# aubin-tchoi/shot-fpfh

Measured on AMD Instinct MI355X. Metric: descriptors/sec (SHOT+FPFH) on 1M-pt cloud, higher is better.
Workload: dtype f64

## Files before the change

### include/shotfpfh.h

```cpp
#ifndef SHOTFPFH_H
#define SHOTFPFH_H

#include <stddef.h>
#include <stdint.h>

#ifdef __cplusplus
extern "C" {
#endif

#define SF_OK 0
#define SF_ERR_ARG (-1)
#define SF_ERR_HIP (-2)
#define SF_ERR_NOMEM (-3)
#define SF_ERR_COMM (-4)
#define SF_ERR_STATE (-5)
#define SF_ERR_UNSUPPORTED (-6)
#define SF_ERR_BIN_RANGE (-7)

#define SF_HOST 0
#define SF_OUT_DEVICE 1
#define SF_IN_DEVICE 2

#define SF_SHOT_LEN 352
#define SF_SHOT_MAX_COSINE_BINS 64
#define SF_FAST_FPFH_BINS 8
#define SF_MAX_FPFH_BINS 1290

typedef struct sf_ctx sf_ctx;
typedef struct sf_cloud sf_cloud;
typedef struct sf_nbrs sf_nbrs;
typedef struct sf_spfh sf_spfh;
typedef struct sf_voxels sf_voxels;

const char *sf_last_error(void);
const char *sf_version(void);
int sf_device_count(void);
sf_ctx *sf_create(int device);
void sf_destroy(sf_ctx *ctx);
int sf_sync(sf_ctx *ctx);
void *sf_stream(sf_ctx *ctx);
int sf_fork(sf_ctx *ctx);
int sf_switch(sf_ctx *ctx, int side);
int sf_join(sf_ctx *ctx);
int sf_mark(sf_ctx *ctx);
int sf_wait_mark(sf_ctx *ctx);

void *sf_dev_alloc(sf_ctx *ctx, size_t bytes);
int sf_dev_free(sf_ctx *ctx, void *dev_ptr);
void *sf_host_alloc(sf_ctx *ctx, size_t bytes);
int sf_host_free(sf_ctx *ctx, void *host_ptr);
int sf_h2d(sf_ctx *ctx, void *dst_dev, const void *src_host, size_t bytes);
int sf_d2h(sf_ctx *ctx, void *dst_host, const void *src_dev, size_t bytes);
int sf_d2d(sf_ctx *ctx, void *dst_dev, const void *src_dev, size_t bytes);

sf_cloud *sf_cloud_upload(sf_ctx *ctx, const double *xyz, const double *normals, int64_t n, int flags);
int sf_cloud_set_normals(sf_ctx *ctx, sf_cloud *cloud, const double *normals, int flags);
int sf_cloud_build_grid(sf_ctx *ctx, sf_cloud *cloud, double cell);
int sf_cloud_build_grid_block(sf_ctx *ctx, sf_cloud *cloud, double cell, int64_t begin, int64_t end, int reach,
                              int64_t *pop_begin, int64_t *pop_end);
int64_t sf_cloud_size(const sf_cloud *cloud);
void sf_cloud_free(sf_ctx *ctx, sf_cloud *cloud);
int sf_cloud_perm(sf_ctx *ctx, sf_cloud *cloud, int32_t *perm);
int sf_cloud_halo_range(sf_ctx *ctx, sf_cloud *cloud, int64_t begin, int64_t end, int64_t *halo_begin,
                        int64_t *halo_end);
int sf_cloud_layer_table(sf_ctx *ctx, sf_cloud *cloud, int64_t *first, int64_t cap, int64_t *n_layers);

sf_nbrs *sf_radius_search(sf_ctx *ctx, sf_cloud *cloud, const double *queries, int64_t m, double radius,
                          int flags);
sf_nbrs *sf_radius_search_self(sf_ctx *ctx, sf_cloud *cloud, double radius, int64_t begin, int64_t end);
sf_nbrs *sf_knn_search(sf_ctx *ctx, sf_cloud *cloud, const double *queries, int64_t m, int k, int flags);
sf_nbrs *sf_nbrs_import(sf_ctx *ctx, sf_cloud *cloud, const double *queries, int64_t m, const int64_t *offsets,
                        const int64_t *idx, double radius, int flags);
sf_nbrs *sf_nbrs_slice(sf_ctx *ctx, sf_nbrs *nbrs, int64_t first, int64_t count);
int64_t sf_nbrs_num_queries(const sf_nbrs *nbrs);
int64_t sf_nbrs_total(const sf_nbrs *nbrs);
int64_t sf_nbrs_max_count(const sf_nbrs *nbrs);
int64_t sf_nbrs_max_count_all(const sf_nbrs *nbrs);
int sf_nbrs_export(sf_ctx *ctx, sf_cloud *cloud, sf_nbrs *nbrs, int64_t *offsets ,
                   int32_t *idx , double *dist );
void sf_nbrs_free(sf_ctx *ctx, sf_nbrs *nbrs);

int sf_normals_radius(sf_ctx *ctx, sf_cloud *cloud, const double *queries, int64_t m, int64_t begin, int64_t end, double radius,
                      const double *pre, double *out , int flags);
int sf_normals(sf_ctx *ctx, sf_cloud *cloud, sf_nbrs *nbrs, const double *pre, double *out ,
               int flags);

int sf_iss_saliency(sf_ctx *ctx, sf_cloud *cloud, double salient_radius, double gamma_21, double gamma_32, int min_neighbors,
                    double *saliency , int32_t *count , int flags);
int sf_iss_select(sf_ctx *ctx, sf_cloud *cloud, const double *saliency , double non_max_radius, int min_neighbors,
                  int64_t *selected , int64_t *n_selected, int flags);
int sf_iss_keypoints(sf_ctx *ctx, sf_cloud *cloud, double salient_radius, double non_max_radius, double gamma_21, double gamma_32,
                     int min_neighbors, double *saliency , int64_t *selected , int64_t *n_selected,
                     int flags);
int sf_pca(sf_ctx *ctx, sf_cloud *cloud, sf_nbrs *nbrs, double *eigenvalues ,
           double *eigenvectors , double *moments , int flags);

int sf_shot_lrf(sf_ctx *ctx, sf_cloud *cloud, sf_nbrs *nbrs, double *lrf , int flags);
int sf_shot(sf_ctx *ctx, sf_cloud *cloud, sf_nbrs *nbrs, const double *lrf , int normalize,
            int64_t min_neighborhood_size, double *out , int flags);
int sf_shot_single_scale(sf_ctx *ctx, sf_cloud *cloud, sf_nbrs *nbrs, int normalize, int64_t min_neighborhood_size,
                         double *lrf , double *out , int flags);

int sf_azimuth_idx(sf_ctx *ctx, const double *x, const double *y, int64_t n, int64_t *idx, int flags);
int sf_shot_serial(sf_ctx *ctx, sf_cloud *cloud, sf_nbrs *nbrs, int64_t min_neighborhood_size, double *out ,
                   int flags);
int sf_shot_serial_bins(sf_ctx *ctx, sf_cloud *cloud, sf_nbrs *nbrs, int64_t n_cosine_bins, int64_t min_neighborhood_size,
                        double *out , int flags);

typedef struct sf_graph sf_graph;
unsigned long long sf_sync_count(void);
int sf_graph_begin(sf_ctx *ctx);
sf_graph *sf_graph_end(sf_ctx *ctx);
int sf_graph_launch(sf_ctx *ctx, sf_graph *graph);
void sf_graph_free(sf_ctx *ctx, sf_graph *graph);

sf_spfh *sf_spfh_create(sf_ctx *ctx, sf_cloud *cloud, int n_bins, int64_t max_count);
sf_spfh *sf_spfh_create_for_radius(sf_ctx *ctx, sf_cloud *cloud, int n_bins, int64_t max_count, double radius);
int sf_spfh_elem_bytes(const sf_spfh *spfh);
int sf_spfh_compute(sf_ctx *ctx, sf_cloud *cloud, sf_nbrs *self_nbrs, sf_spfh *spfh, const double *edges);
int sf_spfh_compute_moments(sf_ctx *ctx, sf_cloud *cloud, sf_nbrs *self_nbrs, sf_spfh *spfh, const double *edges,
                            double *cov_dev );
int sf_shot_from_moments(sf_ctx *ctx, sf_cloud *cloud, sf_nbrs *nbrs, const double *cov_dev , int normalize,
                         int64_t min_neighborhood_size, double *lrf , double *out ,
                         int flags);
int sf_lrf_raw_from_moments(sf_ctx *ctx, sf_cloud *cloud, sf_nbrs *nbrs, const double *cov_dev, double *lrf_dev);
int sf_shot_from_raw_lrf(sf_ctx *ctx, sf_cloud *cloud, sf_nbrs *nbrs, double *lrf_dev, int normalize,
                         int64_t min_neighborhood_size, double *out_dev);
int sf_spfh_allgather(sf_ctx *ctx, sf_spfh *spfh, int64_t rows_per_rank);
int sf_spfh_exchange_rows(sf_ctx *ctx, sf_spfh *spfh, int n_ops, const int *peer, const int64_t *send_begin,
                          const int64_t *send_end, const int64_t *recv_begin, const int64_t *recv_end);
int sf_spfh_rows_image(sf_ctx *ctx, sf_spfh *spfh, int64_t begin, int64_t end, void *host, size_t cap, int write_back,
                       size_t *bytes);
int sf_spfh_export(sf_ctx *ctx, sf_cloud *cloud, sf_spfh *spfh, double *out , int flags);
void sf_spfh_free(sf_ctx *ctx, sf_spfh *spfh);
int sf_fpfh(sf_ctx *ctx, sf_cloud *cloud, sf_nbrs *self_nbrs, sf_spfh *spfh, const int64_t *kp_idx, int64_t m,
            double *out , int flags);

int sf_match_argmin(sf_ctx *ctx, const double *a, int64_t m1, const double *b, int64_t m2, int64_t d,
                    int64_t *idx, double *dist, int64_t *col_idx, int flags);
int sf_match_top2(sf_ctx *ctx, const double *a, int64_t m1, const double *b, int64_t m2, int64_t d,
                  int64_t *idx, double *dist, int64_t *n_exact, int flags);

int sf_rows_nonzero(sf_ctx *ctx, const double *rows_dev, int64_t m, int64_t d, unsigned char *mask_dev);
int sf_rows_gather(sf_ctx *ctx, const double *rows_dev, int64_t n_rows, const int64_t *sel_dev, int64_t m, int64_t d,
                   double *out_dev);
int sf_match_argmin_multiscale(sf_ctx *ctx, const double *a, const double *b, int n_scales, int64_t m1, int64_t m2,
                               int64_t d, const unsigned char *a_ok, const unsigned char *b_ok, double max_val,
                               int64_t *idx, double *dist, int flags);

int sf_match_col_candidates(sf_ctx *ctx, const double *local_dist_dev, const double *global_dist_dev,
                            const int64_t *local_idx_dev, int64_t row_offset, int64_t m, void *cand_dev);

typedef struct sf_match_stream sf_match_stream;
sf_match_stream *sf_match_stream_begin(sf_ctx *ctx, const double *a_dev, const unsigned char *a_ok_dev, int64_t m1,
                                       const double *b_dev, const unsigned char *b_ok_dev, int64_t m2, int64_t d,
                                       double b_entry_max, int64_t max_ranges);
int sf_match_stream_feed(sf_ctx *ctx, sf_match_stream *stream, int64_t row_begin, int64_t row_end);
int sf_match_stream_end(sf_ctx *ctx, sf_match_stream *stream, int64_t *idx_dev, double *dist_dev );
void sf_match_stream_abort(sf_ctx *ctx, sf_match_stream *stream);
int sf_rows_abs_max(sf_ctx *ctx, const double *rows_dev, int64_t m, int64_t d, double *out_host);

int sf_ransac_score(sf_ctx *ctx, const double *a, const double *b, int64_t m, const double *Rt, int64_t n_draws,
                    double thr, int64_t *inliers, int flags);

#define SF_RANSAC_MIN_DRAW_SIZE 3
#define SF_RANSAC_MAX_DRAW_SIZE 8
int sf_ransac_hypotheses(sf_ctx *ctx, const double *a_dev, const double *b_dev, int64_t m, const int64_t *draws_dev,
                         int64_t n_draws, int draw_size, double edge_similarity, unsigned char *status_dev, double *Rt_dev);
int sf_ransac_refit_sums(sf_ctx *ctx, const double *a_dev, const double *b_dev, int64_t m, const double *Rt , double thr,
                         double *sums );
int sf_ransac_prerejective(sf_ctx *ctx, const double *a_dev, const double *b_dev, int64_t m, const int64_t *draws_dev,
                           int64_t n_draws, int draw_size, double edge_similarity, double thr, unsigned char *status_dev,
                           double *Rt_dev, int64_t *map_dev, int64_t *counts_dev, int64_t *result , double *best_Rt );

int sf_fgr_sums(sf_ctx *ctx, const double *a_dev, const double *b_dev, int64_t m, const int64_t *sel_dev , int64_t k,
                const double *state , double *sums );
int sf_fgr(sf_ctx *ctx, const double *a_dev, const double *b_dev, int64_t m, const int64_t *sel_dev , int64_t k,
           double distance_threshold, int iterations, int decrease_every, double division_factor, double *Rt ,
           double *info , double *trace );

int sf_consistency_degree(sf_ctx *ctx, const double *a_dev, const double *b_dev, int64_t m,
                          const unsigned char *member_dev , double distance_threshold, double min_edge,
                          unsigned *degree_out_dev);
int sf_consistency_group(sf_ctx *ctx, const double *a_dev, const double *b_dev, int64_t m, double distance_threshold,
                         double min_edge, unsigned *degree_dev, unsigned char *member_dev, unsigned *group_degree_dev,
                         int64_t *info );

#define SF_SC2_MAX_MATCHES 32768
#define SF_SC2_TILE 256
#define SF_SC2_PAD(m) (((m) + SF_SC2_TILE - 1) / SF_SC2_TILE * SF_SC2_TILE)
int sf_consistency_matrix(sf_ctx *ctx, const double *a_dev, const double *b_dev, int64_t m, double distance_threshold,
                          double min_edge, unsigned char *cmat_dev);
int sf_consistency_sc2(sf_ctx *ctx, const unsigned char *cmat_dev, int64_t m, unsigned *s2_dev);
int sf_consistency_sc2_group(sf_ctx *ctx, const double *a_dev, const double *b_dev, int64_t m, double distance_threshold,
                             double min_edge, unsigned *s2_dev, unsigned char *member_dev, unsigned *group_degree_dev,
                             int64_t *info );

#define SF_SC2_MAX_SEEDS 1024
#define SF_SC2_SEED_TILE 64
int sf_sc2_seeds(sf_ctx *ctx, const unsigned *s2_dev, int64_t m, int64_t n_seeds, int *seeds_dev);
int sf_sc2_seed_rows(sf_ctx *ctx, const unsigned char *cmat_dev, int64_t m, const int *seeds_dev, int64_t n_seeds,
                     unsigned *rows_dev);
int sf_sc2_seed_fits(sf_ctx *ctx, const double *a_dev, const double *b_dev, int64_t m, const int *seeds_dev,
                     const unsigned *rows_dev, int64_t n_seeds, double group_share, unsigned char *status_dev, int *size_dev,
                     double *Rt_dev, double *sums_dev , unsigned char *member_dev );
int sf_sc2_registration(sf_ctx *ctx, const double *a_dev, const double *b_dev, int64_t m, double distance_threshold,
                        double min_edge, int64_t n_seeds, double group_share, unsigned *s2_dev, int *seeds_dev,
                        unsigned char *status_dev, int *size_dev, double *Rt_dev, int64_t *map_dev, int64_t *counts_dev,
                        int64_t *result , double *best_Rt );

sf_voxels *sf_voxels_build(sf_ctx *ctx, const double *xyz, int64_t n, double voxel_size, int flags);
int64_t sf_voxels_count(const sf_voxels *vox);
int sf_voxels_inverse(sf_ctx *ctx, sf_voxels *vox, int64_t *inverse );
int sf_voxels_select(sf_ctx *ctx, sf_voxels *vox, const int64_t *order , int64_t *selected ,
                     int64_t *counts );
void sf_voxels_free(sf_ctx *ctx, sf_voxels *vox);

int sf_icp_accumulate(sf_ctx *ctx, sf_cloud *ref, const double *pts_dev, const int64_t *sel_dev, int64_t m, const double *Rt,
                      double d_max, int mode, double *sums );
int sf_transform_points(sf_ctx *ctx, double *pts_dev, int64_t n, const double *Rt );

int sf_icp_accumulate_gicp(sf_ctx *ctx, sf_cloud *ref, const double *pts_dev, const double *nrm_dev ,
                           const int64_t *sel_dev, int64_t m, const double *Rt, double d_max, double epsilon, double *sums );

int sf_icp_accumulate_robust(sf_ctx *ctx, sf_cloud *ref, const double *pts_dev, const double *nrm_dev ,
                             const int64_t *sel_dev, int64_t m, const double *Rt, double d_max, int mode , double epsilon,
                             int loss , double scale, double *sums );

int sf_comm_unique_id(char id[128]);
int sf_comm_init(sf_ctx *ctx, const char id[128], int nranks, int rank);
int sf_comm_allgather(sf_ctx *ctx, const void *send_dev, void *recv_dev, size_t bytes_per_rank);
int sf_comm_exchange(sf_ctx *ctx, int n_ops, const int *peer, const void *const *send_dev, const size_t *send_bytes,
                     void *const *recv_dev, const size_t *recv_bytes);
int sf_comm_allreduce_min_u64(sf_ctx *ctx, const void *send_dev, void *recv_dev, size_t n);
int sf_comm_collective_stats(sf_ctx *ctx, int on);
int sf_comm_destroy(sf_ctx *ctx);

int sf_profile_enable(sf_ctx *ctx, int on);
int sf_profile_reset(sf_ctx *ctx);
int sf_profile_only(sf_ctx *ctx, const char *name);
int64_t sf_profile_report(sf_ctx *ctx, char *buf, int64_t cap);

#ifdef __cplusplus
}
#endif
#endif
```

### shot_fpfh_amd/_ffi.py

```python
from __future__ import annotations

import ctypes as C
import os

_HERE = os.path.dirname(os.path.abspath(__file__))
LIB_PATH = os.path.join(_HERE, "libshotfpfh.so")

SF_HOST, SF_OUT_DEVICE, SF_IN_DEVICE = 0, 1, 2
SHOT_LEN = 352
MAX_COSINE_BINS = 64
SF_ERR_BIN_RANGE = -7
MAX_FPFH_BINS = 1290


class ShotFpfhError(RuntimeError):
    """Raised for any failure reported by the native library (or its absence)."""


_vp, _i64, _i32, _f64, _int, _sz = C.c_void_p, C.c_int64, C.c_int32, C.c_double, C.c_int, C.c_size_t

SIGNATURES = {
    "sf_last_error": (C.c_char_p, []),
    "sf_version": (C.c_char_p, []),
    "sf_device_count": (_int, []),
    "sf_create": (_vp, [_int]),
    "sf_destroy": (None, [_vp]),
    "sf_sync": (_int, [_vp]),
    "sf_stream": (_vp, [_vp]),
    "sf_fork": (_int, [_vp]),
    "sf_switch": (_int, [_vp, _int]),
    "sf_join": (_int, [_vp]),
    "sf_mark": (_int, [_vp]),
    "sf_wait_mark": (_int, [_vp]),
    "sf_dev_alloc": (_vp, [_vp, _sz]),
    "sf_dev_free": (_int, [_vp, _vp]),
    "sf_host_alloc": (_vp, [_vp, _sz]),
    "sf_host_free": (_int, [_vp, _vp]),
    "sf_h2d": (_int, [_vp, _vp, _vp, _sz]),
    "sf_d2h": (_int, [_vp, _vp, _vp, _sz]),
    "sf_d2d": (_int, [_vp, _vp, _vp, _sz]),
    "sf_cloud_upload": (_vp, [_vp, _vp, _vp, _i64, _int]),
    "sf_cloud_set_normals": (_int, [_vp, _vp, _vp, _int]),
    "sf_cloud_build_grid": (_int, [_vp, _vp, _f64]),
    "sf_cloud_build_grid_block": (_int, [_vp, _vp, _f64, _i64, _i64, _int, _vp, _vp]),
    "sf_cloud_size": (_i64, [_vp]),
    "sf_cloud_free": (None, [_vp, _vp]),
    "sf_cloud_perm": (_int, [_vp, _vp, _vp]),
    "sf_cloud_halo_range": (_int, [_vp, _vp, _i64, _i64, _vp, _vp]),
    "sf_cloud_layer_table": (_int, [_vp, _vp, _vp, _i64, _vp]),
    "sf_radius_search": (_vp, [_vp, _vp, _vp, _i64, _f64, _int]),
    "sf_radius_search_self": (_vp, [_vp, _vp, _f64, _i64, _i64]),
    "sf_knn_search": (_vp, [_vp, _vp, _vp, _i64, _int, _int]),
    "sf_nbrs_import": (_vp, [_vp, _vp, _vp, _i64, _vp, _vp, _f64, _int]),
    "sf_nbrs_slice": (_vp, [_vp, _vp, _i64, _i64]),
    "sf_nbrs_num_queries": (_i64, [_vp]),
    "sf_nbrs_total": (_i64, [_vp]),
    "sf_nbrs_max_count": (_i64, [_vp]),
    "sf_nbrs_max_count_all": (_i64, [_vp]),
    "sf_nbrs_export": (_int, [_vp, _vp, _vp, _vp, _vp, _vp]),
    "sf_nbrs_free": (None, [_vp, _vp]),
    "sf_normals": (_int, [_vp, _vp, _vp, _vp, _vp, _int]),
    "sf_normals_radius": (_int, [_vp, _vp, _vp, _i64, _i64, _i64, _f64, _vp, _vp, _int]),
    "sf_iss_saliency": (_int, [_vp, _vp, _f64, _f64, _f64, _int, _vp, _vp, _int]),
    "sf_iss_select": (_int, [_vp, _vp, _vp, _f64, _int, _vp, _vp, _int]),
    "sf_iss_keypoints": (_int, [_vp, _vp, _f64, _f64, _f64, _f64, _int, _vp, _vp, _vp, _int]),
    "sf_pca": (_int, [_vp, _vp, _vp, _vp, _vp, _vp, _int]),
    "sf_shot_lrf": (_int, [_vp, _vp, _vp, _vp, _int]),
    "sf_shot": (_int, [_vp, _vp, _vp, _vp, _int, _i64, _vp, _int]),
    "sf_shot_single_scale": (_int, [_vp, _vp, _vp, _int, _i64, _vp, _vp, _int]),
    "sf_azimuth_idx": (_int, [_vp, _vp, _vp, _i64, _vp, _int]),
    "sf_shot_serial": (_int, [_vp, _vp, _vp, _i64, _vp, _int]),
    "sf_shot_serial_bins": (_int, [_vp, _vp, _vp, _i64, _i64, _vp, _int]),
    "sf_sync_count": (C.c_ulonglong, []),
    "sf_graph_begin": (_int, [_vp]),
    "sf_graph_end": (_vp, [_vp]),
    "sf_graph_launch": (_int, [_vp, _vp]),
    "sf_graph_free": (None, [_vp, _vp]),
    "sf_spfh_create": (_vp, [_vp, _vp, _int, _i64]),
    "sf_spfh_create_for_radius": (_vp, [_vp, _vp, _int, _i64, C.c_double]),
    "sf_spfh_elem_bytes": (_int, [_vp]),
    "sf_spfh_compute": (_int, [_vp, _vp, _vp, _vp, _vp]),
    "sf_spfh_compute_moments": (_int, [_vp, _vp, _vp, _vp, _vp, _vp]),
    "sf_shot_from_moments": (_int, [_vp, _vp, _vp, _vp, _int, _i64, _vp, _vp, _int]),
    "sf_lrf_raw_from_moments": (_int, [_vp, _vp, _vp, _vp, _vp]),
    "sf_shot_from_raw_lrf": (_int, [_vp, _vp, _vp, _vp, _int, _i64, _vp]),
    "sf_spfh_allgather": (_int, [_vp, _vp, _i64]),
    "sf_spfh_exchange_rows": (_int, [_vp, _vp, _int, _vp, _vp, _vp, _vp, _vp]),
    "sf_spfh_rows_image": (_int, [_vp, _vp, _i64, _i64, _vp, _sz, _int, _vp]),
    "sf_spfh_export": (_int, [_vp, _vp, _vp, _vp, _int]),
    "sf_spfh_free": (None, [_vp, _vp]),
    "sf_fpfh": (_int, [_vp, _vp, _vp, _vp, _vp, _i64, _vp, _int]),
    "sf_match_argmin": (_int, [_vp, _vp, _i64, _vp, _i64, _i64, _vp, _vp, _vp, _int]),
    "sf_match_top2": (_int, [_vp, _vp, _i64, _vp, _i64, _i64, _vp, _vp, _vp, _int]),
    "sf_rows_nonzero": (_int, [_vp, _vp, _i64, _i64, _vp]),
    "sf_rows_gather": (_int, [_vp, _vp, _i64, _vp, _i64, _i64, _vp]),
    "sf_match_argmin_multiscale": (_int, [_vp, _vp, _vp, _int, _i64, _i64, _i64, _vp, _vp, _f64, _vp, _vp, _int]),
    "sf_match_col_candidates": (_int, [_vp, _vp, _vp, _vp, _i64, _i64, _vp]),
    "sf_match_stream_begin": (_vp, [_vp, _vp, _vp, _i64, _vp, _vp, _i64, _i64, _f64, _i64]),
    "sf_match_stream_feed": (_int, [_vp, _vp, _i64, _i64]),
    "sf_match_stream_end": (_int, [_vp, _vp, _vp, _vp]),
    "sf_match_stream_abort": (None, [_vp, _vp]),
    "sf_rows_abs_max": (_int, [_vp, _vp, _i64, _i64, _vp]),
    "sf_ransac_score": (_int, [_vp, _vp, _vp, _i64, _vp, _i64, _f64, _vp, _int]),
    "sf_ransac_hypotheses": (_int, [_vp, _vp, _vp, _i64, _vp, _i64, _int, _f64, _vp, _vp]),
    "sf_ransac_refit_sums": (_int, [_vp, _vp, _vp, _i64, _vp, _f64, _vp]),
    "sf_ransac_prerejective": (_int, [_vp, _vp, _vp, _i64, _vp, _i64, _int, _f64, _f64, _vp, _vp, _vp, _vp, _vp, _vp]),
    "sf_fgr_sums": (_int, [_vp, _vp, _vp, _i64, _vp, _i64, _vp, _vp]),
    "sf_fgr": (_int, [_vp, _vp, _vp, _i64, _vp, _i64, _f64, _int, _int, _f64, _vp, _vp, _vp]),
    "sf_consistency_degree": (_int, [_vp, _vp, _vp, _i64, _vp, _f64, _f64, _vp]),
    "sf_consistency_group": (_int, [_vp, _vp, _vp, _i64, _f64, _f64, _vp, _vp, _vp, _vp]),
    "sf_consistency_matrix": (_int, [_vp, _vp, _vp, _i64, _f64, _f64, _vp]),
    "sf_consistency_sc2": (_int, [_vp, _vp, _i64, _vp]),
    "sf_consistency_sc2_group": (_int, [_vp, _vp, _vp, _i64, _f64, _f64, _vp, _vp, _vp, _vp]),
    "sf_sc2_seeds": (_int, [_vp, _vp, _i64, _i64, _vp]),
    "sf_sc2_seed_rows": (_int, [_vp, _vp, _i64, _vp, _i64, _vp]),
    "sf_sc2_seed_fits": (_int, [_vp, _vp, _vp, _i64, _vp, _vp, _i64, _f64, _vp, _vp, _vp, _vp, _vp]),
    "sf_sc2_registration": (_int, [_vp, _vp, _vp, _i64, _f64, _f64, _i64, _f64, _vp, _vp, _vp, _vp, _vp, _vp, _vp, _vp, _vp]),
    "sf_voxels_build": (_vp, [_vp, _vp, _i64, _f64, _int]),
    "sf_voxels_count": (_i64, [_vp]),
    "sf_voxels_inverse": (_int, [_vp, _vp, _vp]),
    "sf_voxels_select": (_int, [_vp, _vp, _vp, _vp, _vp]),
    "sf_voxels_free": (None, [_vp, _vp]),
    "sf_icp_accumulate": (_int, [_vp, _vp, _vp, _vp, _i64, _vp, _f64, _int, _vp]),
    "sf_transform_points": (_int, [_vp, _vp, _i64, _vp]),
    "sf_icp_accumulate_gicp": (_int, [_vp, _vp, _vp, _vp, _vp, _i64, _vp, _f64, _f64, _vp]),
    "sf_icp_accumulate_robust": (_int, [_vp, _vp, _vp, _vp, _vp, _i64, _vp, _f64, _int, _f64, _int, _f64, _vp]),
    "sf_comm_unique_id": (_int, [_vp]),
    "sf_comm_init": (_int, [_vp, _vp, _int, _int]),
    "sf_comm_allgather": (_int, [_vp, _vp, _vp, _sz]),
    "sf_comm_exchange": (_int, [_vp, _int, _vp, _vp, _vp, _vp, _vp]),
    "sf_comm_allreduce_min_u64": (_int, [_vp, _vp, _vp, _sz]),
    "sf_comm_collective_stats": (_int, [_vp, _int]),
    "sf_comm_destroy": (_int, [_vp]),
    "sf_profile_enable": (_int, [_vp, _int]),
    "sf_profile_reset": (_int, [_vp]),
    "sf_profile_only": (_int, [_vp, C.c_char_p]),
    "sf_profile_report": (_i64, [_vp, _vp, _i64]),
}

_lib = None


def load() -> C.CDLL:
    global _lib
    if _lib is not None:
        return _lib
    if not os.path.exists(LIB_PATH):
        raise ShotFpfhError(
            f"{LIB_PATH} is missing: build it with `python -c 'import __graft_entry__ as g; g.build()'` "
            "(hipcc --offload-arch=gfx950).  shot_fpfh_amd has no CPU fallback."
        )
    try:
        lib = C.CDLL(LIB_PATH, mode=C.RTLD_GLOBAL)
    except OSError as exc:
        raise ShotFpfhError(f"cannot load {LIB_PATH}: {exc}") from exc
    for name, (res, args) in SIGNATURES.items():
        fn = getattr(lib, name)
        fn.restype = res
        fn.argtypes = args
    _lib = lib
    return lib


def last_error() -> str:
    return load().sf_last_error().decode("utf-8", "replace")


def check(rc: int, what: str = "") -> None:
    if rc != 0:
        raise ShotFpfhError(f"{what or 'libshotfpfh'} failed ({rc}): {last_error()}")


def check_handle(h, what: str):
    if not h:
        raise ShotFpfhError(f"{what} failed: {last_error()}")
    return h
```

### shot_fpfh_amd/csrc/device_util.h

```cpp
#pragma once
#include <hip/hip_runtime.h>

#include <cstdint>

struct sf_cloud;

struct sf_grid_desc {
    double lo[3];
    double inv_cell;
    double inv_cell_x;
    double cell;
    int dim[3];
    int xsub;
};

#ifdef __HIPCC__
__host__ __device__ inline int sf_cell_coord(double v, double lo, double inv_cell, int dim)
{
    double t = floor((v - lo) * inv_cell);
    if (!(t >= 0.0)) t = 0.0;
    double top = (double)(dim - 1);
    if (t > top) t = top;
    return (int)t;
}

__device__ inline int sf_lane() { return (int)__builtin_amdgcn_mbcnt_hi(~0u, __builtin_amdgcn_mbcnt_lo(~0u, 0u)); }

__device__ inline int sf_prefix_count(unsigned long long mask)
{
    return (int)__builtin_amdgcn_mbcnt_hi((unsigned)(mask >> 32), __builtin_amdgcn_mbcnt_lo((unsigned)mask, 0u));
}

__device__ inline double sf_wave_sum(double v)
{
#define SF_DPP_ADD_ALL(ctrl)                                                                                    \
    {                                                                                                           \
        const int lo = __builtin_amdgcn_mov_dpp(__double2loint(v), ctrl, 0xf, 0xf, true);                       \
        const int hi = __builtin_amdgcn_mov_dpp(__double2hiint(v), ctrl, 0xf, 0xf, true);                       \
        v += __hiloint2double(hi, lo);                                                                          \
    }
#define SF_DPP_ADD(ctrl, row_mask)                                                                              \
    {                                                                                                           \
        const int lo = __builtin_amdgcn_update_dpp(0, __double2loint(v), ctrl, row_mask, 0xf, false);           \
        const int hi = __builtin_amdgcn_update_dpp(0, __double2hiint(v), ctrl, row_mask, 0xf, false);           \
        v += __hiloint2double(hi, lo);                                                                          \
    }
    SF_DPP_ADD_ALL(0xB1)
    SF_DPP_ADD_ALL(0x4E)
    SF_DPP_ADD_ALL(0x141)
    SF_DPP_ADD_ALL(0x140)
    SF_DPP_ADD(0x142, 0xa)
    SF_DPP_ADD(0x143, 0xc)
#undef SF_DPP_ADD
#undef SF_DPP_ADD_ALL
    return __hiloint2double(__builtin_amdgcn_readlane(__double2hiint(v), 63),
                            __builtin_amdgcn_readlane(__double2loint(v), 63));
}

__device__ inline double sf_wave_max_nonneg(double v)
{
#define SF_DPP_MAX(ctrl, row_mask)                                                                              \
    {                                                                                                           \
        const int lo = __builtin_amdgcn_update_dpp(0, __double2loint(v), ctrl, row_mask, 0xf, false);           \
        const int hi = __builtin_amdgcn_update_dpp(0, __double2hiint(v), ctrl, row_mask, 0xf, false);           \
        v = fmax(v, __hiloint2double(hi, lo));                                                                  \
    }
    SF_DPP_MAX(0xB1, 0xf)
    SF_DPP_MAX(0x4E, 0xf)
    SF_DPP_MAX(0x141, 0xf)
    SF_DPP_MAX(0x140, 0xf)
    SF_DPP_MAX(0x142, 0xa)
    SF_DPP_MAX(0x143, 0xc)
#undef SF_DPP_MAX
    return __hiloint2double(__builtin_amdgcn_readlane(__double2hiint(v), 63),
                            __builtin_amdgcn_readlane(__double2loint(v), 63));
}

__device__ inline double sf_wave_sum8(const double (&v)[8])
{
    const int lane = sf_lane();
    const bool b5 = lane & 32, b4 = lane & 16, b3 = lane & 8;
    double k4[4], k2[2];
#pragma unroll
    for (int i = 0; i < 4; ++i) {
        const double mine = b5 ? v[4 + i] : v[i], send = b5 ? v[i] : v[4 + i];
        k4[i] = mine + __shfl_xor(send, 32);
    }
#pragma unroll
    for (int i = 0; i < 2; ++i) {
        const double mine = b4 ? k4[2 + i] : k4[i], send = b4 ? k4[i] : k4[2 + i];
        k2[i] = mine + __shfl_xor(send, 16);
    }
    double r;
    {
        const double mine = b3 ? k2[1] : k2[0], send = b3 ? k2[0] : k2[1];
        const int lo = __builtin_amdgcn_update_dpp(0, __double2loint(send), 0x128, 0xf, 0xf, false);
        const int hi = __builtin_amdgcn_update_dpp(0, __double2hiint(send), 0x128, 0xf, 0xf, false);
        r = mine + __hiloint2double(hi, lo);
    }
#define SF_DPP_ADD(ctrl)                                                                                  \
    {                                                                                                     \
        const int lo = __builtin_amdgcn_update_dpp(0, __double2loint(r), ctrl, 0xf, 0xf, false);          \
        const int hi = __builtin_amdgcn_update_dpp(0, __double2hiint(r), ctrl, 0xf, 0xf, false);          \
        r += __hiloint2double(hi, lo);                                                                    \
    }
    SF_DPP_ADD(0xB1)
    SF_DPP_ADD(0x4E)
    SF_DPP_ADD(0x141)
#undef SF_DPP_ADD
    return r;
}

__device__ inline double sf_wave_sum4(const double (&v)[4])
{
    const int lane = sf_lane();
    const bool b5 = lane & 32, b4 = lane & 16;
    double k2[2];
#pragma unroll
    for (int i = 0; i < 2; ++i) {
        const double mine = b5 ? v[2 + i] : v[i], send = b5 ? v[i] : v[2 + i];
        k2[i] = mine + __shfl_xor(send, 32);
    }
    const double mine = b4 ? k2[1] : k2[0], send = b4 ? k2[0] : k2[1];
    double r = mine + __shfl_xor(send, 16);
#define SF_DPP_ADD(ctrl)                                                                                  \
    {                                                                                                     \
        const int lo = __builtin_amdgcn_update_dpp(0, __double2loint(r), ctrl, 0xf, 0xf, false);          \
        const int hi = __builtin_amdgcn_update_dpp(0, __double2hiint(r), ctrl, 0xf, 0xf, false);          \
        r += __hiloint2double(hi, lo);                                                                    \
    }
    SF_DPP_ADD(0xB1)
    SF_DPP_ADD(0x4E)
    SF_DPP_ADD(0x141)
    SF_DPP_ADD(0x140)
#undef SF_DPP_ADD
    return r;
}
__device__ inline double sf_read_lane(double v, int lane)
{
    return __hiloint2double(__builtin_amdgcn_readlane(__double2hiint(v), lane), __builtin_amdgcn_readlane(__double2loint(v), lane));
}

__device__ inline double sf_row16_sum(double v)
{
#define SF_DPP_ADD(ctrl)                                                                                  \
    {                                                                                                     \
        const int lo = __builtin_amdgcn_update_dpp(0, __double2loint(v), ctrl, 0xf, 0xf, false);          \
        const int hi = __builtin_amdgcn_update_dpp(0, __double2hiint(v), ctrl, 0xf, 0xf, false);          \
        v += __hiloint2double(hi, lo);                                                                    \
    }
    SF_DPP_ADD(0xB1)
    SF_DPP_ADD(0x4E)
    SF_DPP_ADD(0x141)
    SF_DPP_ADD(0x140)
#undef SF_DPP_ADD
    return v;
}

__device__ inline int sf_row16_sum(int v)
{
    v += __builtin_amdgcn_update_dpp(0, v, 0xB1, 0xf, 0xf, false);
    v += __builtin_amdgcn_update_dpp(0, v, 0x4E, 0xf, 0xf, false);
    v += __builtin_amdgcn_update_dpp(0, v, 0x141, 0xf, 0xf, false);
    v += __builtin_amdgcn_update_dpp(0, v, 0x140, 0xf, 0xf, false);
    return v;
}

__device__ inline void sf_store_stream(double *p, double v) { __builtin_nontemporal_store(v, p); }
__device__ inline void sf_store_stream2(double *p, double a, double b)
{
    typedef double sf_d2 __attribute__((ext_vector_type(2)));
    const sf_d2 v = {a, b};
    __builtin_nontemporal_store(v, reinterpret_cast<sf_d2 *>(p));
}

#define SF_LIST_LOAD(p) __builtin_nontemporal_load(p)
#define SF_LIST_STORE(p, v) __builtin_nontemporal_store((int)(v), p)

__device__ inline long long sf_xcd_block()
{
    const unsigned b = blockIdx.x, chunk = gridDim.x >> 3;
    return (long long)(b & 7u) * chunk + (b >> 3);
}

__device__ inline void sf_load_xyz(const double *__restrict__ rec, int j, double &x, double &y, double &z)
{
    const double2 *p = reinterpret_cast<const double2 *>(rec + 6 * (size_t)j);
    const double2 a = p[0], b = p[1];
    x = a.x; y = a.y; z = b.x;
}
__device__ inline void sf_load_pn(const double *__restrict__ rec, int j, double &x, double &y, double &z, double &nx,
                                  double &ny, double &nz)
{
    const double2 *p = reinterpret_cast<const double2 *>(rec + 6 * (size_t)j);
    const double2 a = p[0], b = p[1], c = p[2];
    x = a.x; y = a.y; z = b.x; nx = b.y; ny = c.x; nz = c.y;
}

__device__ inline double sf_sqrt_fast(double x)
{
    const double y = __builtin_amdgcn_rsq(x);
    double g = x * y, h = 0.5 * y;
    const double r = __builtin_fma(-h, g, 0.5);
    g = __builtin_fma(g, r, g);
    h = __builtin_fma(h, r, h);
    const double d = __builtin_fma(-g, g, x);
    g = __builtin_fma(d, h, g);
    return x > 0.0 ? g : 0.0;
}

__device__ inline double sf_rcp_fast(double d)
{
    double r = __builtin_amdgcn_rcp(d);
    double e = __builtin_fma(-d, r, 1.0);
    r = __builtin_fma(r, e, r);
    e = __builtin_fma(-d, r, 1.0);
    return __builtin_fma(r, e, r);
}

__device__ inline int sf_uniform(int v) { return __builtin_amdgcn_readfirstlane(v); }

__device__ inline long long sf_uniform64(long long v)
{
    unsigned lo = (unsigned)__builtin_amdgcn_readfirstlane((int)(unsigned)v);
    unsigned hi = (unsigned)__builtin_amdgcn_readfirstlane((int)(unsigned)((unsigned long long)v >> 32));
    return (long long)(((unsigned long long)hi << 32) | lo);
}
#endif

static inline unsigned sf_xcd_grid(long long blocks) { return (unsigned)(((blocks + 7) / 8) * 8); }

sf_grid_desc sf_make_grid_desc(const sf_cloud *c);
int sf_cloud_ensure_sorted_normals(struct sf_ctx *ctx, sf_cloud *c);
int sf_cloud_ensure_inv_perm(struct sf_ctx *ctx, sf_cloud *c);
int sf_cloud_normals_max2(struct sf_ctx *ctx, sf_cloud *c, double *out);
```

### shot_fpfh_amd/csrc/fpfh.hip

```cpp
#include <algorithm>
#include <cmath>
#include <cstring>

#include "common.h"
#include "device_util.h"

namespace {


template <typename CT, int LPR, int NP, int NCH>
__global__ __launch_bounds__(256) void k_fpfh(const double *__restrict__ rec, const int64_t *__restrict__ offset,
                                              const int32_t *__restrict__ cnt, const int32_t *__restrict__ idx,
                                              int64_t nbrs_begin,
                                              const int32_t *__restrict__ kp_pos, int64_t m, int nb3, int stride,
                                              const CT *__restrict__ counts, unsigned table_bytes,
                                              const int32_t *__restrict__ kk, double *__restrict__ out)
{
    constexpr int BPP = 16 / (int)sizeof(CT);
    constexpr int RPI = 64 / LPR;
    const int lane = threadIdx.x & 63;
    const int64_t q = sf_uniform64(sf_xcd_block() * 4 + (threadIdx.x >> 6));
    if (q >= m) return;
    const int64_t i = kp_pos ? (int64_t)kp_pos[q] : nbrs_begin + q;
    const int64_t slot = i - nbrs_begin;
// ... 23 lines not shown
            acc[u][0] = __builtin_fma(u2d(v.x & 0xffffu), ww, acc[u][0]);
            acc[u][1] = __builtin_fma(u2d(v.x), ww, acc[u][1]);
            acc[u][2] = __builtin_fma(u2d(v.y & 0xffffu), ww, acc[u][2]);
            acc[u][3] = __builtin_fma(u2d(v.y), ww, acc[u][3]);
            acc[u][4 % BPP] = __builtin_fma(u2d(v.z & 0xffffu), ww, acc[u][4 % BPP]);
            acc[u][5 % BPP] = __builtin_fma(u2d(v.z), ww, acc[u][5 % BPP]);
            acc[u][6 % BPP] = __builtin_fma(u2d(v.w & 0xffffu), ww, acc[u][6 % BPP]);
            acc[u][7 % BPP] = __builtin_fma(u2d(v.w), ww, acc[u][7 % BPP]);
        } else {
            acc[u][0] = __builtin_fma(u2d(v.x), ww, acc[u][0]);
            acc[u][1] = __builtin_fma(u2d(v.y), ww, acc[u][1]);
            acc[u][2] = __builtin_fma(u2d(v.z), ww, acc[u][2]);
            acc[u][3] = __builtin_fma(u2d(v.w), ww, acc[u][3]);
        }
    };
    auto stream_rows = [&](int j, double w, int cnt) {
        constexpr int UNR = 4;
        for (int tt = 0; tt < cnt; tt += RPI * UNR) {
            uint4 v[UNR][NP];
            double ww[UNR];
#pragma unroll
            for (int e = 0; e < UNR; ++e) {
                const int src = tt + e * RPI + grp;
                const int jj = __shfl(j, src & 63);
                ww[e] = (tt + e * RPI < cnt) ? __shfl(w, src & 63) : 0.0;
                const unsigned voff = (unsigned)jj * (unsigned)(LPR * 16 * NP) + (unsigned)piece * 16u;
#pragma unroll
                for (int u = 0; u < NP; ++u) {
                    const auto r = __builtin_amdgcn_raw_buffer_load_b128(rsrc, voff + (unsigned)u * 1024u, 0, 0);
                    v[e][u] = make_uint4(r[0], r[1], r[2], r[3]);
                }
            }
#pragma unroll
            for (int e = 0; e < UNR; ++e)
#pragma unroll
                for (int u = 0; u < NP; ++u) accumulate(v[e][u], ww[e], u);
        }
    };
    if (NCH > 0) {
        constexpr int NC = NCH > 0 ? NCH : 1;
        int jv[NC];
        double wv[NC];
#pragma unroll
        for (int c = 0; c < NC; ++c) {
            const int t = c * 64 + lane;
            jv[c] = t < k ? idx[s + t] : -1;
        }
        double gx[NC], gy[NC], gz[NC];
        int gk[NC];
#pragma unroll
        for (int c = 0; c < NC; ++c) {
            if (c * 64 < k) {
                const int j = jv[c] < 0 ? 0 : jv[c];
                sf_load_xyz(rec, j, gx[c], gy[c], gz[c]);
                gk[c] = kk[j];
            } else {
                gx[c] = gy[c] = gz[c] = 0.0;
                gk[c] = 1;
            }
        }
#pragma unroll
        for (int c = 0; c < NC; ++c) {
            if (c * 64 < k) {
                wv[c] = jv[c] < 0 ? 0.0 : weight_of(gx[c], gy[c], gz[c], gk[c]);
                jv[c] = jv[c] < 0 ? 0 : jv[c];
                stream_rows(jv[c], wv[c], min(64, k - c * 64));
            }
        }
    } else {
        for (int t0 = 0; t0 < k; t0 += 64) {
            const int t = t0 + lane;
            int j = 0;
            double w = 0.0;
            if (t < k) {
                j = idx[s + t];
                double x, y, z;
                sf_load_xyz(rec, j, x, y, z);
                w = weight_of(x, y, z, kk[j]);
            }
            stream_rows(j, w, min(64, k - t0));
        }
    }
#pragma unroll
    for (int off = LPR; off < 64; off <<= 1)
#pragma unroll
        for (int u = 0; u < NP; ++u)
#pragma unroll
            for (int e = 0; e < BPP; ++e) acc[u][e] += __shfl_xor(acc[u][e], off);
    if (sizeof(CT) == 2) {
#pragma unroll
        for (int u = 0; u < NP; ++u)
#pragma unroll
            for (int e = 1; e < BPP; e += 2) acc[u][e] = (acc[u][e] - acc[u][e - 1]) * (1.0 / 65536.0);
    }
    {
        const double kd = (double)k;
        double inv_k = __builtin_amdgcn_rcp(kd);
        inv_k = __builtin_fma(inv_k, __builtin_fma(-kd, inv_k, 1.0), inv_k);
        inv_k = __builtin_fma(inv_k, __builtin_fma(-kd, inv_k, 1.0), inv_k);
        const CT *own = counts + i * (int64_t)stride;
        double *o = out + q * (int64_t)nb3;
#pragma unroll
        for (int u = 0; u < NP; ++u)
#pragma unroll
            for (int e0 = 0; e0 < BPP; e0 += RPI) {
                double a = acc[u][e0];
#pragma unroll
                for (int g = 1; g < RPI; ++g)
                    if (e0 + g < BPP) a = grp == g ? acc[u][e0 + g] : a;
                const int e = e0 + grp;
                const int b = (u * 64 + piece) * BPP + e;
                if (e < BPP && b < nb3) o[b] = (double)own[b] / kd + a * inv_k;
            }
    }
}

#include "fpfh_mc.h"

__device__ inline void fpfh_mc_wrong_form(const unsigned *__restrict__ live, double *__restrict__ out, int64_t q, int nb3)
{
    const int lane = threadIdx.x & 63;
    for (int b = lane; b < nb3; b += 64) out[q * nb3 + b] = __builtin_nan("");
    if (lane == 0) atomicOr(const_cast<unsigned *>(live) + 2, 1u);
}

template <int NKS, bool HI, bool PADC = false>
__global__ __launch_bounds__(64 * SF_MC_WPB) __attribute__((amdgpu_waves_per_eu(PADC ? 5 : 6, 8))) void k_fpfh_mc(const double *__restrict__ rec, const int64_t *__restrict__ offset,
                                                 const int32_t *__restrict__ cnt, const int32_t *__restrict__ idx,
                                                 int64_t nbrs_begin, const int32_t *__restrict__ kp_pos, int64_t m,
                                                 sf_bin_window W, const uint8_t *__restrict__ counts, unsigned table_bytes,
                                                 const double *__restrict__ p4, const unsigned *__restrict__ live,
                                                 const uint8_t *__restrict__ packed, unsigned packed_bytes,
                                                 double *__restrict__ out, const uint8_t *__restrict__ hi, int limit,
                                                 const int32_t *__restrict__ sel, int64_t nsel, int64_t view_first)
{
    __shared__ __attribute__((aligned(16))) unsigned rowbuf_all[SF_MC_WPB][32 * 32];
    __shared__ __attribute__((aligned(16))) unsigned char abuf_all[SF_MC_WPB][9 * 64];
    const int wv_id = threadIdx.x >> 6;
    int64_t q = sf_uniform64(sf_xcd_block() * SF_MC_WPB + wv_id);
    if (sel) {
        if (q >= nsel) return;
        q = (int64_t)sf_uniform(sel[q]) - view_first;
        if (q < 0) return;
    }
    if (q >= m) return;
    if (__popc(sf_uniform(*live) & 0xffu) <= 2) {
        fpfh_mc_wrong_form(live, out, q, W.nb3);
        return;
    }
    fpfh_mc_body<NKS, HI, PADC>(rec, offset, cnt, idx, nbrs_begin, kp_pos, W, counts, table_bytes, p4, out, q, rowbuf_all[wv_id],
                          abuf_all[wv_id], hi, limit);
}

template <int NKS, bool HI>
__global__ __launch_bounds__(64 * SF_MC_WPB) __attribute__((amdgpu_waves_per_eu(8, 8))) void k_fpfh_mc_sparse(
    const double *__restrict__ rec, const int64_t *__restrict__ offset, const int32_t *__restrict__ cnt,
    const int32_t *__restrict__ idx, int64_t nbrs_begin, const int32_t *__restrict__ kp_pos, int64_t m, sf_bin_window W,
    const uint8_t *__restrict__ counts, unsigned table_bytes, const double *__restrict__ p4, const unsigned *__restrict__ live,
    const uint8_t *__restrict__ packed, unsigned packed_bytes, double *__restrict__ out, const uint8_t *__restrict__ hi, int limit,
    const int32_t *__restrict__ sel, int64_t nsel, int64_t view_first)
{
    __shared__ __attribute__((aligned(16))) unsigned rowbuf_all[SF_MC_WPB][32 * 32];
    __shared__ __attribute__((aligned(16))) unsigned char abuf_all[SF_MC_WPB][9 * 64];
    const int wv_id = threadIdx.x >> 6;
    int64_t q = sf_uniform64(sf_xcd_block() * SF_MC_WPB + wv_id);
    if (sel) {
        if (q >= nsel) return;
        q = (int64_t)sf_uniform(sel[q]) - view_first;
        if (q < 0) return;
    }
    if (q >= m) return;
    const unsigned mask = sf_uniform(*live) & 0xffu;
    if (__popc(mask) > 2) {
        fpfh_mc_wrong_form(live, out, q, W.nb3);
        return;
    }
    const int b0 = mask ? __ffs(mask) - 1 : 0;
    const unsigned rest = mask & (mask - 1u);
    const int b1 = rest ? __ffs(rest) - 1 : (b0 + 1) & 7;
    if (sf_uniform(live[1]) == mask) {
        fpfh_mc_body_sparse<NKS, true, HI>(rec, offset, cnt, idx, nbrs_begin, kp_pos, W, counts, packed, packed_bytes, p4, out, q,
                                           b0, b1, rowbuf_all[wv_id], abuf_all[wv_id], hi, limit);
    } else {
        fpfh_mc_body_sparse<NKS, false, HI>(rec, offset, cnt, idx, nbrs_begin, kp_pos, W, counts, counts, table_bytes, p4, out, q,
                                            b0, b1, rowbuf_all[wv_id], abuf_all[wv_id], hi, limit);
    }
}

#ifndef SF_MCL_SC
#define SF_MCL_SC 8
#endif
template <bool SEL, bool SPARSE, bool PADC = false>
__global__ __launch_bounds__(64 * SF_MC_WPB) void k_fpfh_mcl(const double *__restrict__ rec, const int64_t *__restrict__ offset,
                                                 const int32_t *__restrict__ cnt, const int32_t *__restrict__ idx,
                                                 int64_t nbrs_begin, const int32_t *__restrict__ kp_pos, int64_t m,
                                                 sf_bin_window W, const uint8_t *__restrict__ counts, unsigned table_bytes,
                                                 const double *__restrict__ p4, const unsigned *__restrict__ live,
                                                 const uint8_t *__restrict__ packed, unsigned packed_bytes,
                                                 double *__restrict__ out, const uint8_t *__restrict__ hi, int limit,
                                                 const int32_t *__restrict__ sel, int64_t nsel, int64_t view_first)
{
    __shared__ __attribute__((aligned(16))) unsigned rowbuf_all[SF_MC_WPB][32 * 32];
    __shared__ __attribute__((aligned(16))) unsigned char abuf_all[SF_MC_WPB][9 * 64];
    const int wv_id = threadIdx.x >> 6;
    int64_t q = sf_uniform64(sf_xcd_block() * SF_MC_WPB + wv_id);
    if (SEL) {
        if (q >= nsel) return;
        q = (int64_t)sf_uniform(sel[q]) - view_first;
        if (q < 0) return;
    }
    if (q >= m) return;
    const unsigned mask = sf_uniform(*live) & 0xffu;
    if ((__popc(mask) <= 2) != SPARSE) {
        const int64_t i = kp_pos ? (int64_t)kp_pos[q] : nbrs_begin + q;
        if (sf_uniform(cnt[i - nbrs_begin]) > limit) fpfh_mc_wrong_form(live, out, q, W.nb3);
        return;
    }
    if (SPARSE) {
        const int b0 = mask ? __ffs(mask) - 1 : 0;
        const unsigned rest = mask & (mask - 1u);
        const int b1 = rest ? __ffs(rest) - 1 : (b0 + 1) & 7;
        if (sf_uniform(live[1]) == mask) {
            fpfh_mcl_body_sparse<true, SF_MCL_SC>(rec, offset, cnt, idx, nbrs_begin, kp_pos, W, counts, packed, packed_bytes, p4, out, q, b0, b1,
                                                  rowbuf_all[wv_id], abuf_all[wv_id], hi, limit);
        } else {
            fpfh_mcl_body_sparse<false, SF_MCL_SC>(rec, offset, cnt, idx, nbrs_begin, kp_pos, W, counts, counts, table_bytes, p4, out, q, b0, b1,
                                                   rowbuf_all[wv_id], abuf_all[wv_id], hi, limit);
        }
    } else {
        fpfh_mcl_body<4, PADC>(rec, offset, cnt, idx, nbrs_begin, kp_pos, W, counts, table_bytes, p4, out, q, rowbuf_all[wv_id], abuf_all[wv_id], hi,
                         limit);
    }
}



constexpr int FG_TILE = 512;
__global__ __launch_bounds__(256) void k_fpfh_generic(const double *__restrict__ rec, const int64_t *__restrict__ offset,
                                                      const int32_t *__restrict__ cnt, const int32_t *__restrict__ idx,
                                                      int64_t nbrs_begin, const int32_t *__restrict__ kp_pos, int64_t m, int nb3,
                                                      int stride, const unsigned *__restrict__ counts,
                                                      const int32_t *__restrict__ kk, double *__restrict__ out)
{
    __shared__ int tj[FG_TILE];
    __shared__ double tinvd[FG_TILE], tk[FG_TILE];
    const int64_t q = blockIdx.x;
    if (q >= m) return;
    const int64_t i = kp_pos ? (int64_t)kp_pos[q] : nbrs_begin + q;
    const int64_t lq = i - nbrs_begin, s = offset[lq];
    const int k = cnt[lq];
    double px, py, pz;
    sf_load_xyz(rec, (int)i, px, py, pz);
    double *o = out + q * (int64_t)nb3;
    for (int t0 = 0; t0 < k || t0 == 0; t0 += FG_TILE) {
        const int nt = min(FG_TILE, k - t0);
        __syncthreads();
        for (int t = threadIdx.x; t < nt; t += 256) {
            const int j = idx[s + t0 + t];
            double x, y, z;
            sf_load_xyz(rec, j, x, y, z);
            const double cx = x - px, cy = y - py, cz = z - pz;
            const double d = sqrt((cx * cx + cy * cy) + cz * cz);
            tj[t] = j;
            tinvd[t] = d > 0.0 ? d : 0.0;
            tk[t] = (double)kk[j];
        }
        __syncthreads();
        for (int b = threadIdx.x; b < nb3; b += 256) {
            double acc = t0 ? o[b] : 0.0;
            for (int t = 0; t < nt; ++t)
                if (tinvd[t] > 0.0) acc += ((double)counts[(int64_t)tj[t] * stride + b] / tk[t]) / tinvd[t];
            o[b] = acc;
        }
        if (k == 0) break;
    }
    __syncthreads();
    const double kd = (double)k;
    for (int b = threadIdx.x; b < nb3; b += 256)
        o[b] = (double)counts[i * (int64_t)stride + b] / kd + o[b] / kd;
}

__global__ void k_map_positions(const int64_t *__restrict__ kp_idx, const int32_t *__restrict__ inv_perm, int64_t m,
                                int64_t n, int32_t *__restrict__ pos, int *__restrict__ bad)
{
    int64_t i = (int64_t)blockIdx.x * blockDim.x + threadIdx.x;
    if (i >= m) return;
    int64_t v = kp_idx[i];
    if (v < 0) v += n;
    if (v < 0 || v >= n) { *bad = 1; pos[i] = 0; return; }
    pos[i] = inv_perm[v];
}

}


template <typename CT>
static int launch_fpfh(sf_ctx *ctx, sf_cloud *c, sf_nbrs *nb, sf_spfh *sp, const int32_t *kp_pos, int64_t m,
                       double *dout)
{
    const dim3 grid(sf_xcd_grid(sf_div_up(m, 4))), block(256);
    const size_t tb = (size_t)sp->rows_alloc * sp->stride * sizeof(CT);
    if (tb >= ((size_t)1 << 32)) {
        sf_set_error("sf_fpfh: SPFH table of %zu bytes exceeds the 4 GiB buffer-addressing limit of the K7 kernel", tb);
        return SF_ERR_UNSUPPORTED;
    }
    const unsigned table_bytes = (unsigned)tb;
    const int row_bytes = sp->stride * (int)sizeof(CT);
    int nch = 0;
    if (sizeof(CT) == 2) {
        const int64_t chunks = sf_div_up(nb->max_count > 0 ? nb->max_count : 1, 64);
        nch = chunks <= 2 ? 2 : (chunks <= 4 ? (int)chunks : 0);
    }
#define SF_FPFH_LAUNCH(LPR, NP, NCH)                                                                                 \
    SF_LAUNCH(ctx, "k7_fpfh", (k_fpfh<CT, LPR, NP, NCH>), grid, block, c->rec, nb->offset, nb->count, nb->idx,      \
              nb->self_begin, kp_pos, m, sp->nb3, sp->stride, (const CT *)sp->counts, table_bytes, sp->k, dout)
#define SF_FPFH_SHAPE(LPR, NP)                                                 \
    {                                                                          \
        if (sizeof(CT) == 2 && nch == 2) { SF_FPFH_LAUNCH(LPR, NP, 2); }       \
        else if (sizeof(CT) == 2 && nch == 3) { SF_FPFH_LAUNCH(LPR, NP, 3); }  \
        else if (sizeof(CT) == 2 && nch == 4) { SF_FPFH_LAUNCH(LPR, NP, 4); }  \
        else { SF_FPFH_LAUNCH(LPR, NP, 0); }                                   \
    }
    if (row_bytes == 256) SF_FPFH_SHAPE(16, 1)
    else if (row_bytes == 512) SF_FPFH_SHAPE(32, 1)
    else if (row_bytes == 1024) SF_FPFH_SHAPE(64, 1)
    else if (row_bytes == 2048) SF_FPFH_SHAPE(64, 2)
    else {
        sf_set_error("sf_fpfh: SPFH rows of %d bytes unsupported", row_bytes);
        return SF_ERR_UNSUPPORTED;
    }
#undef SF_FPFH_SHAPE
#undef SF_FPFH_LAUNCH
    return SF_OK;
}

static int launch_fpfh_mc(sf_ctx *ctx, sf_cloud *c, sf_nbrs *nb, sf_spfh *sp, const int32_t *kp_pos, int64_t m, double *dout)
{
    const dim3 grid(sf_xcd_grid(sf_div_up(m, SF_MC_WPB))), block(64 * SF_MC_WPB);
    const size_t tb = (size_t)sp->rows_alloc * 128;
    if (tb >= ((size_t)1 << 32) || sp->stride != 128 || (nb->max_count > 255 && !sp->hi)) {
        sf_set_error("sf_fpfh: uint8 SPFH table of %zu bytes / lists of %lld points outside the matrix-core kernel's range", tb,
                     (long long)nb->max_count);
        return SF_ERR_UNSUPPORTED;
    }
    sf_dispatch d = sf_nbrs_dispatch(nb);
    if (d.chunks == 0 || d.limit > 255) {
        d.chunks = d.chunks == 0 ? 4 : d.chunks;
        d.limit = 255;
    }
    if (kp_pos && d.n_mid) {
        d.chunks = 4;
        d.limit = 255;
        d.n_mid = 0;
    }
    if (sp->win_len > 127) {
        d.chunks = 4;
        d.limit = 255;
        d.n_mid = 0;
    }
    const int long_limit = 255;
    const bool any_tail = nb->max_count > long_limit;
    const uint8_t *hi = sp->hi;
    const sf_bin_window W{sp->nb3, sp->win_lo, sp->win_len};
    const bool padc = sp->win_len > 127;
#define SF_MC_ARGS c->rec, nb->offset, nb->count, nb->idx, nb->self_begin, kp_pos, m, W, (const uint8_t *)sp->counts,       \
                   (unsigned)tb, (const double *)sp->p4, (const unsigned *)sp->live, (const uint8_t *)sp->packed,                \
                   (unsigned)((size_t)sp->rows_alloc * 32), dout, hi
    if (!sp->host_live_valid) {
        void *pin = nullptr;
        SF_CHECK(sf_ctx_pinned(ctx, &pin));
        SF_HIP(hipMemcpyAsync(pin, sp->live, 3 * sizeof(unsigned), hipMemcpyDeviceToHost, ctx->stream));
        SF_HIP(hipStreamSynchronize(ctx->stream));
        memcpy(sp->host_live, pin, 2 * sizeof(unsigned));
        sp->host_live_valid = true;
        if (((const unsigned *)pin)[2]) {
            sf_set_error("sf_fpfh: an earlier launch took the wrong matrix-core form for this table (host copy of the block mask was stale); its rows are NaN");
            return SF_ERR_STATE;
        }
    }
    const bool sparse = __builtin_popcount(sp->host_live[0] & 0xffu) <= 2;
#define SF_MC_LAUNCH2(NAME, GRID, NKS, HI, LIMIT, SELP, NSEL)                                                         \
    if (sparse) { SF_LAUNCH(ctx, NAME, (k_fpfh_mc_sparse<NKS, HI>), GRID, block, SF_MC_ARGS, LIMIT, SELP, NSEL, d.view_first); } \
    else if (padc) { SF_LAUNCH(ctx, NAME, (k_fpfh_mc<4, true, true>), GRID, block, SF_MC_ARGS, LIMIT, SELP, NSEL, d.view_first); } \
    else { SF_LAUNCH(ctx, NAME, (k_fpfh_mc<NKS, true>), GRID, block, SF_MC_ARGS, LIMIT, SELP, NSEL, d.view_first); }
#define SF_MC_LAUNCH(NKS)                                                                                            \
    if (hi) { SF_MC_LAUNCH2("k7_fpfh", grid, NKS, true, d.limit, (const int32_t *)nullptr, (int64_t)0) }             \
    else { SF_MC_LAUNCH2("k7_fpfh", grid, NKS, false, d.limit, (const int32_t *)nullptr, (int64_t)0) }
    if (d.chunks <= 1) { SF_MC_LAUNCH(1); }
    else if (d.chunks == 2) { SF_MC_LAUNCH(2); }
    else if (d.chunks == 3) { SF_MC_LAUNCH(3); }
    else { SF_MC_LAUNCH(4); }
    if (d.n_mid) {
        const dim3 grid_mid(sf_xcd_grid(sf_div_up(d.n_mid, SF_MC_WPB)));
        if (hi) { SF_MC_LAUNCH2("k7_fpfh_mid", grid_mid, 4, true, 255, d.mid_sel, d.n_mid) }
        else { SF_MC_LAUNCH2("k7_fpfh_mid", grid_mid, 4, false, 255, d.mid_sel, d.n_mid) }
    }
#undef SF_MC_LAUNCH
#undef SF_MC_LAUNCH2
    if (any_tail) {
#define SF_MCL_LAUNCH(SEL, GRID, SELP, NSEL, VF)                                                                       \
        if (sparse) { SF_LAUNCH(ctx, "k7_fpfh_tail", (k_fpfh_mcl<SEL, true>), dim3(sf_xcd_grid(sf_div_up(GRID, SF_MC_WPB))), block, SF_MC_ARGS, long_limit, SELP, NSEL, VF); } \
        else if (padc) { SF_LAUNCH(ctx, "k7_fpfh_tail", (k_fpfh_mcl<SEL, false, true>), dim3(sf_xcd_grid(sf_div_up(GRID, SF_MC_WPB))), block, SF_MC_ARGS, long_limit, SELP, NSEL, VF); } \
        else { SF_LAUNCH(ctx, "k7_fpfh_tail", (k_fpfh_mcl<SEL, false>), dim3(sf_xcd_grid(sf_div_up(GRID, SF_MC_WPB))), block, SF_MC_ARGS, long_limit, SELP, NSEL, VF); }
        if (!kp_pos && d.n_tail) {
            SF_MCL_LAUNCH(true, d.n_tail, d.tail_sel, d.n_tail, d.view_first)
        } else {
            SF_MCL_LAUNCH(false, m, (const int32_t *)nullptr, (int64_t)0, (int64_t)0)
        }
#undef SF_MCL_LAUNCH
    }
#undef SF_MC_ARGS
    return SF_OK;
}

extern "C" int sf_fpfh(sf_ctx *ctx, sf_cloud *c, sf_nbrs *nb, sf_spfh *sp, const int64_t *kp_idx, int64_t m, double *out,
                       int flags)
{
    if (!ctx || !c || !nb || !sp || !out || m < 0) { sf_set_error("sf_fpfh: bad argument"); return SF_ERR_ARG; }
    if (!nb->self) { sf_set_error("sf_fpfh: needs a sf_radius_search_self result"); return SF_ERR_ARG; }
    SF_CHECK(sf_nbrs_on_grid(nb, c, "sf_fpfh"));
    if (!kp_idx && m != nb->m) { sf_set_error("sf_fpfh: m must equal the query count when kp_idx is NULL"); return SF_ERR_ARG; }
    if (kp_idx && !(nb->self_begin == 0 && nb->m == c->n)) {
        sf_set_error("sf_fpfh: keypoints by index need neighbour lists of the whole cloud");
        return SF_ERR_ARG;
    }
    SF_HIP(hipSetDevice(ctx->device));
    sf_pool_guard tmp(ctx);
    int32_t *pos = nullptr;
    if (kp_idx && m) {
        const int64_t *src = kp_idx;
        int64_t *dkp = nullptr;
        int *dbad = nullptr;
        if (!(flags & SF_IN_DEVICE)) {
            SF_CHECK(tmp.alloc(&dkp, (size_t)m));
            SF_HIP(hipMemcpyAsync(dkp, kp_idx, (size_t)m * sizeof(int64_t), hipMemcpyHostToDevice, ctx->stream));
            src = dkp;
        }
        SF_CHECK(tmp.alloc(&pos, (size_t)m));
        SF_CHECK(tmp.alloc(&dbad, 1));
        SF_HIP(hipMemsetAsync(dbad, 0, sizeof(int), ctx->stream));
        SF_CHECK(sf_cloud_ensure_inv_perm(ctx, c));
        SF_LAUNCH(ctx, "k7_map_positions", k_map_positions, dim3((unsigned)sf_div_up(m, 256)), dim3(256), src,
                  c->inv_perm, m, c->n, pos, dbad);
        int bad = 0;
        SF_HIP(hipMemcpyAsync(&bad, dbad, sizeof(int), hipMemcpyDeviceToHost, ctx->stream));
        SF_HIP(hipStreamSynchronize(ctx->stream));
        if (bad) {
            sf_set_error("sf_fpfh: keypoint index out of range for a cloud of %lld points", (long long)c->n);
            return SF_ERR_ARG;
        }
    }
    const int64_t tot = m * sp->nb3;
    double *dout = out, *owned = nullptr;
    if (!(flags & SF_OUT_DEVICE)) {
        SF_CHECK(tmp.alloc(&owned, (size_t)tot));
        dout = owned;
    }
    int rc = SF_OK;
    if (m && sp->n_bins > SF_FAST_FPFH_BINS && sp->elem_bytes != 1) {
        if (m > 2147483000LL) { sf_set_error("sf_fpfh: too many keypoints for one launch"); return SF_ERR_UNSUPPORTED; }
        SF_LAUNCH(ctx, "k7_fpfh", k_fpfh_generic, dim3((unsigned)m), dim3(256), c->rec, nb->offset, nb->count, nb->idx,
                  nb->self_begin, (const int32_t *)pos, m, sp->nb3, sp->stride, (const unsigned *)sp->counts, sp->k, dout);
    } else if (m)
        rc = sp->elem_bytes == 1   ? launch_fpfh_mc(ctx, c, nb, sp, pos, m, dout)
             : sp->elem_bytes == 2 ? launch_fpfh<uint16_t>(ctx, c, nb, sp, pos, m, dout)
                                   : launch_fpfh<uint32_t>(ctx, c, nb, sp, pos, m, dout);
    if (rc == SF_OK && owned) {
        if (tot) SF_HIP(hipMemcpyAsync(out, owned, (size_t)tot * sizeof(double), hipMemcpyDeviceToHost, ctx->stream));
        SF_HIP(hipStreamSynchronize(ctx->stream));
    }
    return rc;
}
```

### shot_fpfh_amd/csrc/fpfh_mc.h

```cpp
#pragma once
#include <hip/hip_runtime.h>

#include <cstdint>

#include "device_util.h"

typedef int v4i __attribute__((ext_vector_type(4)));

struct sf_bin_window { int nb3, win_lo, win_len; };
__device__ __forceinline__ void fpfh_mc_zero_outside(double *__restrict__ o, const sf_bin_window &W, int lane)
{
    if (W.win_len != W.nb3)
        for (int b = lane; b < W.nb3; b += 64)
            if (b < W.win_lo || b >= W.win_lo + W.win_len) sf_store_stream(o + b, 0.0);
}

__device__ __forceinline__ void fpfh_mc_store_row(double *__restrict__ o, int n, int i0, double v0, int i1, double v1,
                                                  double *stage , int lane)
{
    if (i0 < n) stage[i0] = v0;
    if (i1 < n) stage[i1] = v1;
    __builtin_amdgcn_fence(__ATOMIC_RELEASE, "wavefront");
    __builtin_amdgcn_wave_barrier();
    __builtin_amdgcn_fence(__ATOMIC_ACQUIRE, "wavefront");
    const int shift = (int)((reinterpret_cast<uintptr_t>(o) >> 3) & 1u);
    const int e = 2 * lane - shift;
    const bool a_ok = e >= 0 && e < n, b_ok = e + 1 < n;
    const double a = a_ok ? stage[e] : 0.0, b = b_ok ? stage[e + 1] : 0.0;
    if (a_ok && b_ok) sf_store_stream2(o + e, a, b);
    else if (a_ok) sf_store_stream(o + e, a);
    else if (b_ok) sf_store_stream(o + e + 1, b);
}

typedef int v2i_t __attribute__((ext_vector_type(2)));
#ifndef SF_MC_WPB
#define SF_MC_WPB 4
#endif

typedef unsigned sf_u2 __attribute__((ext_vector_type(2)));
template <int W>
__device__ __forceinline__ void sf_lane_swap(double &a, double &b)
{
    const unsigned alo = (unsigned)__double2loint(a), ahi = (unsigned)__double2hiint(a);
    const unsigned blo = (unsigned)__double2loint(b), bhi = (unsigned)__double2hiint(b);
    const sf_u2 lo = W == 32 ? __builtin_amdgcn_permlane32_swap(alo, blo, false, false) : __builtin_amdgcn_permlane16_swap(alo, blo, false, false);
    const sf_u2 hi = W == 32 ? __builtin_amdgcn_permlane32_swap(ahi, bhi, false, false) : __builtin_amdgcn_permlane16_swap(ahi, bhi, false, false);
    a = __hiloint2double((int)hi[0], (int)lo[0]);
    b = __hiloint2double((int)hi[1], (int)lo[1]);
}

template <int NKS>
__device__ __forceinline__ void fpfh_mc_list(const int32_t *__restrict__ idx, int64_t s, int k, int lane, int (&jv)[NKS])
{
#pragma unroll
    for (int c = 0; c < NKS; ++c) {
        const int t = c * 64 + lane;
        jv[c] = -1;
        if (c == 0 || c * 64 < k) jv[c] = t < k ? SF_LIST_LOAD(idx + s + t) : -1;
    }
}

template <int NKS, bool HI>
__device__ __forceinline__ int fpfh_mc_weights(const double *__restrict__ p4, double px, double py, double pz, int k,
                                               int (&jv)[NKS], double (&wv)[NKS], unsigned long long (&lm)[NKS])
{
    double gx[NKS], gy[NKS], gz[NKS], gk[NKS];
#pragma unroll
    for (int c = 0; c < NKS; ++c) {
        gx[c] = gy[c] = gz[c] = gk[c] = 0.0;
        if (c == 0 || c * 64 < k) {
            const int j = jv[c] < 0 ? 0 : jv[c];
            const double2 *pp = reinterpret_cast<const double2 *>(p4 + 4 * (size_t)j);
            const double2 u0 = pp[0], u1 = pp[1];
            gx[c] = u0.x; gy[c] = u0.y; gz[c] = u1.x; gk[c] = u1.y;
        }
    }
    double wmax = 0.0;
#pragma unroll
    for (int c = 0; c < NKS; ++c) {
        wv[c] = 0.0;
        if (c == 0 || c * 64 < k) {
            const double cx = gx[c] - px, cy = gy[c] - py, cz = gz[c] - pz;
            const double d2 = (cx * cx + cy * cy) + cz * cz;
            const double kd = gk[c], xx = d2 * (kd * kd);
            const double y0 = __builtin_amdgcn_rsq(xx);
            const double y1 = __builtin_fma(0.5 * y0, __builtin_fma(-(xx * y0), y0, 1.0), y0);
            const double y2 = __builtin_fma(0.5 * y1, __builtin_fma(-(xx * y1), y1, 1.0), y1);
            wv[c] = (jv[c] >= 0 && d2 > 0.0) ? y2 : 0.0;
            wmax = fmax(wmax, wv[c]);
            if (HI) lm[c] = __ballot(wv[c] > 0.0 && kd > 255.0);
        } else if (HI) {
            lm[c] = 0ull;
        }
        jv[c] = jv[c] < 0 ? 0 : jv[c];
    }
    wmax = sf_wave_max_nonneg(wmax);
    const int e2 = wmax > 0.0 ? (int)((__double2hiint(wmax) >> 20) & 0x7ff) - 1023 : 0;
    return 61 - e2;
}

template <int NKS>
__device__ __forceinline__ void fpfh_mc_hi(const uint8_t *__restrict__ hi, const int (&jv)[NKS], const double (&wv)[NKS],
                                           const unsigned long long (&lm)[NKS], int o0, int o1, double &c0, double &c1)
{
#pragma unroll
    for (int c = 0; c < NKS; ++c) {
        unsigned long long mk = lm[c];
        while (mk) {
            int t[4];
            bool on[4];
#pragma unroll
            for (int u = 0; u < 4; ++u) {
                on[u] = mk != 0ull;
                t[u] = on[u] ? __builtin_ctzll(mk) : t[0];
                mk &= mk - 1;
            }
            unsigned b0[4], b1[4];
            double w[4];
#pragma unroll
            for (int u = 0; u < 4; ++u) {
                const int j = __builtin_amdgcn_readlane(jv[c], t[u]);
                const uint8_t *r = hi + (size_t)j * 128;
                b0[u] = r[o0];
                b1[u] = r[o1];
                const double wu = __hiloint2double(__builtin_amdgcn_readlane(__double2hiint(wv[c]), t[u]),
                                                   __builtin_amdgcn_readlane(__double2loint(wv[c]), t[u]));
                w[u] = on[u] ? wu * 256.0 : 0.0;
            }
#pragma unroll
            for (int u = 0; u < 4; ++u) {
                c0 = __builtin_fma(w[u], (double)b0[u], c0);
                c1 = __builtin_fma(w[u], (double)b1[u], c1);
            }
        }
    }
}

__device__ __forceinline__ void fpfh_mc_limbs(unsigned char *abuf, int lane, double w, int S)
{
    const double x = ldexp(w, S - 32);
    const unsigned hi = (unsigned)x;
    const unsigned lo = (unsigned)ldexp(x - (double)hi, 32);
    const unsigned long long W = ((unsigned long long)hi << 32) | lo;
    const unsigned long long D = (W + 0x8080808080808080ull) ^ 0x8080808080808080ull;
    *reinterpret_cast<unsigned long long *>(abuf + 8 * lane) = D;
}

__device__ __forceinline__ long fpfh_mc_a_operand(const unsigned char *abuf, int a, int kb, int st)
{
    const unsigned char *ap = (a & 1) ? abuf + 512 : abuf + 8 * (32 * (st & 1) + 8 * kb + (a >> 1));
    const v2i_t t = __builtin_amdgcn_ds_read_tr8_b64_v2i32((__attribute__((address_space(3))) v2i_t *)ap);
    return (long)(((unsigned long long)(unsigned)t[1] << 32) | (unsigned)t[0]);
}

template <int NKS, bool HI, bool PADC = false>
__device__ __forceinline__ void fpfh_mc_body(const double *__restrict__ rec, const int64_t *__restrict__ offset,
                                             const int32_t *__restrict__ cnt, const int32_t *__restrict__ idx,
                                             int64_t nbrs_begin, const int32_t *__restrict__ kp_pos, sf_bin_window W,
                                             const uint8_t *__restrict__ counts, unsigned table_bytes,
                                             const double *__restrict__ p4, double *__restrict__ out, int64_t q,
                                             unsigned *rowbuf , unsigned char *abuf ,
                                             const uint8_t *__restrict__ hi, int limit)
{
    const int lane = threadIdx.x & 63;
    const int64_t i = kp_pos ? (int64_t)kp_pos[q] : nbrs_begin + q;
    const int64_t slot = i - nbrs_begin;
    const int64_t s = offset[slot];
    const int k = cnt[slot];
    if (sf_uniform(k) > limit) return;
    const double px = rec[6 * i + 0], py = rec[6 * i + 1], pz = rec[6 * i + 2];
    const auto rsrc = __builtin_amdgcn_make_buffer_rsrc(const_cast<uint8_t *>(counts), 0, (int)table_bytes, 0x00020000);
    const int a = lane & 15, kb = lane >> 4;
    const unsigned own0 = counts[i * 128 + 16 * (4 * (kb >> 1) + 2 * (kb & 1)) + a], own1 = counts[i * 128 + 16 * (4 * (kb >> 1) + 2 * (kb & 1)) + a + 16];
    if (lane == 0) *reinterpret_cast<unsigned long long *>(abuf + 512) = 0ull;
    const int frow = ((a >> 2) & 3) | ((kb & 1) << 2);
    const int rd_base = (8 * kb + (a >> 1)) * 128 + 8 * (a & 1);
    int xoff[8];
#pragma unroll
    for (int bb = 0; bb < 8; ++bb) xoff[bb] = rd_base + 16 * (bb ^ frow);
    const int dma_chunk = (lane & 7) ^ ((lane >> 4) & 3);
    const unsigned lds_rows = (unsigned)__builtin_amdgcn_readfirstlane(
        (int)(unsigned)(size_t)(__attribute__((address_space(3))) unsigned *)rowbuf);
#define SF_MC_DMA(ST)                                                                                               \
    {                                                                                                               \
        _Pragma("unroll") for (int u = 0; u < 4; ++u) {                                                             \
            const int jr0 = __shfl(jv[(ST) >> 1], 32 * ((ST) & 1) + 8 * u + (lane >> 3));                           \
            const int jr = jr0 < 0 ? 0 : jr0;                          \
            const unsigned voff = (unsigned)jr * 128u + 16u * (unsigned)(dma_chunk ^ ((u & 1) << 2));              \
            unsigned keep_;                                                                                         \
            asm volatile("s_mov_b32 %0, m0\n\ts_mov_b32 m0, %3\n\ts_nop 0\n\t"                                     \
                         "buffer_load_dwordx4 %1, %2, 0 offen lds\n\ts_mov_b32 m0, %0"                              \
                         : "=&s"(keep_)                                                                             \
                         : "v"(voff), "s"(rsrc), "s"(lds_rows + 1024u * u)                                          \
                         : "memory");                                                                               \
        }                                                                                                           \
    }
    int jv[NKS];
    double wv[NKS];
    unsigned long long lm[NKS];
    fpfh_mc_list<NKS>(idx, s, k, lane, jv);
    SF_MC_DMA(0)
    const int S = fpfh_mc_weights<NKS, HI>(p4, px, py, pz, k, jv, wv, lm);

    v4i acc[8];
#pragma unroll
    for (int bb = 0; bb < 8; ++bb) acc[bb] = v4i{0, 0, 0, 0};
    v4i accp = v4i{0, 0, 0, 0};

#pragma unroll
    for (int st = 0; st < 2 * NKS; ++st) {
        if (st * 32 < k) {
            if (st > 0) SF_MC_DMA(st)
            if ((st & 1) == 0) fpfh_mc_limbs(abuf, lane, wv[st >> 1], S);
            asm volatile("s_waitcnt vmcnt(0)" ::: "memory");
            __builtin_amdgcn_wave_barrier();
            const long A = fpfh_mc_a_operand(abuf, a, kb, st);
            const unsigned char *rb = reinterpret_cast<const unsigned char *>(rowbuf);
#pragma unroll
            for (int bb = 0; bb < 8; ++bb) {
                const v2i_t t = __builtin_amdgcn_ds_read_tr8_b64_v2i32(
                    (__attribute__((address_space(3))) v2i_t *)(rb + xoff[bb]));
                const long B = (long)(((unsigned long long)(unsigned)t[1] << 32) | (unsigned)t[0]);
                acc[bb] = __builtin_amdgcn_mfma_i32_16x16x32_i8(A, B, acc[bb], 0, 0, 0);
            }
            if (PADC) accp = __builtin_amdgcn_mfma_i32_16x16x32_i8(A, (long)0x8080808080808080ull, accp, 0, 0, 0);
            asm volatile("s_waitcnt lgkmcnt(0)" ::: "memory");
            __builtin_amdgcn_wave_barrier();
        }
    }
    int rpad[4];
#pragma unroll
    for (int r = 0; r < 4; ++r) rpad[r] = PADC ? accp[r] : __builtin_amdgcn_update_dpp(0, acc[7][r], 0x150 + 15, 0xf, 0xf, false);
    const int pad01 = (rpad[1] << 8) + rpad[0], pad23 = (rpad[3] << 8) + rpad[2];
    const double p0 = ldexp(1.0, 32 * kb - S);
    const double f0 = p0, f2 = p0 * 65536.0;
    const double kd = (double)k;
    double inv_k = __builtin_amdgcn_rcp(kd);
    inv_k = __builtin_fma(inv_k, __builtin_fma(-kd, inv_k, 1.0), inv_k);
    inv_k = __builtin_fma(inv_k, __builtin_fma(-kd, inv_k, 1.0), inv_k);
    double part[8];
#pragma unroll
    for (int bb = 0; bb < 8; ++bb) {
        const int e01 = ((acc[bb][1] << 8) + acc[bb][0]) - pad01;
        const int e23 = ((acc[bb][3] << 8) + acc[bb][2]) - pad23;
        part[bb] = __builtin_fma((double)e23, f2, (double)e01 * f0);
    }
    double keep[4];
#pragma unroll
    for (int u = 0; u < 4; ++u) {
        double a_ = part[u], b_ = part[4 + u];
        sf_lane_swap<32>(a_, b_);
        keep[u] = a_ + b_;
    }
    double a0 = keep[0], b0_ = keep[2], a1 = keep[1], b1_ = keep[3];
    sf_lane_swap<16>(a0, b0_);
    sf_lane_swap<16>(a1, b1_);
    const double vsel0 = a0 + b0_, vsel1 = a1 + b1_;
    {
        const int bb0 = 4 * (kb >> 1) + 2 * (kb & 1);
        const int b0 = 16 * bb0 + a, b1 = b0 + 16;
        double *o = out + q * (int64_t)W.nb3;
        fpfh_mc_zero_outside(o, W, lane);
        o += W.win_lo;
        const double c0 = (double)(own0 ^ 128u), c1 = (double)(own1 ^ 128u);
        double s0 = c0 * inv_k, s1 = c1 * inv_k;
        s0 = __builtin_fma(__builtin_fma(-s0, kd, c0), inv_k, s0);
        s1 = __builtin_fma(__builtin_fma(-s1, kd, c1), inv_k, s1);
        double h0 = 0.0, h1 = 0.0;
        if (HI) fpfh_mc_hi<NKS>(hi, jv, wv, lm, b0, b1, h0, h1);
        const double r0 = s0 + (HI ? vsel0 + h0 : vsel0) * inv_k, r1 = s1 + (HI ? vsel1 + h1 : vsel1) * inv_k;
        if (W.win_len == W.nb3 && W.win_len <= 126) {
            fpfh_mc_store_row(o, W.win_len, b0, r0, b1, r1, reinterpret_cast<double *>(rowbuf), lane);
        } else {
            if (b0 < W.win_len) sf_store_stream(o + b0, r0);
            if (b1 < W.win_len) sf_store_stream(o + b1, r1);
        }
    }
}

#undef SF_MC_DMA

template <int NKS, bool PACKED, bool HI>
__device__ __forceinline__ void fpfh_mc_body_sparse(const double *__restrict__ rec, const int64_t *__restrict__ offset,
                                                    const int32_t *__restrict__ cnt, const int32_t *__restrict__ idx,
                                                    int64_t nbrs_begin, const int32_t *__restrict__ kp_pos, sf_bin_window W,
                                                    const uint8_t *__restrict__ counts, const uint8_t *__restrict__ rows,
                                                    unsigned rows_bytes, const double *__restrict__ p4,
                                                    double *__restrict__ out, int64_t q, int b0, int b1,
                                                    unsigned *rowbuf , unsigned char *abuf ,
                                                    const uint8_t *__restrict__ hi, int limit)
{
    const int lane = threadIdx.x & 63;
    const int64_t i = kp_pos ? (int64_t)kp_pos[q] : nbrs_begin + q;
    const int64_t slot = i - nbrs_begin;
    const int64_t s = offset[slot];
    const int k = cnt[slot];
    if (sf_uniform(k) > limit) return;
    const double px = rec[6 * i + 0], py = rec[6 * i + 1], pz = rec[6 * i + 2];
    const auto rsrc = __builtin_amdgcn_make_buffer_rsrc(const_cast<uint8_t *>(rows), 0, (int)rows_bytes, 0x00020000);
    const int a = lane & 15, kb = lane >> 4;
    const int bb0 = 4 * (kb >> 1) + 2 * (kb & 1);
    const int o0 = 16 * bb0 + a, o1 = o0 + 16;
    const unsigned own0 = counts[i * 128 + o0], own1 = counts[i * 128 + o1];
    if (lane == 0) *reinterpret_cast<unsigned long long *>(abuf + 512) = 0ull;
    const int d_u = (lane >> 4) & 1, d_row = 16 * (lane >> 5) + (lane & 15);
    const unsigned dma_chunk16 = PACKED ? 16u * (unsigned)d_u : 16u * (unsigned)(d_u ? b1 : b0);
    constexpr unsigned ROW_BYTES = PACKED ? 32u : 128u;
    const int rd_piece = 32 * (kb >> 1) + 8 * (kb & 1) + (a >> 1);
    const int rd0 = 16 * rd_piece + 8 * (a & 1), rd1 = rd0 + 256;
    const unsigned lds_rows = (unsigned)__builtin_amdgcn_readfirstlane(
        (int)(unsigned)(size_t)(__attribute__((address_space(3))) unsigned *)rowbuf);
#define SF_MCS_DMA(ST)                                                                                              \
    {                                                                                                               \
        const int jr0 = __shfl(jv[((ST) >> 1) < NKS ? ((ST) >> 1) : 0], 32 * ((ST) & 1) + d_row);                   \
        const int jr = jr0 < 0 ? 0 : jr0;                              \
        const unsigned voff = (unsigned)jr * ROW_BYTES + dma_chunk16;                                               \
        unsigned keep_;                                                                                             \
        asm volatile("s_mov_b32 %0, m0\n\ts_mov_b32 m0, %3\n\ts_nop 0\n\t"                                         \
                     "buffer_load_dwordx4 %1, %2, 0 offen lds\n\ts_mov_b32 m0, %0"                                  \
                     : "=&s"(keep_)                                                                                 \
                     : "v"(voff), "s"(rsrc), "s"(lds_rows + 1024u * (unsigned)((ST) & 3))                           \
                     : "memory");                                                                                   \
    }
    int jv[NKS];
    double wv[NKS];
    unsigned long long lm[NKS];
    fpfh_mc_list<NKS>(idx, s, k, lane, jv);
    SF_MCS_DMA(0)
    if (32 < k) SF_MCS_DMA(1)
    if (NKS >= 2 && 64 < k) SF_MCS_DMA(2)
    if (NKS >= 2 && 96 < k) SF_MCS_DMA(3)
    const int S = fpfh_mc_weights<NKS, HI>(p4, px, py, pz, k, jv, wv, lm);

    v4i acc0 = v4i{0, 0, 0, 0}, acc1 = v4i{0, 0, 0, 0}, accp = v4i{0, 0, 0, 0};
    const long Bpad = (long)0x8080808080808080ull;

#pragma unroll
    for (int st = 0; st < 2 * NKS; ++st) {
        if (st * 32 < k) {
            if (st >= 4) SF_MCS_DMA(st)
            if ((st & 1) == 0) fpfh_mc_limbs(abuf, lane, wv[st >> 1], S);
            asm volatile("s_waitcnt vmcnt(0)" ::: "memory");
            __builtin_amdgcn_wave_barrier();
            const long A = fpfh_mc_a_operand(abuf, a, kb, st);
            const unsigned char *rb = reinterpret_cast<const unsigned char *>(rowbuf);
            const v2i_t t0 = __builtin_amdgcn_ds_read_tr8_b64_v2i32((__attribute__((address_space(3))) v2i_t *)(rb + rd0 + 1024 * (st & 3)));
            const v2i_t t1 = __builtin_amdgcn_ds_read_tr8_b64_v2i32((__attribute__((address_space(3))) v2i_t *)(rb + rd1 + 1024 * (st & 3)));
            accp = __builtin_amdgcn_mfma_i32_16x16x32_i8(A, Bpad, accp, 0, 0, 0);
            acc0 = __builtin_amdgcn_mfma_i32_16x16x32_i8(A, (long)(((unsigned long long)(unsigned)t0[1] << 32) | (unsigned)t0[0]), acc0, 0, 0, 0);
            acc1 = __builtin_amdgcn_mfma_i32_16x16x32_i8(A, (long)(((unsigned long long)(unsigned)t1[1] << 32) | (unsigned)t1[0]), acc1, 0, 0, 0);
            asm volatile("s_waitcnt lgkmcnt(0)" ::: "memory");
            __builtin_amdgcn_wave_barrier();
        }
    }
    const int pad01 = (accp[1] << 8) + accp[0], pad23 = (accp[3] << 8) + accp[2];
    const double p0 = ldexp(1.0, 32 * kb - S);
    const double f0 = p0, f2 = p0 * 65536.0;
    const double kd = (double)k;
    double inv_k = __builtin_amdgcn_rcp(kd);
    inv_k = __builtin_fma(inv_k, __builtin_fma(-kd, inv_k, 1.0), inv_k);
    inv_k = __builtin_fma(inv_k, __builtin_fma(-kd, inv_k, 1.0), inv_k);
    double part0, part1;
    {
        const int e01 = ((acc0[1] << 8) + acc0[0]) - pad01, e23 = ((acc0[3] << 8) + acc0[2]) - pad23;
        part0 = __builtin_fma((double)e23, f2, (double)e01 * f0);
        const int g01 = ((acc1[1] << 8) + acc1[0]) - pad01, g23 = ((acc1[3] << 8) + acc1[2]) - pad23;
        part1 = __builtin_fma((double)g23, f2, (double)g01 * f0);
    }
    sf_lane_swap<32>(part0, part1);
    double v = part0 + part1;
    double w = v;
    sf_lane_swap<16>(v, w);
    const double tot = v + w;
    double mine = tot, other = tot;
    sf_lane_swap<32>(mine, other);
    const double tot0 = mine, tot1 = other;
    {
        double *o = out + q * (int64_t)W.nb3;
        fpfh_mc_zero_outside(o, W, lane);
        o += W.win_lo;
        const double c0 = (double)(own0 ^ 128u), c1 = (double)(own1 ^ 128u);
        double s0 = c0 * inv_k, s1 = c1 * inv_k;
        s0 = __builtin_fma(__builtin_fma(-s0, kd, c0), inv_k, s0);
        s1 = __builtin_fma(__builtin_fma(-s1, kd, c1), inv_k, s1);
        const double v0 = bb0 == b0 ? tot0 : (bb0 == b1 ? tot1 : 0.0);
        const double v1 = bb0 + 1 == b0 ? tot0 : (bb0 + 1 == b1 ? tot1 : 0.0);
        double h0 = 0.0, h1 = 0.0;
        if (HI) fpfh_mc_hi<NKS>(hi, jv, wv, lm, o0, o1, h0, h1);
        const double r0 = s0 + (HI ? v0 + h0 : v0) * inv_k, r1 = s1 + (HI ? v1 + h1 : v1) * inv_k;
        if (W.win_len == W.nb3 && W.win_len <= 126) {
            fpfh_mc_store_row(o, W.win_len, o0, r0, o1, r1, reinterpret_cast<double *>(rowbuf), lane);
        } else {
            if (o0 < W.win_len) sf_store_stream(o + o0, r0);
            if (o1 < W.win_len) sf_store_stream(o + o1, r1);
        }
    }
}

#undef SF_MCS_DMA

template <int SC>
__device__ __forceinline__ void fpfh_mcl_load(const int32_t *__restrict__ idx, const double *__restrict__ p4, int64_t s, int k,
                                              int base, int lane, double px, double py, double pz, int (&jv)[SC], double (&wv)[SC],
                                              unsigned long long (&lm)[SC])
{
#pragma unroll
    for (int c = 0; c < SC; ++c) {
        const int t = base + 64 * c + lane;
        jv[c] = (base + 64 * c < k && t < k) ? SF_LIST_LOAD(idx + s + t) : -1;
    }
    double2 u0[SC], u1[SC];
#pragma unroll
    for (int c = 0; c < SC; ++c) {
        u0[c] = u1[c] = make_double2(0.0, 0.0);
        if (base + 64 * c < k) {
            const double2 *pp = reinterpret_cast<const double2 *>(p4 + 4 * (size_t)(jv[c] < 0 ? 0 : jv[c]));
            u0[c] = pp[0];
            u1[c] = pp[1];
        }
    }
#pragma unroll
    for (int c = 0; c < SC; ++c) {
        const double cx = u0[c].x - px, cy = u0[c].y - py, cz = u1[c].x - pz;
        const double d2 = (cx * cx + cy * cy) + cz * cz;
        const double kd = u1[c].y, xx = d2 * (kd * kd);
        const double y0 = __builtin_amdgcn_rsq(xx);
        const double y1 = __builtin_fma(0.5 * y0, __builtin_fma(-(xx * y0), y0, 1.0), y0);
        const double y2 = __builtin_fma(0.5 * y1, __builtin_fma(-(xx * y1), y1, 1.0), y1);
        const bool on = jv[c] >= 0;
        wv[c] = (on && d2 > 0.0) ? y2 : 0.0;
        lm[c] = __ballot(wv[c] > 0.0 && kd > 255.0);
        jv[c] = on ? jv[c] : 0;
    }
}

__device__ __forceinline__ double fpfh_mcl_pair(int hi_limb, int lo_limb, int pad_hi, int pad_lo)
{
    return __builtin_fma((double)hi_limb - (double)pad_hi, 256.0, (double)lo_limb - (double)pad_lo);
}

template <bool PACKED, int SC>
__device__ __forceinline__ void fpfh_mcl_body_sparse(const double *__restrict__ rec, const int64_t *__restrict__ offset,
                                                     const int32_t *__restrict__ cnt, const int32_t *__restrict__ idx,
                                                     int64_t nbrs_begin, const int32_t *__restrict__ kp_pos, sf_bin_window W,
                                                     const uint8_t *__restrict__ counts, const uint8_t *__restrict__ rows,
                                                     unsigned rows_bytes, const double *__restrict__ p4,
                                                     double *__restrict__ out, int64_t q, int b0, int b1,
                                                     unsigned *rowbuf , unsigned char *abuf ,
                                                     const uint8_t *__restrict__ hi, int limit)
{
    const int lane = threadIdx.x & 63;
    const int64_t i = kp_pos ? (int64_t)kp_pos[q] : nbrs_begin + q;
    const int64_t slot = i - nbrs_begin;
    const int k = sf_uniform(cnt[slot]);
    if (k <= limit) return;
    const int64_t s = offset[slot];
    const double px = rec[6 * i + 0], py = rec[6 * i + 1], pz = rec[6 * i + 2];
    const auto rsrc = __builtin_amdgcn_make_buffer_rsrc(const_cast<uint8_t *>(rows), 0, (int)rows_bytes, 0x00020000);
    const int a = lane & 15, kb = lane >> 4;
    const int bb0 = 4 * (kb >> 1) + 2 * (kb & 1);
    const int o0 = 16 * bb0 + a, o1 = o0 + 16;
    unsigned own0 = (unsigned)counts[i * 128 + o0] ^ 128u, own1 = (unsigned)counts[i * 128 + o1] ^ 128u;
    if (k > 255) { own0 += 256u * (unsigned)hi[i * 128 + o0]; own1 += 256u * (unsigned)hi[i * 128 + o1]; }
    if (lane == 0) *reinterpret_cast<unsigned long long *>(abuf + 512) = 0ull;
    const int d_u = (lane >> 4) & 1, d_row = 16 * (lane >> 5) + (lane & 15);
    const unsigned dma_chunk16 = PACKED ? 16u * (unsigned)d_u : 16u * (unsigned)(d_u ? b1 : b0);
    constexpr unsigned ROW_BYTES = PACKED ? 32u : 128u;
    const int rd_piece = 32 * (kb >> 1) + 8 * (kb & 1) + (a >> 1);
    const int rd0 = 16 * rd_piece + 8 * (a & 1), rd1 = rd0 + 256;
    const unsigned lds_rows = (unsigned)__builtin_amdgcn_readfirstlane(
        (int)(unsigned)(size_t)(__attribute__((address_space(3))) unsigned *)rowbuf);
#define SF_MCL_DMA(ST)                                                                                              \
    {                                                                                                               \
        const int jr = __shfl(jv[((ST) >> 1) < SC ? ((ST) >> 1) : 0], 32 * ((ST) & 1) + d_row);                     \
        const unsigned voff = (unsigned)jr * ROW_BYTES + dma_chunk16;                                               \
        unsigned keep_;                                                                                             \
        asm volatile("s_mov_b32 %0, m0\n\ts_mov_b32 m0, %3\n\ts_nop 0\n\t"                                         \
                     "buffer_load_dwordx4 %1, %2, 0 offen lds\n\ts_mov_b32 m0, %0"                                  \
                     : "=&s"(keep_)                                                                                 \
                     : "v"(voff), "s"(rsrc), "s"(lds_rows + 1024u * (unsigned)((ST) & 3))                           \
                     : "memory");                                                                                   \
    }
    int jv[SC];
    double wv[SC];
    unsigned long long lm[SC];
    double wmax = 0.0;
    for (int base = 0; base < k; base += 64 * SC) {
        fpfh_mcl_load<SC>(idx, p4, s, k, base, lane, px, py, pz, jv, wv, lm);
#pragma unroll
        for (int c = 0; c < SC; ++c) wmax = fmax(wmax, wv[c]);
    }
    wmax = sf_wave_max_nonneg(wmax);
    const int e2 = wmax > 0.0 ? (int)((__double2hiint(wmax) >> 20) & 0x7ff) - 1023 : 0;
    const int S = 61 - e2;

    v4i acc0 = v4i{0, 0, 0, 0}, acc1 = v4i{0, 0, 0, 0}, accp = v4i{0, 0, 0, 0};
    const long Bpad = (long)0x8080808080808080ull;
    double h0 = 0.0, h1 = 0.0;
    for (int base = 0; base < k; base += 64 * SC) {
        if (k > 64 * SC) fpfh_mcl_load<SC>(idx, p4, s, k, base, lane, px, py, pz, jv, wv, lm);
        const int left = k - base;
        const int nst = left >= 64 * SC ? 2 * SC : (left + 31) >> 5;
#pragma unroll
        for (int st = 0; st < 4; ++st)
            if (st < nst) SF_MCL_DMA(st)
#pragma unroll
        for (int st = 0; st < 2 * SC; ++st) {
            if (st < nst) {
                if ((st & 1) == 0) fpfh_mc_limbs(abuf, lane, wv[st >> 1], S);
                if (st + 3 < nst) asm volatile("s_waitcnt vmcnt(3)" ::: "memory");
                else if (st + 2 < nst) asm volatile("s_waitcnt vmcnt(2)" ::: "memory");
                else if (st + 1 < nst) asm volatile("s_waitcnt vmcnt(1)" ::: "memory");
                else asm volatile("s_waitcnt vmcnt(0)" ::: "memory");
                __builtin_amdgcn_wave_barrier();
                const long A = fpfh_mc_a_operand(abuf, a, kb, st);
                const unsigned char *rb = reinterpret_cast<const unsigned char *>(rowbuf);
                const v2i_t t0 = __builtin_amdgcn_ds_read_tr8_b64_v2i32((__attribute__((address_space(3))) v2i_t *)(rb + rd0 + 1024 * (st & 3)));
                const v2i_t t1 = __builtin_amdgcn_ds_read_tr8_b64_v2i32((__attribute__((address_space(3))) v2i_t *)(rb + rd1 + 1024 * (st & 3)));
                accp = __builtin_amdgcn_mfma_i32_16x16x32_i8(A, Bpad, accp, 0, 0, 0);
                acc0 = __builtin_amdgcn_mfma_i32_16x16x32_i8(A, (long)(((unsigned long long)(unsigned)t0[1] << 32) | (unsigned)t0[0]), acc0, 0, 0, 0);
                acc1 = __builtin_amdgcn_mfma_i32_16x16x32_i8(A, (long)(((unsigned long long)(unsigned)t1[1] << 32) | (unsigned)t1[0]), acc1, 0, 0, 0);
                asm volatile("s_waitcnt lgkmcnt(0)" ::: "memory");
                __builtin_amdgcn_wave_barrier();
                if (st + 4 < nst) SF_MCL_DMA(st + 4)
            }
        }
        fpfh_mc_hi<SC>(hi, jv, wv, lm, o0, o1, h0, h1);
    }
    const double p0 = ldexp(1.0, 32 * kb - S);
// ... 158 lines not shown
```

### shot_fpfh_amd/csrc/spfh.hip

```cpp
#include <algorithm>
#include <cmath>
#include <cstring>

#include "common.h"
#include "device_util.h"

namespace {

#define SF_WIN_FPFH_BINS 11
struct fpfh_edges {
    double a[SF_WIN_FPFH_BINS + 1], p[SF_WIN_FPFH_BINS + 1], t[SF_WIN_FPFH_BINS + 1];
    double tan_t[SF_WIN_FPFH_BINS + 1];
    double p_inv_width;
};

__device__ inline int hist_bin(const double *e, int nb, double x)
{
    if (!(x >= e[0]) || x > e[nb]) return -1;
    int b = 0;
#pragma unroll
    for (int i = 1; i < SF_WIN_FPFH_BINS; ++i)
        if (i < nb && x >= e[i]) b = i;
    return b;
}

__device__ inline int theta_bin(const fpfh_edges &ed, int nb, double a, double b)
{
    const double band = 1e-13;
    const double aa = fabs(a);
    if (b > band * aa) {
        int bin = 0;
        double gap = 1.0e300;
#pragma unroll
        for (int i = 1; i < SF_WIN_FPFH_BINS; ++i)
            if (i < nb) {
                const double di = __builtin_fma(-ed.tan_t[i], b, a);
                bin += di >= 0.0 ? 1 : 0;
                gap = fmin(gap, fabs(di));
            }
        if (gap > band * (aa + fabs(ed.tan_t[1]) * b)) return bin;
    } else if (b < -band * aa) {
        return -1;
    }
    return hist_bin(ed.t, nb, atan2(a, b));
}

__device__ inline int theta_bin_fast(const fpfh_edges &ed, int nb, double a, double b, double E)
{
    const double band = 1e-13;
    const double aa = fabs(a) + E;
    if (b > band * aa) {
        int bin = 0;
        double gap = 1.0e300;
#pragma unroll
        for (int i = 1; i < SF_WIN_FPFH_BINS; ++i)
            if (i < nb) {
                const double di = __builtin_fma(-ed.tan_t[i], b, a);
                bin += di >= 0.0 ? 1 : 0;
                gap = fmin(gap, fabs(di));
            }
        return gap > band * (aa + fabs(ed.tan_t[1]) * b) + E ? bin : -2;
    }
    return b < -band * aa ? -1 : -2;
}

#ifndef SF_SPFH_WPB
#define SF_SPFH_WPB 2
#endif

template <typename CT, int NCH, int NB, bool SEL>
__global__ __launch_bounds__(64 * SF_SPFH_WPB) __attribute__((amdgpu_waves_per_eu((NCH == 0 || NCH >= 4) ? 5 : 6))) void k_spfh(const double *__restrict__ rec,
                                              const int64_t *__restrict__ offset, const int32_t *__restrict__ cnt,
    const int32_t *__restrict__ idx,
                                              int64_t m, int64_t self_begin, fpfh_edges ed, int nb_rt, int nb3, int stride,
                                              CT *__restrict__ counts, int32_t *__restrict__ kout, unsigned bias,
                                              double *__restrict__ p4, double mom_radius, double *__restrict__ cov,
                                              unsigned *__restrict__ live, int alpha_bin, double nrm_max,
                                              uint8_t *__restrict__ packed, int pack_b0, int pack_b1,
                                              uint8_t *__restrict__ hi, int limit, const int32_t *__restrict__ sel,
                                              int64_t nsel, int64_t view_first, int alpha_pair, int win_lo, int win_len)
{
    const int nb = NB > 0 ? NB : nb_rt;
    __shared__ unsigned int hist[SF_SPFH_WPB][SF_FAST_FPFH_BINS * SF_FAST_FPFH_BINS * SF_FAST_FPFH_BINS];
    const int lane = threadIdx.x & 63, wave = threadIdx.x >> 6;
    int64_t q = sf_uniform64(sf_xcd_block() * SF_SPFH_WPB + wave);
    if (SEL) {
        if (q >= nsel) return;
        q = (int64_t)sf_uniform(sel[q]) - view_first;
        if (q < 0) return;
    }
    if (q >= m) return;
    unsigned int *h = hist[wave];
    for (int b = lane; b < win_len; b += 64) h[b] = 0;
    const int64_t i = self_begin + q;
    const int64_t s = offset[q];
    const int k = cnt[q];
#ifndef SF_AB_NOLIMIT
    if (!SEL && sf_uniform(k) > limit) return;
#endif
    const double px = rec[6 * i + 0], py = rec[6 * i + 1], pz = rec[6 * i + 2];
    const double ux = rec[6 * i + 3], uy = rec[6 * i + 4], uz = rec[6 * i + 5];
    __builtin_amdgcn_wave_barrier();
    const double p_inv_width = ed.p_inv_width;
    const double uu = (ux * ux + uy * uy) + uz * uz;
    const double e_per_dist = 1.5e-14 * nrm_max * uu;
    auto pair = [&](double cx, double cy, double cz, double njx, double njy, double njz) {
        const double d2 = (cx * cx + cy * cy) + cz * cz;
        if (d2 > 0.0) {
            const double num = (cx * ux + cy * uy) + cz * uz;
            const double y0 = __builtin_amdgcn_rsq(d2);
            const double y1 = __builtin_fma(0.5 * y0, __builtin_fma(-(d2 * y0), y0, 1.0), y0);
            double phi = num * y1;
            const double pos = (phi - ed.p[0]) * p_inv_width;
            if (fabs(pos - rint(pos)) <= 1e-9) phi = num / sqrt(d2);
            const double b = (njx * ux + njy * uy) + __builtin_fma(njz, uz, 0.0);
            constexpr bool EVEN = NB > 0 && NB % 2 == 0;
            int ba = alpha_bin, bt = -2;
            if (alpha_bin >= 0 || (EVEN && alpha_pair >= 0)) {
                const double nc = (njx * cx + njy * cy) + njz * cz;
                bt = theta_bin_fast(ed, nb, nc * uu - b * num, b, e_per_dist * (d2 * y1) * 1.01);
            }
            if (!EVEN) {
                if (bt == -2) {
                    const double vx = cy * uz - cz * uy, vy = cz * ux - cx * uz, vz = cx * uy - cy * ux;
                    if (alpha_bin < 0) ba = hist_bin(ed.a, nb, (vx * njx + vz * njz) + vy * njy);
                    const double wx = uy * vz - uz * vy, wy = uz * vx - ux * vz, wz = ux * vy - uy * vx;
                    bt = theta_bin(ed, nb, (njx * wx + njz * wz) + njy * wy, b);
                }
            } else if (bt == -2 || alpha_bin < 0) {
                const double vx = cy * uz - cz * uy, vy = cz * ux - cx * uz, vz = cx * uy - cy * ux;
                if (bt == -2) {
                    const double wx = uy * vz - uz * vy, wy = uz * vx - ux * vz, wz = ux * vy - uy * vx;
                    bt = theta_bin(ed, nb, (njx * wx + njz * wz) + njy * wy, b);
                }
                if (alpha_bin < 0) {
                    const double alpha = (vx * njx + vz * njz) + vy * njy;
                    ba = alpha_pair >= 0 ? alpha_pair + (alpha >= ed.a[alpha_pair + 1] ? 1 : 0) : hist_bin(ed.a, nb, alpha);
                }
            }
            const int bp = hist_bin(ed.p, nb, phi);
            if ((ba | bp | bt) >= 0) atomicAdd(&h[(ba * nb + bp) * nb + bt - win_lo], 1u);
        }
    };
    double ws = 0, a11 = 0, a21 = 0, a31 = 0, a22 = 0, a32 = 0, a33 = 0;
    auto moments = [&](double cx, double cy, double cz) {
        const double w = mom_radius - sf_sqrt_fast((cx * cx + cy * cy) + cz * cz);
        ws += w;
        const double wx = cx * w, wy = cy * w, wz = cz * w;
        a11 = __builtin_fma(cx, wx, a11); a21 = __builtin_fma(cy, wx, a21); a31 = __builtin_fma(cz, wx, a31);
        a22 = __builtin_fma(cy, wy, a22); a32 = __builtin_fma(cz, wy, a32); a33 = __builtin_fma(cz, wz, a33);
    };
    if (NCH > 0) {
        constexpr int NC = NCH > 0 ? NCH : 1;
        const int ku = sf_uniform(k);
        int jj[NC];
#pragma unroll
        for (int c = 0; c < NC; ++c) {
            const int t = c * 64 + lane;
            jj[c] = -1;
            if (c == 0 || c * 64 < ku) jj[c] = t < k ? SF_LIST_LOAD(idx + s + t) : -1;
        }
        double cx[NC], cy[NC], cz[NC], ax[NC], ay[NC], az[NC];
#pragma unroll
        for (int c = 0; c < NC; ++c) {
            cx[c] = cy[c] = cz[c] = ax[c] = ay[c] = az[c] = 0.0;
            if (c == 0 || c * 64 < ku) {
                const int j = jj[c] < 0 ? 0 : jj[c];
                sf_load_pn(rec, j, cx[c], cy[c], cz[c], ax[c], ay[c], az[c]);
            }
        }
#pragma unroll
        for (int c = 0; c < NC; ++c)
            if ((c == 0 || c * 64 < ku) && jj[c] >= 0) {
                if (cov) moments(cx[c] - px, cy[c] - py, cz[c] - pz);
                pair(cx[c] - px, cy[c] - py, cz[c] - pz, ax[c], ay[c], az[c]);
            }
    } else {
        for (int t = lane; t < k; t += 64) {
            double x, y, z, a, b, c;
            sf_load_pn(rec, idx[s + t], x, y, z, a, b, c);
            if (cov) moments(x - px, y - py, z - pz);
            pair(x - px, y - py, z - pz, a, b, c);
        }
    }
    if (cov) {
        const double part[8] = {ws, a11, a21, a31, a22, a32, a33, 0.0};
        const double tot = sf_wave_sum8(part);
        const double wsum = __hiloint2double(__builtin_amdgcn_readlane(__double2hiint(tot), 0),
                                             __builtin_amdgcn_readlane(__double2loint(tot), 0));
        const double iw = sf_rcp_fast(wsum);
        const int e = lane >> 3;
        if ((lane & 7) == 0 && e >= 1 && e <= 6) cov[6 * q + e - 1] = tot * iw;
    }
    __builtin_amdgcn_wave_barrier();
    __threadfence_block();
    CT *row = counts + i * (int64_t)stride;
    bool hi_empty = false;
    if (live) {
        const unsigned v0 = lane < win_len ? h[lane] : 0u, v1 = lane + 64 < win_len ? h[lane + 64] : 0u;
        __builtin_nontemporal_store((CT)(v0 ^ bias), row + lane);
        __builtin_nontemporal_store((CT)(v1 ^ bias), row + lane + 64);
        if (hi && sf_uniform(k) > 255) {
            hi[i * 128 + lane] = (uint8_t)(v0 >> 8);
            hi[i * 128 + lane + 64] = (uint8_t)(v1 >> 8);
            hi_empty = __ballot(((v0 | v1) >> 8) != 0u) == 0ull;
        }
        if (packed && lane < 8) {
            const int first = 16 * (lane < 4 ? pack_b0 : pack_b1) + 4 * (lane & 3);
            unsigned w = 0u;
#pragma unroll
            for (int t = 0; t < 4; ++t) w |= (((first + t < win_len ? h[first + t] : 0u) ^ bias) & 0xffu) << (8 * t);
            reinterpret_cast<unsigned *>(packed + i * 32)[lane] = w;
        }
        const unsigned long long n0 = __ballot(v0 != 0u), n1 = __ballot(v1 != 0u);
        unsigned mask = 0u;
#pragma unroll
        for (int kq = 0; kq < 4; ++kq) {
            mask |= ((n0 >> (16 * kq)) & 0xffffull) ? 1u << kq : 0u;
            mask |= ((n1 >> (16 * kq)) & 0xffffull) ? 16u << kq : 0u;
        }
        if (lane == 0 && (mask & ~*live)) atomicOr(live, mask);
    } else {
        for (int b = lane; b < stride; b += 64) row[b] = (CT)((b < nb3 ? h[b] : 0u) ^ bias);
    }
    if (lane == 0) {
        kout[i] = k;
        if (p4) {
            double2 *o = reinterpret_cast<double2 *>(p4 + 4 * i);
            o[0] = make_double2(rec[6 * i + 0], rec[6 * i + 1]);
            o[1] = make_double2(rec[6 * i + 2], hi_empty ? -(double)k : (double)k);
        }
    }
}

__device__ inline void spfh_pack_row(const uint8_t *__restrict__ counts, uint8_t *__restrict__ packed, int64_t row, unsigned mask)
{
    const int b0 = mask ? __ffs(mask) - 1 : 0;
    const unsigned rest = mask & (mask - 1u);
    const int b1 = rest ? __ffs(rest) - 1 : (b0 + 1) & 7;
    const uint4 *src = reinterpret_cast<const uint4 *>(counts + row * 128);
    uint4 *dst = reinterpret_cast<uint4 *>(packed + row * 32);
    dst[0] = src[b0];
    dst[1] = src[b1];
}

__global__ __launch_bounds__(256) void k_spfh_pack(const uint8_t *__restrict__ counts, int64_t begin, int64_t end,
                                                   const unsigned *__restrict__ live, uint8_t *__restrict__ packed)
{
    const unsigned mask = live[0] & 0xffu;
    if (__popc(mask) > 2) return;
    const int64_t row = begin + (int64_t)blockIdx.x * blockDim.x + threadIdx.x;
    if (row < end) spfh_pack_row(counts, packed, row, mask);
}

__global__ __launch_bounds__(256) void k_spfh_repack(const uint8_t *__restrict__ counts, int64_t n, int64_t begin, int64_t end,
                                                     const unsigned *__restrict__ live, uint8_t *__restrict__ packed)
{
    const unsigned mask = live[0] & 0xffu, sig = live[1];
    if (__popc(mask) > 2 || sig == mask) return;
    for (int64_t row = (int64_t)blockIdx.x * blockDim.x + threadIdx.x; row < n; row += (int64_t)gridDim.x * blockDim.x)
        if (row < begin || row >= end) spfh_pack_row(counts, packed, row, mask);
}

__global__ void k_spfh_live_or(unsigned *__restrict__ live, unsigned det) { live[0] |= det; }

__global__ void k_spfh_pack_done(unsigned *__restrict__ live)
{
    const unsigned mask = live[0] & 0xffu;
    live[1] = __popc(mask) <= 2 ? mask : ~0u;
}

template <typename CT>
__global__ void k_spfh_export(const CT *__restrict__ counts, const int32_t *__restrict__ kk,
                              const int32_t *__restrict__ perm, int64_t n, int nb3, int stride, unsigned bias,
                              double *__restrict__ out, const uint8_t *__restrict__ hi, int win_lo, int win_len)
{
    int64_t g = (int64_t)blockIdx.x * blockDim.x + threadIdx.x;
    if (g >= n * nb3) return;
    int64_t i = g / nb3;
    int b = (int)(g - i * nb3);
    const int col = b - win_lo;
    unsigned cnt = 0u;
    if (col >= 0 && col < win_len) {
        cnt = (unsigned)counts[i * stride + col] ^ bias;
        if (hi && kk[i] > 255) cnt += 256u * (unsigned)hi[i * stride + col];
    }
    out[(int64_t)perm[i] * nb3 + b] = (double)cnt / (double)kk[i];
}

__device__ inline int hist_bin_search(const double *__restrict__ e, int nb, double x)
{
    if (!(x >= e[0]) || x > e[nb]) return -1;
    if (x == e[nb]) return nb - 1;
    int lo = 0, hi = nb + 1;
    while (lo < hi) {
        const int mid = (lo + hi) >> 1;
        if (e[mid] <= x) lo = mid + 1; else hi = mid;
    }
    return lo - 1;
}

__global__ __launch_bounds__(256) void k_spfh_generic(const double *__restrict__ rec, const int64_t *__restrict__ offset,
                                                      const int32_t *__restrict__ cnt, const int32_t *__restrict__ idx, int64_t m,
                                                      int64_t self_begin, const double *__restrict__ edges, int nb, int nb3,
                                                      int stride, unsigned *__restrict__ counts, int32_t *__restrict__ kk)
{
    const int lane = threadIdx.x & 63;
    const int64_t q = sf_uniform64(sf_xcd_block() * 4 + (threadIdx.x >> 6));
    if (q >= m) return;
    const int64_t i = self_begin + q, s = offset[q];
    const int k = cnt[q];
    unsigned *row = counts + i * (int64_t)stride;
    for (int b = lane; b < stride; b += 64) row[b] = 0u;
    if (lane == 0) kk[i] = k;
    __threadfence();
    double px, py, pz, ux, uy, uz;
    sf_load_pn(rec, (int)i, px, py, pz, ux, uy, uz);
    const double *ea = edges, *ep = edges + (nb + 1), *et = edges + 2 * (nb + 1);
    for (int t = lane; t < k; t += 64) {
        double x, y, z, nx, ny, nz;
        sf_load_pn(rec, idx[s + t], x, y, z, nx, ny, nz);
        const double cx = x - px, cy = y - py, cz = z - pz;
        const double dist = sqrt((cx * cx + cy * cy) + cz * cz);
        if (!(dist > 0.0)) continue;
        const double vx = cy * uz - cz * uy, vy = cz * ux - cx * uz, vz = cx * uy - cy * ux;
        const double wx = uy * vz - uz * vy, wy = uz * vx - ux * vz, wz = ux * vy - uy * vx;
        const double alpha = (vx * nx + vz * nz) + vy * ny;
        const double phi = (((cx * ux + cy * uy) + cz * uz) + 0.0) / dist;
        const double theta = atan2((nx * wx + nz * wz) + ny * wy, ((nx * ux + ny * uy) + nz * uz) + 0.0);
        const int ba = hist_bin_search(ea, nb, alpha), bp = hist_bin_search(ep, nb, phi), bt = hist_bin_search(et, nb, theta);
        if (ba < 0 || bp < 0 || bt < 0) continue;
        atomicAdd(&row[(ba * nb + bp) * nb + bt], 1u);
    }
}
}


static bool alpha_bins_within_reach(const double *edges_a, int nb, double reach, int *first, int *last)
// ... 16 lines not shown
    return spfh_create(ctx, c, n_bins, max_count, 0.0);
}

extern "C" sf_spfh *sf_spfh_create_for_radius(sf_ctx *ctx, sf_cloud *c, int n_bins, int64_t max_count, double radius)
{
    return spfh_create(ctx, c, n_bins, max_count, radius);
}

extern "C" int sf_spfh_elem_bytes(const sf_spfh *sp) { return sp ? sp->elem_bytes : 0; }

static sf_spfh *spfh_create(sf_ctx *ctx, sf_cloud *c, int n_bins, int64_t max_count, double radius)
{
    if (!ctx || !c) { sf_set_error("sf_spfh_create: null argument"); return nullptr; }
    if (n_bins < 1 || n_bins > SF_MAX_FPFH_BINS) {
        sf_set_error("sf_spfh_create: n_bins=%d outside 1..%d (n_bins^3 bins per point)", n_bins, SF_MAX_FPFH_BINS);
        return nullptr;
    }
    if (hipSetDevice(ctx->device) != hipSuccess) { sf_set_error("hipSetDevice failed"); return nullptr; }
    sf_spfh *sp = new sf_spfh();
    sp->n = c->n;
    sp->n_bins = n_bins;
    sp->nb3 = n_bins * n_bins * n_bins;
    sp->win_lo = 0;
    sp->win_len = sp->nb3;
    bool window = false;
    if (sp->nb3 > 128 && n_bins <= SF_WIN_FPFH_BINS && max_count <= 65535 && radius > 0.0 && c->nrm_orig && !getenv("SF_FPFH_NO_WINDOW")) {
        double n2 = 0.0, ea[SF_WIN_FPFH_BINS + 1];
        if (sf_cloud_normals_max2(ctx, c, &n2) != SF_OK) { delete sp; return nullptr; }
        for (int i = 0; i <= n_bins; ++i) ea[i] = -1.0 + 2.0 * (double)i / (double)n_bins;
        int a0 = 0, a1 = 0;
        if (alpha_bins_within_reach(ea, n_bins, radius * n2 * (1.0 + 1e-6), &a0, &a1) && (a1 - a0 + 1) * n_bins * n_bins <= 128) {
            window = true;
            sp->win_lo = a0 * n_bins * n_bins;
            sp->win_len = (a1 - a0 + 1) * n_bins * n_bins;
        }
    }
    sp->elem_bytes = (max_count <= 65535 && (sp->nb3 <= 128 || window)) ? 1 : (max_count > 65535 ? 4 : 2);
    if (n_bins > SF_FAST_FPFH_BINS && !window) sp->elem_bytes = 4;
    sp->bias = sp->elem_bytes == 1 ? 128 : 0;
    sp->stride = 128;
    while (sp->stride < (window ? sp->win_len : sp->nb3)) sp->stride *= 2;
    if (n_bins > SF_FAST_FPFH_BINS && !window) sp->stride = (sp->nb3 + 3) & ~3;
    const int64_t nr = ctx->nranks > 0 ? ctx->nranks : 1;
    sp->rows_alloc = std::max<int64_t>(sf_div_up(c->n, nr) * nr, 1);
    size_t nn = (size_t)sp->rows_alloc;
    if ((double)nn * sp->stride * sp->elem_bytes > 2.0e11) {
        sf_set_error("sf_spfh_create: an SPFH table of %lld x %d bins does not fit the device", (long long)nn, sp->nb3);
        delete sp;
        return nullptr;
    }
    const bool bytes_tab = sp->elem_bytes == 1;
    bool ok = sf_pool_alloc(ctx, nn * sp->stride * sp->elem_bytes, &sp->counts) == SF_OK && sf_pool_alloc(ctx, nn * sizeof(int32_t), (void **)&sp->k) == SF_OK;
    if (ok && bytes_tab) ok = sf_pool_alloc(ctx, nn * 4 * sizeof(double), (void **)&sp->p4) == SF_OK;
    if (ok && bytes_tab && max_count > 255) ok = sf_pool_alloc(ctx, nn * 128, (void **)&sp->hi) == SF_OK;
    if (ok && bytes_tab)
        ok = sf_pool_alloc(ctx, 4 * sizeof(unsigned), (void **)&sp->live) == SF_OK && sf_pool_alloc(ctx, nn * 32, (void **)&sp->packed) == SF_OK &&
             hipMemsetAsync(sp->live, 0, 4 * sizeof(unsigned), ctx->stream) == hipSuccess &&
             hipMemsetAsync(sp->live, getenv("SF_FPFH_DENSE") ? 0xff : 0, sizeof(unsigned), ctx->stream) == hipSuccess &&
             hipMemsetAsync(sp->live + 1, 0xff, sizeof(unsigned), ctx->stream) == hipSuccess;
    if (!ok) {
        sf_set_error("sf_spfh_create: out of device memory");
        sf_spfh_free(ctx, sp);
        return nullptr;
    }
    sp->host_live[0] = getenv("SF_FPFH_DENSE") ? ~0u : 0u;
    sp->host_live[1] = ~0u;
    sp->host_live_valid = sp->mask_known = sp->elem_bytes == 1;
    return sp;
}

extern "C" void sf_spfh_free(sf_ctx *ctx, sf_spfh *sp)
{
    if (!sp) return;
    if (ctx) (void)hipStreamSynchronize(ctx->stream);
    for (void *p : {(void *)sp->counts, (void *)sp->k, (void *)sp->p4, (void *)sp->live, (void *)sp->packed, (void *)sp->hi})
        if (p) { if (ctx) sf_pool_release(ctx, p); else (void)hipFree(p); }
    delete sp;
}

static int spfh_compute(sf_ctx *ctx, sf_cloud *c, sf_nbrs *nb, sf_spfh *sp, const double *edges, double *cov)
{
    if (!ctx || !c || !nb || !sp || !edges) { sf_set_error("sf_spfh_compute: null argument"); return SF_ERR_ARG; }
    if (!nb->self) { sf_set_error("sf_spfh_compute: needs a sf_radius_search_self result"); return SF_ERR_ARG; }
    SF_CHECK(sf_nbrs_on_grid(nb, c, "sf_spfh_compute"));
    if (sp->n != c->n || nb->self_begin + nb->m > sp->n) { sf_set_error("sf_spfh_compute: table/cloud size mismatch"); return SF_ERR_ARG; }
    if (sp->elem_bytes == 1 && nb->max_count > 255 && !sp->hi) {
        sf_set_error("sf_spfh_compute: neighbourhood of %lld points needs a wider table (pass max_count to sf_spfh_create)",
                     (long long)nb->max_count);
        return SF_ERR_ARG;
    }
    if (sp->elem_bytes <= 2 && nb->max_count > 65535) {
        sf_set_error("sf_spfh_compute: neighbourhood of %lld points needs a 32-bit table (pass max_count to sf_spfh_create)",
                     (long long)nb->max_count);
        return SF_ERR_ARG;
    }
    SF_HIP(hipSetDevice(ctx->device));
    SF_CHECK(sf_cloud_ensure_sorted_normals(ctx, c));
    if (sp->n_bins > SF_FAST_FPFH_BINS && sp->elem_bytes != 1) {
        if (cov) { sf_set_error("sf_spfh_compute_moments: n_bins=%d has no shared-sweep form (use sf_spfh_compute)", sp->n_bins); return SF_ERR_UNSUPPORTED; }
        const int64_t mg = nb->m;
        if (!mg) return SF_OK;
        sf_pool_guard tmp(ctx);
        double *dedges = nullptr;
        const size_t ne = (size_t)3 * (sp->n_bins + 1);
        SF_CHECK(tmp.alloc(&dedges, ne));
        SF_HIP(hipMemcpyAsync(dedges, edges, ne * sizeof(double), hipMemcpyHostToDevice, ctx->stream));
        SF_LAUNCH(ctx, "k6_spfh", k_spfh_generic, dim3(sf_xcd_grid(sf_div_up(mg, 4))), dim3(256), c->rec, nb->offset, nb->count,
                  nb->idx, mg, nb->self_begin, (const double *)dedges, sp->n_bins, sp->nb3, sp->stride, (unsigned *)sp->counts, sp->k);
        SF_HIP(hipStreamSynchronize(ctx->stream));
        return SF_OK;
    }
    fpfh_edges ed;
    const int nbn = sp->n_bins;
    for (int i = 0; i <= SF_WIN_FPFH_BINS; ++i) {
        ed.a[i] = edges[i <= nbn ? i : nbn];
        ed.p[i] = edges[(nbn + 1) + (i <= nbn ? i : nbn)];
        ed.t[i] = edges[2 * (nbn + 1) + (i <= nbn ? i : nbn)];
        ed.tan_t[i] = std::tan(ed.t[i]);
    }
    ed.p_inv_width = (double)nbn / (ed.p[nbn] - ed.p[0]);
    const int64_t m = nb->m;
    if (!m) return SF_OK;
    int alpha_bin = -1, alpha_pair = -1;
    double nrm_max = 1.0;
    {
        double n2 = 0.0;
        SF_CHECK(sf_cloud_normals_max2(ctx, c, &n2));
        nrm_max = std::sqrt(n2) * (1.0 + 1e-12);
        const double reach = nb->radius * n2 * (1.0 + 1e-9);
        double nearest = INFINITY;
        for (int i = 0; i <= nbn; ++i) nearest = std::min(nearest, std::fabs(ed.a[i]));
        if (std::isfinite(reach) && reach < nearest)
            for (int i = 0; i < nbn; ++i)
                if (ed.a[i] < 0.0 && 0.0 < ed.a[i + 1]) alpha_bin = i;
        int a0 = 0, a1 = 0;
        const bool within = alpha_bins_within_reach(ed.a, nbn, reach, &a0, &a1);
        if (alpha_bin < 0 && within && a1 == a0 + 1) alpha_pair = a0;
        if (getenv("SF_FPFH_NO_ALPHA_SHORTCUT")) alpha_bin = alpha_pair = -1;
        if (sp->elem_bytes == 1 && sp->win_len != sp->nb3) {
            if (!within || a0 * nbn * nbn < sp->win_lo || (a1 + 1) * nbn * nbn > sp->win_lo + sp->win_len) {
                sf_set_error("sf_spfh_compute: the table keeps bins %d .. %d of %d (created for a smaller radius); a search radius of %g "
                             "reaches other alpha bins -- create the table for this radius", sp->win_lo, sp->win_lo + sp->win_len - 1,
                             sp->nb3, nb->radius);
                return SF_ERR_STATE;
            }
        }
    }
    const dim3 grid(sf_xcd_grid(sf_div_up(m, SF_SPFH_WPB))), block(64 * SF_SPFH_WPB);
    const sf_dispatch dsp = sf_nbrs_dispatch(nb);
    const dim3 grid_tail(sf_xcd_grid(sf_div_up(dsp.n_tail > 0 ? dsp.n_tail : 1, SF_SPFH_WPB)));
    const dim3 grid_mid(sf_xcd_grid(sf_div_up(dsp.n_mid > 0 ? dsp.n_mid : 1, SF_SPFH_WPB)));
    uint8_t *const hi_rows = sp->elem_bytes == 1 ? sp->hi : nullptr;
#define SF_SPFH_NB(NAME, GRID, CT, NCH, NB, SEL, SELP, NSEL)                                                            \
    SF_LAUNCH(ctx, NAME, (k_spfh<CT, NCH, NB, SEL>), GRID, block, c->rec, nb->offset, nb->count, nb->idx, m,            \
              nb->self_begin, ed, nbn, sp->nb3, sp->stride, (CT *)sp->counts, sp->k, (unsigned)sp->bias, sp->p4, nb->radius, cov, \
              sizeof(CT) == 1 ? sp->live : (unsigned *)nullptr, alpha_bin, nrm_max, fused_packed, fused_b0, fused_b1,   \
              hi_rows, dsp.limit, SELP, NSEL, dsp.view_first, alpha_pair, sizeof(CT) == 1 ? sp->win_lo : 0,                \
              sizeof(CT) == 1 ? sp->win_len : sp->nb3)
#define SF_SPFH_WIDE_1(NAME, GRID, CT, NCH, SEL, SELP, NSEL)                                                            \
    if (nbn == 9) { SF_SPFH_NB(NAME, GRID, CT, NCH, 9, SEL, SELP, NSEL); }                                              \
    else if (nbn == 11) { SF_SPFH_NB(NAME, GRID, CT, NCH, 11, SEL, SELP, NSEL); }                                       \
    else { sf_set_error("sf_spfh_compute: no fast kernel for %d bins", nbn); return SF_ERR_UNSUPPORTED; }
#define SF_SPFH_WIDE_0(NAME, GRID, CT, NCH, SEL, SELP, NSEL)                                                            \
    { sf_set_error("sf_spfh_compute: no fast kernel for %d bins on this table", nbn); return SF_ERR_UNSUPPORTED; }
#define SF_SPFH_LAUNCH(NAME, GRID, CT, NCH, SEL, SELP, NSEL, WIDE)                                                            \
    switch (nbn) {                    \
    case 1: { SF_SPFH_NB(NAME, GRID, CT, NCH, 1, SEL, SELP, NSEL); } break;                                            \
    case 2: { SF_SPFH_NB(NAME, GRID, CT, NCH, 2, SEL, SELP, NSEL); } break;                                            \
    case 3: { SF_SPFH_NB(NAME, GRID, CT, NCH, 3, SEL, SELP, NSEL); } break;                                            \
    case 4: { SF_SPFH_NB(NAME, GRID, CT, NCH, 4, SEL, SELP, NSEL); } break;                                            \
    case 5: { SF_SPFH_NB(NAME, GRID, CT, NCH, 5, SEL, SELP, NSEL); } break;                                            \
    case 6: { SF_SPFH_NB(NAME, GRID, CT, NCH, 6, SEL, SELP, NSEL); } break;                                            \
    case 7: { SF_SPFH_NB(NAME, GRID, CT, NCH, 7, SEL, SELP, NSEL); } break;                                            \
    case 8: { SF_SPFH_NB(NAME, GRID, CT, NCH, 8, SEL, SELP, NSEL); } break;                                            \
    default: { SF_SPFH_WIDE_##WIDE(NAME, GRID, CT, NCH, SEL, SELP, NSEL); } break;                                       \
    }
#define SF_SPFH_DISPATCH(CT, WIDE)                                                                        \
    switch (dsp.chunks) {                                                                           \
    case 1: { SF_SPFH_LAUNCH("k6_spfh", grid, CT, 1, false, (const int32_t *)nullptr, (int64_t)0, WIDE); } break;                \
    case 2: { SF_SPFH_LAUNCH("k6_spfh", grid, CT, 2, false, (const int32_t *)nullptr, (int64_t)0, WIDE); } break;                \
    case 3: { SF_SPFH_LAUNCH("k6_spfh", grid, CT, 3, false, (const int32_t *)nullptr, (int64_t)0, WIDE); } break;                \
    case 4: { SF_SPFH_LAUNCH("k6_spfh", grid, CT, 4, false, (const int32_t *)nullptr, (int64_t)0, WIDE); } break;                \
    default: { SF_SPFH_LAUNCH("k6_spfh", grid, CT, 0, false, (const int32_t *)nullptr, (int64_t)0, WIDE); } break;               \
    }                                                                                               \
    if (dsp.n_mid) { SF_SPFH_LAUNCH("k6_spfh_mid", grid_mid, CT, 4, true, dsp.mid_sel, dsp.n_mid, WIDE); } \
    if (dsp.n_tail) { SF_SPFH_LAUNCH("k6_spfh_tail", grid_tail, CT, 0, true, dsp.tail_sel, dsp.n_tail, WIDE); }
    uint8_t *fused_packed = nullptr;
    int fused_b0 = -1, fused_b1 = -1;
    if (sp->elem_bytes == 1) {
        unsigned det = 0u;
        const int pin0 = alpha_bin >= 0 ? alpha_bin : alpha_pair, pin1 = alpha_bin >= 0 ? alpha_bin : alpha_pair + 1;
        if (pin0 >= 0)
            for (int blk = (pin0 * nbn * nbn - sp->win_lo) / 16; blk <= ((pin1 + 1) * nbn * nbn - 1 - sp->win_lo) / 16; ++blk) det |= 1u << blk;
        const unsigned m8 = sp->host_live[0] & 0xffu;
        if (det && sp->mask_known && sp->host_live_valid && (m8 | det) == m8 && __builtin_popcount(m8) <= 2 && sp->host_live[1] == m8) {
            fused_packed = sp->packed;
            fused_b0 = m8 ? __builtin_ffs((int)m8) - 1 : 0;
            const unsigned rest = m8 & (m8 - 1u);
            fused_b1 = rest ? __builtin_ffs((int)rest) - 1 : (fused_b0 + 1) & 7;
            SF_SPFH_DISPATCH(uint8_t, 1)
            return SF_OK;
        }
        if (det) SF_LAUNCH(ctx, "k6_spfh_pack", k_spfh_live_or, dim3(1), dim3(1), sp->live, det);
        SF_SPFH_DISPATCH(uint8_t, 1)
        SF_LAUNCH(ctx, "k6_spfh_pack", k_spfh_pack, dim3((unsigned)sf_div_up(m, 256)), dim3(256), (const uint8_t *)sp->counts,
                  nb->self_begin, nb->self_begin + m, (const unsigned *)sp->live, sp->packed);
        SF_LAUNCH(ctx, "k6_spfh_pack", k_spfh_repack, dim3(2048), dim3(256), (const uint8_t *)sp->counts, sp->n, nb->self_begin,
                  nb->self_begin + m, (const unsigned *)sp->live, sp->packed);
        SF_LAUNCH(ctx, "k6_spfh_pack", k_spfh_pack_done, dim3(1), dim3(1), sp->live);
        if (det && sp->mask_known) {
            sp->host_live[0] |= det;
            const unsigned m8 = sp->host_live[0] & 0xffu;
            sp->host_live[1] = __builtin_popcount(m8) <= 2 ? m8 : ~0u;
            sp->host_live_valid = true;
        } else {
            sp->mask_known = false;
            sp->host_live_valid = false;
        }
    } else if (sp->elem_bytes == 2) {
        SF_SPFH_DISPATCH(uint16_t, 0)
    } else {
        SF_SPFH_DISPATCH(uint32_t, 0)
    }
#undef SF_SPFH_DISPATCH
#undef SF_SPFH_WIDE_1
#undef SF_SPFH_WIDE_0
#undef SF_SPFH_LAUNCH
#undef SF_SPFH_NB
    return SF_OK;
}

extern "C" int sf_spfh_compute(sf_ctx *ctx, sf_cloud *c, sf_nbrs *nb, sf_spfh *sp, const double *edges)
{
    return spfh_compute(ctx, c, nb, sp, edges, nullptr);
}

extern "C" int sf_spfh_compute_moments(sf_ctx *ctx, sf_cloud *c, sf_nbrs *nb, sf_spfh *sp, const double *edges,
                                       double *cov_dev)
{
    if (!cov_dev) { sf_set_error("sf_spfh_compute_moments: null cov"); return SF_ERR_ARG; }
    return spfh_compute(ctx, c, nb, sp, edges, cov_dev);
}

extern "C" int sf_spfh_allgather(sf_ctx *ctx, sf_spfh *sp, int64_t rows_per_rank)
{
    if (!ctx || !sp) { sf_set_error("sf_spfh_allgather: null argument"); return SF_ERR_ARG; }
    if (ctx->nranks == 1 && !ctx->comm) return SF_OK;
    if (rows_per_rank <= 0 || rows_per_rank * ctx->nranks > sp->rows_alloc || rows_per_rank * ctx->nranks < sp->n) {
        sf_set_error("sf_spfh_allgather: %lld rows/rank x %d ranks does not tile a table of %lld (+pad %lld) rows",
                     (long long)rows_per_rank, ctx->nranks, (long long)sp->n, (long long)sp->rows_alloc);
        return SF_ERR_ARG;
    }
    const size_t row_bytes = (size_t)sp->stride * sp->elem_bytes;
    char *base = (char *)sp->counts;
    if (ctx->comm && ctx->nranks > 1) {
        sf_pool_guard tmp(ctx);
        int *fw = nullptr;
        SF_CHECK(tmp.alloc(&fw, 2));
        const int word = (int)sp->elem_bytes | (sp->hi ? 1 << 8 : 0) | (sp->p4 ? 1 << 9 : 0) | ((int)sp->stride << 12);
        void *pin = nullptr;
        SF_CHECK(sf_ctx_pinned(ctx, &pin));
        int *hw = (int *)((char *)pin + SF_PINNED_BYTES - 16);
        hw[0] = word;
        hw[1] = -word;
        SF_HIP(hipMemcpyAsync(fw, hw, 2 * sizeof(int), hipMemcpyHostToDevice, ctx->stream));
        SF_CHECK(sf_comm_allreduce_max_i32(ctx, fw, fw, 2));
        SF_HIP(hipMemcpyAsync(hw, fw, 2 * sizeof(int), hipMemcpyDeviceToHost, ctx->stream));
        SF_HIP(hipStreamSynchronize(ctx->stream));
        if (hw[0] != word || hw[1] != -word) {
            sf_set_error("sf_spfh_allgather: the ranks hold SPFH tables of different storage (this rank: %d-byte counts%s%s, stride %d; "
                         "format words over the ranks %#x .. %#x) -- size every rank's table by the longest list of ANY rank",
                         sp->elem_bytes, sp->hi ? " + high-byte rows" : "", sp->p4 ? " + packed rows" : "", (int)sp->stride,
                         (unsigned)-hw[1], (unsigned)hw[0]);
            return SF_ERR_STATE;
        }
    }
    SF_CHECK(sf_comm_allgather(ctx, base + (size_t)ctx->rank * rows_per_rank * row_bytes, base,
                               (size_t)rows_per_rank * row_bytes));
    char *kb = (char *)sp->k;
    SF_CHECK(sf_comm_allgather(ctx, kb + (size_t)ctx->rank * rows_per_rank * sizeof(int32_t), kb,
                               (size_t)rows_per_rank * sizeof(int32_t)));
    if (sp->p4) {
        char *pb = (char *)sp->p4;
        SF_CHECK(sf_comm_allgather(ctx, pb + (size_t)ctx->rank * rows_per_rank * 32, pb, (size_t)rows_per_rank * 32));
    }
    if (sp->hi) {
        char *hb = (char *)sp->hi;
        SF_CHECK(sf_comm_allgather(ctx, hb + (size_t)ctx->rank * rows_per_rank * 128, hb, (size_t)rows_per_rank * 128));
    }
    if (sp->live) {
        SF_HIP(hipMemsetAsync(sp->live, 0xff, 2 * sizeof(unsigned), ctx->stream));
        sp->host_live[0] = sp->host_live[1] = ~0u;
        sp->host_live_valid = sp->mask_known = true;
    }
    return SF_OK;
}

struct spfh_part { char *base; size_t row; };
#define SF_WIRE_PARTS 3
static int spfh_wire_parts(sf_ctx *ctx, sf_spfh *sp, spfh_part parts[SF_WIRE_PARTS])
{
    parts[2] = spfh_part{nullptr, 0};
    if (sp->elem_bytes == 1) {
        const unsigned m8 = sp->host_live[0] & 0xffu;
        const bool sparse = sp->mask_known && sp->host_live_valid && __builtin_popcount(m8) <= 2 && sp->host_live[1] == m8;
        if (!sparse) {
            SF_HIP(hipMemsetAsync(sp->live, 0xff, 2 * sizeof(unsigned), ctx->streams[0]));
            sp->host_live[0] = sp->host_live[1] = ~0u;
            sp->host_live_valid = sp->mask_known = true;
        }
        parts[0] = sparse ? spfh_part{(char *)sp->packed, 32} : spfh_part{(char *)sp->counts, 128};
        parts[1] = spfh_part{(char *)sp->p4, 32};
        if (sp->hi) parts[2] = spfh_part{(char *)sp->hi, 128};
    } else {
        parts[0] = spfh_part{(char *)sp->counts, (size_t)sp->stride * sp->elem_bytes};
        parts[1] = spfh_part{(char *)sp->k, sizeof(int32_t)};
    }
    return SF_OK;
}

extern "C" int sf_spfh_rows_image(sf_ctx *ctx, sf_spfh *sp, int64_t begin, int64_t end, void *host, size_t cap, int write_back,
                                  size_t *bytes)
{
    if (!ctx || !sp || begin < 0 || begin > end || end > sp->n) { sf_set_error("sf_spfh_rows_image: bad argument"); return SF_ERR_ARG; }
    SF_HIP(hipSetDevice(ctx->device));
    spfh_part parts[SF_WIRE_PARTS];
    SF_CHECK(spfh_wire_parts(ctx, sp, parts));
    const size_t rows = (size_t)(end - begin), need = rows * (parts[0].row + parts[1].row + parts[2].row);
    if (bytes) *bytes = need;
    if (!host) return SF_OK;
    if (cap < need) { sf_set_error("sf_spfh_rows_image: %zu bytes needed, %zu given", need, cap); return SF_ERR_ARG; }
    char *h = (char *)host;
    for (const spfh_part &pt : parts) {
        if (!pt.row) continue;
        char *d = pt.base + (size_t)begin * pt.row;
        if (rows) {
            if (write_back) SF_HIP(hipMemcpyAsync(d, h, rows * pt.row, hipMemcpyHostToDevice, ctx->stream));
            else SF_HIP(hipMemcpyAsync(h, d, rows * pt.row, hipMemcpyDeviceToHost, ctx->stream));
        }
        h += rows * pt.row;
    }
    SF_HIP(hipStreamSynchronize(ctx->stream));
    return SF_OK;
}

extern "C" int sf_spfh_exchange_rows(sf_ctx *ctx, sf_spfh *sp, int n_ops, const int *peer, const int64_t *send_begin,
                                     const int64_t *send_end, const int64_t *recv_begin, const int64_t *recv_end)
{
    if (!ctx || !sp || n_ops < 0 || (n_ops && (!peer || !send_begin || !send_end || !recv_begin || !recv_end))) {
        sf_set_error("sf_spfh_exchange_rows: bad argument");
        return SF_ERR_ARG;
    }
    for (int i = 0; i < n_ops; ++i)
        if (send_begin[i] < 0 || send_begin[i] > send_end[i] || send_end[i] > sp->n || recv_begin[i] < 0 ||
            recv_begin[i] > recv_end[i] || recv_end[i] > sp->n) {
            sf_set_error("sf_spfh_exchange_rows: operation %d names rows outside the table of %lld", i, (long long)sp->n);
            return SF_ERR_ARG;
        }
    SF_HIP(hipSetDevice(ctx->device));
    spfh_part parts[SF_WIRE_PARTS];
    SF_CHECK(spfh_wire_parts(ctx, sp, parts));
    std::vector<int> peers;
    std::vector<const void *> sends;
    std::vector<void *> recvs;
    std::vector<size_t> sbytes, rbytes;
    for (int i = 0; i < n_ops; ++i)
        for (const spfh_part &pt : parts) {
            if (!pt.row) continue;
            peers.push_back(peer[i]);
            sends.push_back(pt.base + (size_t)send_begin[i] * pt.row);
            sbytes.push_back((size_t)(send_end[i] - send_begin[i]) * pt.row);
            recvs.push_back(pt.base + (size_t)recv_begin[i] * pt.row);
            rbytes.push_back((size_t)(recv_end[i] - recv_begin[i]) * pt.row);
        }
    return sf_comm_exchange(ctx, (int)peers.size(), peers.data(), sends.data(), sbytes.data(), recvs.data(), rbytes.data());
}

extern "C" int sf_spfh_export(sf_ctx *ctx, sf_cloud *c, sf_spfh *sp, double *out, int flags)
{
    if (!ctx || !c || !sp || !out) { sf_set_error("sf_spfh_export: null argument"); return SF_ERR_ARG; }
    SF_HIP(hipSetDevice(ctx->device));
// ... 27 lines not shown
```

### shot_fpfh_amd/engine.py

```python
from __future__ import annotations

import collections
import ctypes as C
import operator
import os
import threading
import weakref
from typing import Optional

import numpy as np

from . import _ffi
from ._ffi import SF_HOST, SF_IN_DEVICE, SF_OUT_DEVICE, ShotFpfhError

__all__ = ["Engine", "Cloud", "Neighbors", "Spfh", "DeviceArray", "default_engine", "ShotFpfhError", "fpfh_edges"]


def _f64(a, cols: Optional[int] = None) -> np.ndarray:
    arr = np.ascontiguousarray(a, dtype=np.float64)
    if cols is not None and (arr.ndim != 2 or arr.shape[1] != cols):
        raise ValueError(f"expected an (N, {cols}) array, got shape {arr.shape}")
    return arr


# ... 964 lines not shown
                "sf_shot_single_scale",
            )
            return out
        res = self.engine.host_empty((self.m, _ffi.SHOT_LEN))
        _ffi.check(
            self.engine.lib.sf_shot_single_scale(self.engine.h, self.cloud.h, self.h, int(bool(normalize)),
                                                 int(min_neighborhood_size), None, _ptr(res), SF_HOST),
            "sf_shot_single_scale",
        )
        return res

    def shot_serial(self, min_neighborhood_size: int = 10, n_cosine_bins: Optional[int] = None,
                    out: Optional[DeviceArray] = None):
        if n_cosine_bins is None:
            if out is not None:
                raise ValueError("shot_serial: `out` needs n_cosine_bins")
            res = self.engine.host_empty((self.m, _ffi.SHOT_LEN))
            _ffi.check(
                self.engine.lib.sf_shot_serial(self.engine.h, self.cloud.h, self.h, int(min_neighborhood_size), _ptr(res), SF_HOST),
                "sf_shot_serial",
            )
            return res
        n = operator.index(n_cosine_bins)
        if not 1 <= n <= _ffi.MAX_COSINE_BINS:
            raise ValueError(f"shot_serial: n_cosine_bins = {n} outside [1, {_ffi.MAX_COSINE_BINS}]")
        if out is None:
            res = self.engine.host_empty((self.m, 32 * n))
            ptr, flags = _ptr(res), SF_HOST
        else:
            if out.nbytes < self.m * 32 * n * 8:
                raise ValueError(f"shot_serial: `out` holds {out.nbytes} bytes, the rows need {self.m * 32 * n * 8}")
            res, ptr, flags = out, out.ptr, SF_OUT_DEVICE
        rc = self.engine.lib.sf_shot_serial_bins(self.engine.h, self.cloud.h, self.h, n, int(min_neighborhood_size), ptr, flags)
        if rc == _ffi.SF_ERR_BIN_RANGE:
            raise IndexError(_ffi.last_error())
        _ffi.check(rc, "sf_shot_serial_bins")
        return res

    def shot_from_moments(self, moments: DeviceArray, first_row: int, normalize: bool, min_neighborhood_size: int,
                          out: DeviceArray, lrf_out: Optional[DeviceArray] = None) -> DeviceArray:
        _ffi.check(
            self.engine.lib.sf_shot_from_moments(self.engine.h, self.cloud.h, self.h, moments.offset_ptr(first_row * 48),
                                                 int(bool(normalize)), int(min_neighborhood_size),
                                                 None if lrf_out is None else lrf_out.ptr, out.ptr, SF_OUT_DEVICE),
            "sf_shot_from_moments",
        )
        return out

    def lrf_raw_from_moments(self, moments: DeviceArray, first_row: int, lrf_out: DeviceArray) -> None:
        _ffi.check(
            self.engine.lib.sf_lrf_raw_from_moments(self.engine.h, self.cloud.h, self.h, moments.offset_ptr(first_row * 48),
                                                    lrf_out.ptr),
            "sf_lrf_raw_from_moments",
        )

    def shot_from_raw_lrf(self, lrf: DeviceArray, normalize: bool, min_neighborhood_size: int, out: DeviceArray) -> DeviceArray:
        _ffi.check(
            self.engine.lib.sf_shot_from_raw_lrf(self.engine.h, self.cloud.h, self.h, lrf.ptr, int(bool(normalize)),
                                                 int(min_neighborhood_size), out.ptr),
            "sf_shot_from_raw_lrf",
        )
        return out

    def free(self) -> None:
        if getattr(self, "h", None) and self.engine.h:
            self.engine.lib.sf_nbrs_free(self.engine.h, self.h)
        self.h = None

    def __del__(self):
        try:
            self.free()
        except Exception:
            pass


class Spfh:

    def __init__(self, cloud: Cloud, n_bins: int, max_count: int, radius: Optional[float] = None):
        self.cloud, self.engine, self.n_bins = cloud, cloud.engine, int(n_bins)
        self.edges = fpfh_edges(self.n_bins)
        if radius is not None and radius > 0:
            self.h = _ffi.check_handle(
                self.engine.lib.sf_spfh_create_for_radius(self.engine.h, cloud.h, self.n_bins, int(max_count), float(radius)),
                "sf_spfh_create_for_radius")
        else:
            self.h = _ffi.check_handle(
                self.engine.lib.sf_spfh_create(self.engine.h, cloud.h, self.n_bins, int(max_count)), "sf_spfh_create"
            )
        self.elem_bytes = int(self.engine.lib.sf_spfh_elem_bytes(self.h))

    def compute(self, self_nbrs: Neighbors, moments_out: Optional[DeviceArray] = None) -> "Spfh":
        if moments_out is not None:
            _ffi.check(
                self.engine.lib.sf_spfh_compute_moments(self.engine.h, self.cloud.h, self_nbrs.h, self.h, _ptr(self.edges),
                                                        moments_out.ptr),
                "sf_spfh_compute_moments",
            )
            return self
        _ffi.check(
            self.engine.lib.sf_spfh_compute(self.engine.h, self.cloud.h, self_nbrs.h, self.h, _ptr(self.edges)), "sf_spfh_compute"
        )
        return self

    def allgather(self, rows_per_rank: int) -> None:
        _ffi.check(self.engine.lib.sf_spfh_allgather(self.engine.h, self.h, int(rows_per_rank)), "sf_spfh_allgather")

    def exchange_rows(self, ops) -> None:
        ops = list(ops)
        n = len(ops)
        peers = (C.c_int * max(n, 1))(*[int(o[0]) for o in ops])
        cols = [(C.c_int64 * max(n, 1))(*[int(o[j]) for o in ops]) for j in (1, 2, 3, 4)]
        _ffi.check(self.engine.lib.sf_spfh_exchange_rows(self.engine.h, self.h, n, peers, *cols), "sf_spfh_exchange_rows")

    def rows_image(self, begin: int, end: int) -> np.ndarray:
        need = C.c_size_t(0)
        lib, eh = self.engine.lib, self.engine.h
        _ffi.check(lib.sf_spfh_rows_image(eh, self.h, int(begin), int(end), None, 0, 0, C.byref(need)), "sf_spfh_rows_image")
        img = np.zeros(need.value, dtype=np.uint8)
        _ffi.check(lib.sf_spfh_rows_image(eh, self.h, int(begin), int(end), _ptr(img), img.size, 0, None), "sf_spfh_rows_image")
        return img

    def set_rows_image(self, begin: int, end: int, image: np.ndarray) -> None:
        img = np.ascontiguousarray(image, dtype=np.uint8)
        _ffi.check(self.engine.lib.sf_spfh_rows_image(self.engine.h, self.h, int(begin), int(end), _ptr(img), img.size, 1, None),
                   "sf_spfh_rows_image")

    def export(self) -> np.ndarray:
        out = np.zeros((self.cloud.n, self.n_bins**3))
        _ffi.check(self.engine.lib.sf_spfh_export(self.engine.h, self.cloud.h, self.h, _ptr(out), SF_HOST), "sf_spfh_export")
        return out

    def fpfh(self, self_nbrs: Neighbors, keypoints_indices=None, out: Optional[DeviceArray] = None, out_row: int = 0):
        nb3 = self.n_bins**3
        if keypoints_indices is None:
            m, kp = self_nbrs.m, None
        else:
            kp = np.ascontiguousarray(keypoints_indices, dtype=np.int64)
            m = kp.shape[0]
        if out is not None:
            if out_row < 0 or out_row + m > out.shape[0]:
                raise ValueError("fpfh: output rows outside the array")
            _ffi.check(
                self.engine.lib.sf_fpfh(self.engine.h, self.cloud.h, self_nbrs.h, self.h, _ptr(kp), m,
                                        out.offset_ptr(out_row * nb3 * 8), SF_OUT_DEVICE),
                "sf_fpfh",
            )
            return out
        res = self.engine.host_empty((m, nb3))
        _ffi.check(
            self.engine.lib.sf_fpfh(self.engine.h, self.cloud.h, self_nbrs.h, self.h, _ptr(kp), m, _ptr(res), SF_HOST), "sf_fpfh"
        )
        return res

    def free(self) -> None:
        if getattr(self, "h", None) and self.engine.h:
            self.engine.lib.sf_spfh_free(self.engine.h, self.h)
        self.h = None

    def __del__(self):
        try:
            self.free()
        except Exception:
            pass


_default: Optional[Engine] = None
_default_lock = threading.Lock()


def default_engine() -> Engine:
    global _default
    with _default_lock:
        if _default is None or _default.pid != os.getpid() or _default.h is None:
            _default = Engine()
        return _default
```

### shot_fpfh_amd/sharding.py

```python
from __future__ import annotations

from dataclasses import dataclass
from typing import Optional

import numpy as np

from .engine import Cloud, DeviceArray, Engine, Neighbors, Spfh

__all__ = ["ShardPlan", "ExchangePlan", "exchange_plan", "DescriptorJob", "MatchJob", "SubsetMatchJob"]


@dataclass(frozen=True)
class ShardPlan:

    n: int
    world: int = 1
    rank: int = 0

    def __post_init__(self):
        if self.world < 1 or not 0 <= self.rank < self.world or self.n < 0:
            raise ValueError(f"bad shard plan n={self.n} world={self.world} rank={self.rank}")

    @property
    def rows_per_rank(self) -> int:
        return -(-self.n // self.world) if self.n else 0

    def block(self, rank: Optional[int] = None) -> tuple[int, int]:
        r = self.rank if rank is None else rank
        b = min(r * self.rows_per_rank, self.n)
        return b, min(b + self.rows_per_rank, self.n)

    @property
    def begin(self) -> int:
        return self.block()[0]

    @property
    def end(self) -> int:
        return self.block()[1]


@dataclass(frozen=True)
class ExchangePlan:

    halo: tuple[int, int]
    interior: tuple[int, int]
    ops: tuple


def _layer_of(first: np.ndarray, pos: int) -> int:
    return int(np.searchsorted(first, pos, side="right")) - 1


def exchange_plan(layer_first, n: int, world: int, rank: int) -> ExchangePlan:
    first = np.asarray(layer_first, dtype=np.int64)
    nl = first.size - 1
    if nl < 1 or first[0] != 0 or first[-1] != n:
        raise ValueError("layer table does not describe a cloud of this size")

    def halo_of(r: int):
        b, e = ShardPlan(n, world, r).block()
        if b == e:
            return b, e, b, e
        zb, ze = _layer_of(first, b), _layer_of(first, e - 1)
        return b, e, min(int(first[max(zb - 1, 0)]), b), max(int(first[min(ze + 2, nl)]), e)

    b, e, hb, he = halo_of(rank)
    i0 = i1 = b
    if b < e:
        zb, ze = _layer_of(first, b), _layer_of(first, e - 1)
        ok = [z for z in range(zb, ze + 1) if first[max(z - 1, 0)] >= b and first[min(z + 2, nl)] <= e]
        if ok:
            i0, i1 = max(int(first[ok[0]]), b), min(int(first[ok[-1] + 1]), e)
    ops = []
    for p in range(world):
        if p == rank:
            continue
        pb, pe, phb, phe = halo_of(p)
        rb, re = (max(hb, pb), min(b, pe)) if p < rank else (max(e, pb), min(he, pe))
        sb, se = (max(phb, b), min(pb, e)) if rank < p else (max(pe, b), min(phe, e))
        rb, re = (rb, re) if re > rb else (0, 0)
        sb, se = (sb, se) if se > sb else (0, 0)
        if re > rb or se > sb:
            ops.append((p, sb, se, rb, re))
    return ExchangePlan((hb, he), (i0, i1), tuple(ops))


class DescriptorJob:

    def __init__(self, engine: Engine, points, normals, radius: float, n_bins: int = 5, normalize: bool = True,
                 min_neighborhood_size: int = 10, world: int = 1, rank: int = 0, spfh_exchange: str = "neighbor",
                 do_fpfh: bool = True, do_shot: bool = True, overlap_chains: bool = False, share_sweep: bool = True,
                 emulate_peers: bool = False):
        if spfh_exchange not in ("neighbor", "halo", "allgather"):
            raise ValueError("spfh_exchange must be 'neighbor', 'halo' or 'allgather'")
        self.emulate_peers = bool(emulate_peers)
        self._halo_filled = False
        self.engine, self.radius, self.n_bins = engine, float(radius), int(n_bins)
        self.normalize, self.min_nb = bool(normalize), int(min_neighborhood_size)
        self.exchange, self.do_fpfh, self.do_shot = spfh_exchange, do_fpfh, do_shot
        self.overlap = bool(overlap_chains)
        self.share_sweep = bool(share_sweep) and do_fpfh and do_shot and self.n_bins <= 8
        self.moments: Optional[DeviceArray] = None
        self.cloud: Cloud = engine.cloud(points, normals)
        self.plan = ShardPlan(self.cloud.n, world, rank)
        m = self.plan.end - self.plan.begin
        self.m = m
        self.fpfh_out: Optional[DeviceArray] = engine.empty((m, self.n_bins**3)) if do_fpfh else None
        self.lrf_out: Optional[DeviceArray] = engine.empty((m, 9)) if do_shot else None
        self.shot_out: Optional[DeviceArray] = engine.empty((m, 352)) if do_shot else None
        self.spfh: Optional[Spfh] = None
        self._spfh_wide = -1
        self.last_pairs = 0

    def _spfh_table(self, max_count: int) -> Spfh:
        byte_capable = self.n_bins**3 <= 128 or getattr(self, "_spfh_bytes", False)
        if max_count <= 65535 and byte_capable:
            wide = 0 if max_count <= 255 else 3
        else:
            wide = 2 if max_count > 65535 else 1
        if wide == 0 and self._spfh_wide == 3:
            wide = 3
        if self.spfh is None or wide != self._spfh_wide:
            if self.spfh is not None:
                self.spfh.free()
            self.spfh = self.engine.spfh(self.cloud, self.n_bins, max_count, self.radius)
            self._spfh_bytes = getattr(self.spfh, "elem_bytes", 0) == 1
            if self._spfh_bytes and max_count <= 65535:
                wide = 3 if (max_count > 255 or wide == 3) else 0
            self._spfh_wide = wide
        return self.spfh

    def _prefill_halo(self, hb: int, he: int) -> None:
        cloud, (b, e) = self.cloud, self.plan.block()
        cloud.build_grid(self.radius, block=(b, e), reach=2)
        nb = cloud.radius_search_self(self.radius, hb, he)
        try:
            self._spfh_table(nb.max_count).compute(nb)
        finally:
            nb.free()
        self._halo_filled = True

    def _exchange_plan(self) -> ExchangePlan:
        first = self.cloud.layer_table()
        key = first.tobytes()
        if getattr(self, "_xp_key", None) != key:
            self._xp_key, self._xp = key, exchange_plan(first, self.cloud.n, self.plan.world, self.plan.rank)
        return self._xp

    def _step_neighbor(self) -> None:
        eng, cloud, (b, e) = self.engine, self.cloud, self.plan.block()
        cloud.build_grid(self.radius, block=(b, e), reach=1)
        xp = self._exchange_plan() if self.do_fpfh else None
        if self.do_fpfh and self.emulate_peers and not self._halo_filled:
            self._prefill_halo(*xp.halo)
            cloud.build_grid(self.radius, block=(b, e), reach=1)
        fold = self.do_fpfh and not self.emulate_peers
        if fold:
            eng.collective_stats(True)
        try:
            nb: Neighbors = cloud.radius_search_self(self.radius, b, e)
        finally:
            if fold:
                eng.collective_stats(False)
        try:
            self.last_pairs = nb.total
            if not self.do_fpfh:
                nb.shot_single_scale(self.normalize, self.min_nb, out=self.shot_out, lrf_out=self.lrf_out)
                return
            kind = self._spfh_wide
            longest = max(nb.max_count_all, nb.max_count)
            if getattr(eng, "fold_max_count", None) is not None and not self.emulate_peers:
                longest = eng.fold_max_count(longest)
            spfh = self._spfh_table(longest)
            if self.emulate_peers and self._spfh_wide != kind and kind != -1:
                raise RuntimeError("emulate_peers: the table changed its storage after the halo rows were filled")
            shared = self.share_sweep
            if shared:
                if self.moments is None or self.moments.shape[0] < nb.m:
                    if self.moments is not None:
                        self.moments.free()
                    self.moments = eng.empty((nb.m, 6))
                spfh.compute(nb, moments_out=self.moments)
            else:
                spfh.compute(nb)
            i0, i1 = xp.interior
            pieces = [(i0, i1), (b, i0), (i1, e)]
            views = [(lo, nb.slice(lo - b, hi - lo)) if (lo, hi) != (b, e) else (lo, nb) for lo, hi in pieces if hi > lo]
            forked = False
            try:
                eng.fork()
                forked = True
                if not self.emulate_peers:
                    spfh.exchange_rows(xp.ops)
                eng.mark()
                if shared:
                    nb.lrf_raw_from_moments(self.moments, 0, self.lrf_out)
                eng.switch(0)
                for lo, view in views:
                    if (lo, lo + view.m) != (i0, i1):
                        eng.wait_mark()
                    spfh.fpfh(view, None, out=self.fpfh_out, out_row=lo - b)
                eng.join()
                forked = False
                if shared:
                    nb.shot_from_raw_lrf(self.lrf_out, self.normalize, self.min_nb, self.shot_out)
                elif self.do_shot:
                    nb.shot_single_scale(self.normalize, self.min_nb, out=self.shot_out, lrf_out=self.lrf_out)
            finally:
                if forked:
                    eng.join()
                for _, view in views:
                    if view is not nb:
                        view.free()
        finally:
            nb.free()

    def step(self) -> None:
        cloud, (b, e) = self.cloud, self.plan.block()
        if self.plan.world > 1 and self.exchange == "neighbor":
            return self._step_neighbor()
        if self.plan.world > 1:
            cloud.build_grid(self.radius, block=(b, e), reach=2 if self.do_fpfh and self.exchange == "halo" else 1)
        else:
            cloud.build_grid(self.radius)
        if self.do_fpfh and self.exchange == "halo" and self.plan.world > 1:
            hb, he = cloud.halo_range(b, e)
        else:
            hb, he = b, e
        fold = self.plan.world > 1 and self.do_fpfh and self.exchange == "allgather"
        if fold:
            self.engine.collective_stats(True)
        try:
            nb: Neighbors = cloud.radius_search_self(self.radius, hb, he)
        finally:
            if fold:
                self.engine.collective_stats(False)
        try:
            self.last_pairs = nb.total
            blk = nb if (hb, he) == (b, e) else nb.slice(b - hb, e - b)
            try:
                two_streams = self.overlap and self.do_fpfh and self.do_shot
                if self.do_fpfh:
                    longest = nb.max_count
                    if fold:
                        longest = max(nb.max_count_all, longest)
                        if getattr(self.engine, "fold_max_count", None) is not None:
                            longest = self.engine.fold_max_count(longest)
                    spfh = self._spfh_table(longest)
                shared = self.share_sweep
                if shared:
                    if self.moments is None or self.moments.shape[0] < nb.m:
                        if self.moments is not None:
                            self.moments.free()
                        self.moments = self.engine.empty((nb.m, 6))
                    spfh.compute(nb, moments_out=self.moments)
                side_eig = shared and not two_streams
                forked = False
                try:
                    if side_eig:
                        self.engine.fork()
                        forked = True
                        blk.lrf_raw_from_moments(self.moments, b - hb, self.lrf_out)
                        self.engine.switch(0)
                    if two_streams:
                        self.engine.fork()
                        forked = True
                    if self.do_fpfh:
                        if not shared:
                            spfh.compute(nb)
                        if self.exchange == "allgather" and self.plan.world > 1:
                            spfh.allgather(self.plan.rows_per_rank)
                        spfh.fpfh(blk, None, out=self.fpfh_out)
                    if two_streams:
                        self.engine.switch(0)
                    if side_eig:
                        self.engine.join()
                        forked = False
                        blk.shot_from_raw_lrf(self.lrf_out, self.normalize, self.min_nb, self.shot_out)
                    elif self.do_shot:
                        if shared:
                            blk.shot_from_moments(self.moments, b - hb, self.normalize, self.min_nb, out=self.shot_out,
                                                  lrf_out=self.lrf_out)
                        else:
                            blk.shot_single_scale(self.normalize, self.min_nb, out=self.shot_out, lrf_out=self.lrf_out)
                finally:
                    if forked:
                        self.engine.join()
            finally:
                if blk is not nb:
                    blk.free()
        finally:
            nb.free()

    def step_replay(self) -> None:
        if self.plan.world > 1 and not self.emulate_peers:
            return self.step()
        g = getattr(self, "_graph", None)
        if g is not None:
            return g.launch()
        self._eager_steps = getattr(self, "_eager_steps", 0) + 1
        if getattr(self, "_graph_failed", None):
            return self.step()
        if self._eager_steps <= 2 or not getattr(self, "_sync_free", False):
            before = self.engine.lib.sf_sync_count()
            self.step()
            self._sync_free = self.engine.lib.sf_sync_count() == before
            if self._eager_steps > 8 and not self._sync_free:
                self._graph_failed = "the step waits for the device (a host read-back in it): not capturable"
            return
        try:
            self._graph = self.engine.capture(self.step)
        except Exception as exc:
            self._graph_failed = f"{type(exc).__name__}: {exc}"
            return self.step()
        return self._graph.launch()

    def block_original_indices(self) -> np.ndarray:
        b, e = self.plan.block()
        return self.cloud.perm()[b:e].astype(np.int64)

    def close(self) -> None:
        if getattr(self, "_graph", None) is not None:
            self._graph.free()
            self._graph = None
        for obj in (self.spfh, self.fpfh_out, self.lrf_out, self.shot_out, self.moments, self.cloud):
            if obj is not None:
                obj.free()
        self.spfh = self.fpfh_out = self.lrf_out = self.shot_out = self.moments = None


class MatchJob:

    def __init__(self, engine: Engine, length: int, n_scan: int, n_ref: int, world: int = 1, rank: int = 0, chunks: int = 1):
        self.engine, self.d = engine, int(length)
        self.scan_plan, self.ref_plan = ShardPlan(n_scan, world, rank), ShardPlan(n_ref, world, rank)
        rpr = max(self.ref_plan.rows_per_rank, 1)
        self.ref_all: DeviceArray = engine.empty((rpr * world, self.d))
        self.ref_ok: DeviceArray = engine.empty((rpr * world,), np.uint8)
        m = self.scan_plan.end - self.scan_plan.begin
        self.scan_ok: DeviceArray = engine.empty((max(m, 1),), np.uint8)
        self.idx: DeviceArray = engine.empty((max(m, 1),), np.int64)
        self.dist: DeviceArray = engine.empty((max(m, 1),), np.float64)
        self.m = m
        self.chunks = 1
        if chunks > 1 and rpr % 64 == 0 and m > 0:
            self._piece = -(-(-(-rpr // int(chunks))) // 64) * 64
            self.chunks = -(-rpr // self._piece)

    def _pieces(self, c: int):
        plan, rpr = self.ref_plan, max(self.ref_plan.rows_per_rank, 1)
        out = []
        for r in range(plan.world):
            rb = r * rpr + c * self._piece
            re = min(r * rpr + min((c + 1) * self._piece, rpr), plan.n)
            if re > rb:
                out.append((r, rb, re))
        return out

    def run(self, scan_block: DeviceArray, ref_block: DeviceArray, gather: bool = True, match: bool = True) -> None:
        eng, plan = self.engine, self.ref_plan
        row_bytes = self.d * 8
        b, e = plan.block()
        self.ref_all.copy_from_device(ref_block, dst_byte_offset=b * row_bytes, nbytes=(e - b) * row_bytes)
        self._scan_block, self._ref_block = scan_block, ref_block
        if self.chunks > 1:
            return self._run_streamed(scan_block, gather, match)
        if gather:
            eng.allgather(self.ref_all, plan.rows_per_rank * row_bytes)
        if not match:
            return
        eng.rows_nonzero_device(self.ref_all, self.ref_ok, n_rows=plan.n)
        if self.m:
            eng.rows_nonzero_device(scan_block, self.scan_ok, n_rows=self.m)
            eng.match_masked_device(scan_block, self.scan_ok, self.ref_all, self.ref_ok, self.idx, self.dist,
                                    a_rows=self.m, b_rows=plan.n)

    def _bmax_over_ranks(self, local: float) -> float:
        if self.ref_plan.world == 1:
            return local
        buf = self.engine.empty((1,), np.uint64)
        try:
            buf.from_host(~np.array([local], dtype=np.float64).view(np.uint64))
            self.engine.allreduce_min_u64(buf, 1)
            return float((~buf.to_host()).view(np.float64)[0])
        finally:
            buf.free()

    def _run_streamed(self, scan_block: DeviceArray, do_gather: bool = True, do_match: bool = True) -> None:
        eng, plan, me = self.engine, self.ref_plan, self.ref_plan.rank
        row_bytes = self.d * 8
        b, e = plan.block()

        def exchange(c: int) -> None:
            if not do_gather or plan.world == 1:
                return
            piece = {r: (rb, re) for (r, rb, re) in self._pieces(c)}
            sb, se = piece.get(me, (0, 0))
            ops = []
            for p in range(plan.world):
                if p == me:
                    continue
                rb, re = piece.get(p, (0, 0))
                if se > sb or re > rb:
                    ops.append((p, self.ref_all if se > sb else None, sb * row_bytes, (se - sb) * row_bytes,
                                self.ref_all if re > rb else None, rb * row_bytes, (re - rb) * row_bytes))
            eng.exchange(ops)

# ... 178 lines not shown
```

Before: 560.7 million.

## Compute SHOT frame moments inside the FPFH K7 kernel instead of SPFH

Moves the weighted covariance (frame moment) accumulation out of the SPFH kernel and into the sparse FPFH K7 kernel, which already loads neighbour positions and distances. This lets the SPFH pass run without moments at a higher occupancy target. Single-rank runs with eligible tables take a new step path that calls SPFH plain, then FPFH with moments, then LRF and SHOT. The wave-reduction helpers also switch from shuffles to permlane swaps. The cost is extra register pressure in the FPFH kernel and a more serialized schedule, since the LRF now has to wait for FPFH instead of running on a side stream.

New measurement: 582.9 million, median of 6. 1.04x the previous value.

```diff
diff --git a/include/shotfpfh.h b/include/shotfpfh.h
--- a/include/shotfpfh.h
+++ b/include/shotfpfh.h
@@ -135,6 +135,9 @@
 void sf_spfh_free(sf_ctx *ctx, sf_spfh *spfh);
 int sf_fpfh(sf_ctx *ctx, sf_cloud *cloud, sf_nbrs *self_nbrs, sf_spfh *spfh, const int64_t *kp_idx, int64_t m,
             double *out , int flags);
+int sf_fpfh_carries_moments(sf_ctx *ctx, sf_nbrs *self_nbrs, sf_spfh *spfh);
+int sf_fpfh_moments(sf_ctx *ctx, sf_cloud *cloud, sf_nbrs *self_nbrs, sf_spfh *spfh, int64_t m, double *out ,
+                    double *cov_dev , int flags);
 
 int sf_match_argmin(sf_ctx *ctx, const double *a, int64_t m1, const double *b, int64_t m2, int64_t d,
                     int64_t *idx, double *dist, int64_t *col_idx, int flags);
diff --git a/shot_fpfh_amd/_ffi.py b/shot_fpfh_amd/_ffi.py
--- a/shot_fpfh_amd/_ffi.py
+++ b/shot_fpfh_amd/_ffi.py
@@ -9,6 +9,7 @@
 SF_HOST, SF_OUT_DEVICE, SF_IN_DEVICE = 0, 1, 2
 SHOT_LEN = 352
 MAX_COSINE_BINS = 64
+SF_ERR_UNSUPPORTED = -6
 SF_ERR_BIN_RANGE = -7
 MAX_FPFH_BINS = 1290
 
@@ -90,6 +91,8 @@
     "sf_spfh_export": (_int, [_vp, _vp, _vp, _vp, _int]),
     "sf_spfh_free": (None, [_vp, _vp]),
     "sf_fpfh": (_int, [_vp, _vp, _vp, _vp, _vp, _i64, _vp, _int]),
+    "sf_fpfh_carries_moments": (_int, [_vp, _vp, _vp]),
+    "sf_fpfh_moments": (_int, [_vp, _vp, _vp, _vp, _i64, _vp, _vp, _int]),
     "sf_match_argmin": (_int, [_vp, _vp, _i64, _vp, _i64, _i64, _vp, _vp, _vp, _int]),
     "sf_match_top2": (_int, [_vp, _vp, _i64, _vp, _i64, _i64, _vp, _vp, _vp, _int]),
     "sf_rows_nonzero": (_int, [_vp, _vp, _i64, _i64, _vp]),
diff --git a/shot_fpfh_amd/csrc/device_util.h b/shot_fpfh_amd/csrc/device_util.h
--- a/shot_fpfh_amd/csrc/device_util.h
+++ b/shot_fpfh_amd/csrc/device_util.h
@@ -76,20 +76,34 @@
                             __builtin_amdgcn_readlane(__double2loint(v), 63));
 }
 
+typedef unsigned sf_u2 __attribute__((ext_vector_type(2)));
+template <int W>
+__device__ __forceinline__ void sf_lane_swap(double &a, double &b)
+{
+    const unsigned alo = (unsigned)__double2loint(a), ahi = (unsigned)__double2hiint(a);
+    const unsigned blo = (unsigned)__double2loint(b), bhi = (unsigned)__double2hiint(b);
+    const sf_u2 lo = W == 32 ? __builtin_amdgcn_permlane32_swap(alo, blo, false, false) : __builtin_amdgcn_permlane16_swap(alo, blo, false, false);
+    const sf_u2 hi = W == 32 ? __builtin_amdgcn_permlane32_swap(ahi, bhi, false, false) : __builtin_amdgcn_permlane16_swap(ahi, bhi, false, false);
+    a = __hiloint2double((int)hi[0], (int)lo[0]);
+    b = __hiloint2double((int)hi[1], (int)lo[1]);
+}
+
 __device__ inline double sf_wave_sum8(const double (&v)[8])
 {
     const int lane = sf_lane();
-    const bool b5 = lane & 32, b4 = lane & 16, b3 = lane & 8;
+    const bool b3 = lane & 8;
     double k4[4], k2[2];
 #pragma unroll
     for (int i = 0; i < 4; ++i) {
-        const double mine = b5 ? v[4 + i] : v[i], send = b5 ? v[i] : v[4 + i];
-        k4[i] = mine + __shfl_xor(send, 32);
+        double a = v[i], b = v[4 + i];
+        sf_lane_swap<32>(a, b);
+        k4[i] = a + b;
     }
 #pragma unroll
     for (int i = 0; i < 2; ++i) {
-        const double mine = b4 ? k4[2 + i] : k4[i], send = b4 ? k4[i] : k4[2 + i];
-        k2[i] = mine + __shfl_xor(send, 16);
+        double a = k4[i], b = k4[2 + i];
+        sf_lane_swap<16>(a, b);
+        k2[i] = a + b;
     }
     double r;
     {
@@ -113,16 +127,16 @@
 
 __device__ inline double sf_wave_sum4(const double (&v)[4])
 {
-    const int lane = sf_lane();
-    const bool b5 = lane & 32, b4 = lane & 16;
     double k2[2];
 #pragma unroll
     for (int i = 0; i < 2; ++i) {
-        const double mine = b5 ? v[2 + i] : v[i], send = b5 ? v[i] : v[2 + i];
-        k2[i] = mine + __shfl_xor(send, 32);
-    }
-    const double mine = b4 ? k2[1] : k2[0], send = b4 ? k2[0] : k2[1];
-    double r = mine + __shfl_xor(send, 16);
+        double a = v[i], b = v[2 + i];
+        sf_lane_swap<32>(a, b);
+        k2[i] = a + b;
+    }
+    double r0 = k2[0], r1 = k2[1];
+    sf_lane_swap<16>(r0, r1);
+    double r = r0 + r1;
 #define SF_DPP_ADD(ctrl)                                                                                  \
     {                                                                                                     \
         const int lo = __builtin_amdgcn_update_dpp(0, __double2loint(r), ctrl, 0xf, 0xf, false);          \
diff --git a/shot_fpfh_amd/csrc/fpfh.hip b/shot_fpfh_amd/csrc/fpfh.hip
--- a/shot_fpfh_amd/csrc/fpfh.hip
+++ b/shot_fpfh_amd/csrc/fpfh.hip
@@ -199,14 +199,15 @@
                           abuf_all[wv_id], hi, limit);
 }
 
-template <int NKS, bool HI>
+template <int NKS, bool HI, bool MOM = false>
 __global__ __launch_bounds__(64 * SF_MC_WPB) __attribute__((amdgpu_waves_per_eu(8, 8))) void k_fpfh_mc_sparse(
     const double *__restrict__ rec, const int64_t *__restrict__ offset, const int32_t *__restrict__ cnt,
     const int32_t *__restrict__ idx, int64_t nbrs_begin, const int32_t *__restrict__ kp_pos, int64_t m, sf_bin_window W,
     const uint8_t *__restrict__ counts, unsigned table_bytes, const double *__restrict__ p4, const unsigned *__restrict__ live,
     const uint8_t *__restrict__ packed, unsigned packed_bytes, double *__restrict__ out, const uint8_t *__restrict__ hi, int limit,
-    const int32_t *__restrict__ sel, int64_t nsel, int64_t view_first)
-{
+    const int32_t *__restrict__ sel, int64_t nsel, int64_t view_first, double mom_radius, double *__restrict__ cov)
+{
+    static_assert(!MOM || NKS <= 3, "the moments ride on the forms of at most three chunks");
     __shared__ __attribute__((aligned(16))) unsigned rowbuf_all[SF_MC_WPB][32 * 32];
     __shared__ __attribute__((aligned(16))) unsigned char abuf_all[SF_MC_WPB][9 * 64];
     const int wv_id = threadIdx.x >> 6;
@@ -226,11 +227,11 @@
     const unsigned rest = mask & (mask - 1u);
     const int b1 = rest ? __ffs(rest) - 1 : (b0 + 1) & 7;
     if (sf_uniform(live[1]) == mask) {
-        fpfh_mc_body_sparse<NKS, true, HI>(rec, offset, cnt, idx, nbrs_begin, kp_pos, W, counts, packed, packed_bytes, p4, out, q,
-                                           b0, b1, rowbuf_all[wv_id], abuf_all[wv_id], hi, limit);
+        fpfh_mc_body_sparse<NKS, true, HI, MOM>(rec, offset, cnt, idx, nbrs_begin, kp_pos, W, counts, packed, packed_bytes, p4, out, q,
+                                                b0, b1, rowbuf_all[wv_id], abuf_all[wv_id], hi, limit, mom_radius, cov);
     } else {
-        fpfh_mc_body_sparse<NKS, false, HI>(rec, offset, cnt, idx, nbrs_begin, kp_pos, W, counts, counts, table_bytes, p4, out, q,
-                                            b0, b1, rowbuf_all[wv_id], abuf_all[wv_id], hi, limit);
+        fpfh_mc_body_sparse<NKS, false, HI, MOM>(rec, offset, cnt, idx, nbrs_begin, kp_pos, W, counts, counts, table_bytes, p4, out, q,
+                                                 b0, b1, rowbuf_all[wv_id], abuf_all[wv_id], hi, limit, mom_radius, cov);
     }
 }
 
@@ -381,7 +382,16 @@
     return SF_OK;
 }
 
-static int launch_fpfh_mc(sf_ctx *ctx, sf_cloud *c, sf_nbrs *nb, sf_spfh *sp, const int32_t *kp_pos, int64_t m, double *dout)
+static bool fpfh_mc_carries_moments(const sf_nbrs *nb, const sf_spfh *sp)
+{
+    if (sp->elem_bytes != 1 || sp->stride != 128 || sp->win_len > 127 || !nb->self || nb->max_count > 192 || nb->max_count < 1) return false;
+    if (!sp->host_live_valid || !sp->mask_known || __builtin_popcount(sp->host_live[0] & 0xffu) > 2) return false;
+    const sf_dispatch d = sf_nbrs_dispatch(nb);
+    return d.chunks >= 1 && d.chunks <= 3 && d.n_tail == 0;
+}
+
+static int launch_fpfh_mc(sf_ctx *ctx, sf_cloud *c, sf_nbrs *nb, sf_spfh *sp, const int32_t *kp_pos, int64_t m, double *dout,
+                          double *cov = nullptr)
 {
     const dim3 grid(sf_xcd_grid(sf_div_up(m, SF_MC_WPB))), block(64 * SF_MC_WPB);
     const size_t tb = (size_t)sp->rows_alloc * 128;
@@ -413,6 +423,26 @@
 #define SF_MC_ARGS c->rec, nb->offset, nb->count, nb->idx, nb->self_begin, kp_pos, m, W, (const uint8_t *)sp->counts,       \
                    (unsigned)tb, (const double *)sp->p4, (const unsigned *)sp->live, (const uint8_t *)sp->packed,                \
                    (unsigned)((size_t)sp->rows_alloc * 32), dout, hi
+    if (cov) {
+        if (kp_pos || !fpfh_mc_carries_moments(nb, sp)) {
+            sf_set_error("sf_fpfh_moments: these lists / this table do not take a K7 form that carries the frame moments");
+            return SF_ERR_UNSUPPORTED;
+        }
+#define SF_MCM_LAUNCH2(NAME, GRID, NKS, HI, LIMIT, SELP, NSEL)                                                        \
+        SF_LAUNCH(ctx, NAME, (k_fpfh_mc_sparse<NKS, HI, true>), GRID, block, SF_MC_ARGS, LIMIT, SELP, NSEL, d.view_first, nb->radius, cov)
+#define SF_MCM_LAUNCH(NAME, GRID, NKS, LIMIT, SELP, NSEL)                                                             \
+        if (hi) { SF_MCM_LAUNCH2(NAME, GRID, NKS, true, LIMIT, SELP, NSEL); } else { SF_MCM_LAUNCH2(NAME, GRID, NKS, false, LIMIT, SELP, NSEL); }
+        if (d.chunks <= 1) { SF_MCM_LAUNCH("k7_fpfh", grid, 1, d.limit, (const int32_t *)nullptr, (int64_t)0) }
+        else if (d.chunks == 2) { SF_MCM_LAUNCH("k7_fpfh", grid, 2, d.limit, (const int32_t *)nullptr, (int64_t)0) }
+        else { SF_MCM_LAUNCH("k7_fpfh", grid, 3, d.limit, (const int32_t *)nullptr, (int64_t)0) }
+        if (d.n_mid) {
+            const dim3 grid_mid(sf_xcd_grid(sf_div_up(d.n_mid, SF_MC_WPB)));
+            SF_MCM_LAUNCH("k7_fpfh_mid", grid_mid, 3, 255, d.mid_sel, d.n_mid)
+        }
+#undef SF_MCM_LAUNCH
+#undef SF_MCM_LAUNCH2
+        return SF_OK;
+    }
     if (!sp->host_live_valid) {
         void *pin = nullptr;
         SF_CHECK(sf_ctx_pinned(ctx, &pin));
@@ -427,7 +457,7 @@
     }
     const bool sparse = __builtin_popcount(sp->host_live[0] & 0xffu) <= 2;
 #define SF_MC_LAUNCH2(NAME, GRID, NKS, HI, LIMIT, SELP, NSEL)                                                         \
-    if (sparse) { SF_LAUNCH(ctx, NAME, (k_fpfh_mc_sparse<NKS, HI>), GRID, block, SF_MC_ARGS, LIMIT, SELP, NSEL, d.view_first); } \
+    if (sparse) { SF_LAUNCH(ctx, NAME, (k_fpfh_mc_sparse<NKS, HI>), GRID, block, SF_MC_ARGS, LIMIT, SELP, NSEL, d.view_first, 0.0, (double *)nullptr); } \
     else if (padc) { SF_LAUNCH(ctx, NAME, (k_fpfh_mc<4, true, true>), GRID, block, SF_MC_ARGS, LIMIT, SELP, NSEL, d.view_first); } \
     else { SF_LAUNCH(ctx, NAME, (k_fpfh_mc<NKS, true>), GRID, block, SF_MC_ARGS, LIMIT, SELP, NSEL, d.view_first); }
 #define SF_MC_LAUNCH(NKS)                                                                                            \
@@ -460,8 +490,33 @@
     return SF_OK;
 }
 
+extern "C" int sf_fpfh_carries_moments(sf_ctx *ctx, sf_nbrs *nb, sf_spfh *sp)
+{
+    if (!ctx || !nb || !sp) return 0;
+    return fpfh_mc_carries_moments(nb, sp) ? 1 : 0;
+}
+
+static int fpfh_run(sf_ctx *ctx, sf_cloud *c, sf_nbrs *nb, sf_spfh *sp, const int64_t *kp_idx, int64_t m, double *out, int flags,
+                    double *cov);
+
 extern "C" int sf_fpfh(sf_ctx *ctx, sf_cloud *c, sf_nbrs *nb, sf_spfh *sp, const int64_t *kp_idx, int64_t m, double *out,
                        int flags)
+{
+    return fpfh_run(ctx, c, nb, sp, kp_idx, m, out, flags, nullptr);
+}
+
+extern "C" int sf_fpfh_moments(sf_ctx *ctx, sf_cloud *c, sf_nbrs *nb, sf_spfh *sp, int64_t m, double *out, double *cov_dev, int flags)
+{
+    if (!cov_dev) { sf_set_error("sf_fpfh_moments: null cov"); return SF_ERR_ARG; }
+    if (nb && sp && !fpfh_mc_carries_moments(nb, sp)) {
+        sf_set_error("sf_fpfh_moments: these lists / this table do not take a K7 form that carries the frame moments");
+        return SF_ERR_UNSUPPORTED;
+    }
+    return fpfh_run(ctx, c, nb, sp, nullptr, m, out, flags, cov_dev);
+}
+
+static int fpfh_run(sf_ctx *ctx, sf_cloud *c, sf_nbrs *nb, sf_spfh *sp, const int64_t *kp_idx, int64_t m, double *out, int flags,
+                    double *cov)
 {
     if (!ctx || !c || !nb || !sp || !out || m < 0) { sf_set_error("sf_fpfh: bad argument"); return SF_ERR_ARG; }
     if (!nb->self) { sf_set_error("sf_fpfh: needs a sf_radius_search_self result"); return SF_ERR_ARG; }
@@ -509,7 +564,7 @@
         SF_LAUNCH(ctx, "k7_fpfh", k_fpfh_generic, dim3((unsigned)m), dim3(256), c->rec, nb->offset, nb->count, nb->idx,
                   nb->self_begin, (const int32_t *)pos, m, sp->nb3, sp->stride, (const unsigned *)sp->counts, sp->k, dout);
     } else if (m)
-        rc = sp->elem_bytes == 1   ? launch_fpfh_mc(ctx, c, nb, sp, pos, m, dout)
+        rc = sp->elem_bytes == 1   ? launch_fpfh_mc(ctx, c, nb, sp, pos, m, dout, cov)
              : sp->elem_bytes == 2 ? launch_fpfh<uint16_t>(ctx, c, nb, sp, pos, m, dout)
                                    : launch_fpfh<uint32_t>(ctx, c, nb, sp, pos, m, dout);
     if (rc == SF_OK && owned) {
diff --git a/shot_fpfh_amd/csrc/fpfh_mc.h b/shot_fpfh_amd/csrc/fpfh_mc.h
--- a/shot_fpfh_amd/csrc/fpfh_mc.h
+++ b/shot_fpfh_amd/csrc/fpfh_mc.h
@@ -37,17 +37,6 @@
 #define SF_MC_WPB 4
 #endif
 
-typedef unsigned sf_u2 __attribute__((ext_vector_type(2)));
-template <int W>
-__device__ __forceinline__ void sf_lane_swap(double &a, double &b)
-{
-    const unsigned alo = (unsigned)__double2loint(a), ahi = (unsigned)__double2hiint(a);
-    const unsigned blo = (unsigned)__double2loint(b), bhi = (unsigned)__double2hiint(b);
-    const sf_u2 lo = W == 32 ? __builtin_amdgcn_permlane32_swap(alo, blo, false, false) : __builtin_amdgcn_permlane16_swap(alo, blo, false, false);
-    const sf_u2 hi = W == 32 ? __builtin_amdgcn_permlane32_swap(ahi, bhi, false, false) : __builtin_amdgcn_permlane16_swap(ahi, bhi, false, false);
-    a = __hiloint2double((int)hi[0], (int)lo[0]);
-    b = __hiloint2double((int)hi[1], (int)lo[1]);
-}
 
 template <int NKS>
 __device__ __forceinline__ void fpfh_mc_list(const int32_t *__restrict__ idx, int64_t s, int k, int lane, int (&jv)[NKS])
@@ -60,9 +49,10 @@
     }
 }
 
-template <int NKS, bool HI>
+template <int NKS, bool HI, bool MOM = false>
 __device__ __forceinline__ int fpfh_mc_weights(const double *__restrict__ p4, double px, double py, double pz, int k,
-                                               int (&jv)[NKS], double (&wv)[NKS], unsigned long long (&lm)[NKS])
+                                               int (&jv)[NKS], double (&wv)[NKS], unsigned long long (&lm)[NKS],
+                                               double mom_radius, double &mom_out)
 {
     double gx[NKS], gy[NKS], gz[NKS], gk[NKS];
 #pragma unroll
@@ -76,12 +66,20 @@
         }
     }
     double wmax = 0.0;
+    double ws = 0, a11 = 0, a21 = 0, a31 = 0, a22 = 0, a32 = 0, a33 = 0;
 #pragma unroll
     for (int c = 0; c < NKS; ++c) {
         wv[c] = 0.0;
         if (c == 0 || c * 64 < k) {
             const double cx = gx[c] - px, cy = gy[c] - py, cz = gz[c] - pz;
             const double d2 = (cx * cx + cy * cy) + cz * cz;
+            if (MOM && jv[c] >= 0) {
+                const double w = mom_radius - sf_sqrt_fast(d2);
+                ws += w;
+                const double wx = cx * w, wy = cy * w, wz = cz * w;
+                a11 = __builtin_fma(cx, wx, a11); a21 = __builtin_fma(cy, wx, a21); a31 = __builtin_fma(cz, wx, a31);
+                a22 = __builtin_fma(cy, wy, a22); a32 = __builtin_fma(cz, wy, a32); a33 = __builtin_fma(cz, wz, a33);
+            }
             const double kd = gk[c], xx = d2 * (kd * kd);
             const double y0 = __builtin_amdgcn_rsq(xx);
             const double y1 = __builtin_fma(0.5 * y0, __builtin_fma(-(xx * y0), y0, 1.0), y0);
@@ -93,6 +91,12 @@
             lm[c] = 0ull;
         }
         jv[c] = jv[c] < 0 ? 0 : jv[c];
+    }
+    if (MOM) {
+        const double part[8] = {ws, a11, a21, a31, a22, a32, a33, 0.0};
+        const double tot = sf_wave_sum8(part);
+        const double iw = sf_rcp_fast(sf_read_lane(tot, 0));
+        mom_out = tot * iw;
     }
     wmax = sf_wave_max_nonneg(wmax);
     const int e2 = wmax > 0.0 ? (int)((__double2hiint(wmax) >> 20) & 0x7ff) - 1023 : 0;
@@ -200,7 +204,8 @@
     unsigned long long lm[NKS];
     fpfh_mc_list<NKS>(idx, s, k, lane, jv);
     SF_MC_DMA(0)
-    const int S = fpfh_mc_weights<NKS, HI>(p4, px, py, pz, k, jv, wv, lm);
+    double mom_unused = 0.0;
+    const int S = fpfh_mc_weights<NKS, HI>(p4, px, py, pz, k, jv, wv, lm, 0.0, mom_unused);
 
     v4i acc[8];
 #pragma unroll
@@ -280,7 +285,7 @@
 
 #undef SF_MC_DMA
 
-template <int NKS, bool PACKED, bool HI>
+template <int NKS, bool PACKED, bool HI, bool MOM = false>
 __device__ __forceinline__ void fpfh_mc_body_sparse(const double *__restrict__ rec, const int64_t *__restrict__ offset,
                                                     const int32_t *__restrict__ cnt, const int32_t *__restrict__ idx,
                                                     int64_t nbrs_begin, const int32_t *__restrict__ kp_pos, sf_bin_window W,
@@ -288,7 +293,8 @@
                                                     unsigned rows_bytes, const double *__restrict__ p4,
                                                     double *__restrict__ out, int64_t q, int b0, int b1,
                                                     unsigned *rowbuf , unsigned char *abuf ,
-                                                    const uint8_t *__restrict__ hi, int limit)
+                                                    const uint8_t *__restrict__ hi, int limit, double mom_radius = 0.0,
+                                                    double *__restrict__ cov = nullptr )
 {
     const int lane = threadIdx.x & 63;
     const int64_t i = kp_pos ? (int64_t)kp_pos[q] : nbrs_begin + q;
@@ -330,7 +336,8 @@
     if (32 < k) SF_MCS_DMA(1)
     if (NKS >= 2 && 64 < k) SF_MCS_DMA(2)
     if (NKS >= 2 && 96 < k) SF_MCS_DMA(3)
-    const int S = fpfh_mc_weights<NKS, HI>(p4, px, py, pz, k, jv, wv, lm);
+    double mom = 0.0;
+    const int S = fpfh_mc_weights<NKS, HI, MOM>(p4, px, py, pz, k, jv, wv, lm, mom_radius, mom);
 
     v4i acc0 = v4i{0, 0, 0, 0}, acc1 = v4i{0, 0, 0, 0}, accp = v4i{0, 0, 0, 0};
     const long Bpad = (long)0x8080808080808080ull;
@@ -375,6 +382,7 @@
     double mine = tot, other = tot;
     sf_lane_swap<32>(mine, other);
     const double tot0 = mine, tot1 = other;
+    if (MOM && (lane & 7) == 0 && lane >= 8 && lane < 56) cov[6 * q + (lane >> 3) - 1] = mom;
     {
         double *o = out + q * (int64_t)W.nb3;
         fpfh_mc_zero_outside(o, W, lane);
diff --git a/shot_fpfh_amd/csrc/spfh.hip b/shot_fpfh_amd/csrc/spfh.hip
--- a/shot_fpfh_amd/csrc/spfh.hip
+++ b/shot_fpfh_amd/csrc/spfh.hip
@@ -64,12 +64,15 @@
     return b < -band * aa ? -1 : -2;
 }
 
+#ifndef SF_SPFH_PLAIN_WAVES
+#define SF_SPFH_PLAIN_WAVES 7
+#endif
 #ifndef SF_SPFH_WPB
 #define SF_SPFH_WPB 2
 #endif
 
-template <typename CT, int NCH, int NB, bool SEL>
-__global__ __launch_bounds__(64 * SF_SPFH_WPB) __attribute__((amdgpu_waves_per_eu((NCH == 0 || NCH >= 4) ? 5 : 6))) void k_spfh(const double *__restrict__ rec,
+template <typename CT, int NCH, int NB, bool SEL, bool MOM>
+__global__ __launch_bounds__(64 * SF_SPFH_WPB) __attribute__((amdgpu_waves_per_eu((NCH == 0 || NCH >= 4) ? 5 : (MOM ? 6 : SF_SPFH_PLAIN_WAVES)))) void k_spfh(const double *__restrict__ rec,
                                               const int64_t *__restrict__ offset, const int32_t *__restrict__ cnt,
     const int32_t *__restrict__ idx,
                                               int64_t m, int64_t self_begin, fpfh_edges ed, int nb_rt, int nb3, int stride,
@@ -172,18 +175,18 @@
 #pragma unroll
         for (int c = 0; c < NC; ++c)
             if ((c == 0 || c * 64 < ku) && jj[c] >= 0) {
-                if (cov) moments(cx[c] - px, cy[c] - py, cz[c] - pz);
+                if (MOM) moments(cx[c] - px, cy[c] - py, cz[c] - pz);
                 pair(cx[c] - px, cy[c] - py, cz[c] - pz, ax[c], ay[c], az[c]);
             }
     } else {
         for (int t = lane; t < k; t += 64) {
             double x, y, z, a, b, c;
             sf_load_pn(rec, idx[s + t], x, y, z, a, b, c);
-            if (cov) moments(x - px, y - py, z - pz);
+            if (MOM) moments(x - px, y - py, z - pz);
             pair(x - px, y - py, z - pz, a, b, c);
         }
     }
-    if (cov) {
+    if (MOM) {
         const double part[8] = {ws, a11, a21, a31, a22, a32, a33, 0.0};
         const double tot = sf_wave_sum8(part);
         const double wsum = __hiloint2double(__builtin_amdgcn_readlane(__double2hiint(tot), 0),
@@ -506,11 +509,14 @@
     const dim3 grid_mid(sf_xcd_grid(sf_div_up(dsp.n_mid > 0 ? dsp.n_mid : 1, SF_SPFH_WPB)));
     uint8_t *const hi_rows = sp->elem_bytes == 1 ? sp->hi : nullptr;
 #define SF_SPFH_NB(NAME, GRID, CT, NCH, NB, SEL, SELP, NSEL)                                                            \
-    SF_LAUNCH(ctx, NAME, (k_spfh<CT, NCH, NB, SEL>), GRID, block, c->rec, nb->offset, nb->count, nb->idx, m,            \
+    SF_SPFH_MOM(NAME, GRID, CT, NCH, NB, SEL, SELP, NSEL, true) else SF_SPFH_MOM(NAME, GRID, CT, NCH, NB, SEL, SELP, NSEL, false)
+#define SF_SPFH_MOM(NAME, GRID, CT, NCH, NB, SEL, SELP, NSEL, MOM)                                                       \
+    if ((cov != nullptr) == MOM) {                                                                                      \
+    SF_LAUNCH(ctx, NAME, (k_spfh<CT, NCH, NB, SEL, MOM>), GRID, block, c->rec, nb->offset, nb->count, nb->idx, m,       \
               nb->self_begin, ed, nbn, sp->nb3, sp->stride, (CT *)sp->counts, sp->k, (unsigned)sp->bias, sp->p4, nb->radius, cov, \
               sizeof(CT) == 1 ? sp->live : (unsigned *)nullptr, alpha_bin, nrm_max, fused_packed, fused_b0, fused_b1,   \
               hi_rows, dsp.limit, SELP, NSEL, dsp.view_first, alpha_pair, sizeof(CT) == 1 ? sp->win_lo : 0,                \
-              sizeof(CT) == 1 ? sp->win_len : sp->nb3)
+              sizeof(CT) == 1 ? sp->win_len : sp->nb3); }
 #define SF_SPFH_WIDE_1(NAME, GRID, CT, NCH, SEL, SELP, NSEL)                                                            \
     if (nbn == 9) { SF_SPFH_NB(NAME, GRID, CT, NCH, 9, SEL, SELP, NSEL); }                                              \
     else if (nbn == 11) { SF_SPFH_NB(NAME, GRID, CT, NCH, 11, SEL, SELP, NSEL); }                                       \
@@ -581,6 +587,7 @@
 #undef SF_SPFH_WIDE_0
 #undef SF_SPFH_LAUNCH
 #undef SF_SPFH_NB
+#undef SF_SPFH_MOM
     return SF_OK;
 }
 
diff --git a/shot_fpfh_amd/engine.py b/shot_fpfh_amd/engine.py
--- a/shot_fpfh_amd/engine.py
+++ b/shot_fpfh_amd/engine.py
@@ -1140,6 +1140,17 @@
         )
         return res
 
+    def fpfh_carries_moments(self, self_nbrs: Neighbors) -> bool:
+        return bool(self.engine.lib.sf_fpfh_carries_moments(self.engine.h, self_nbrs.h, self.h))
+
+    def fpfh_moments(self, self_nbrs: Neighbors, out: DeviceArray, moments_out: DeviceArray) -> bool:
+        rc = self.engine.lib.sf_fpfh_moments(self.engine.h, self.cloud.h, self_nbrs.h, self.h, self_nbrs.m, out.ptr,
+                                             moments_out.ptr, SF_OUT_DEVICE)
+        if rc == _ffi.SF_ERR_UNSUPPORTED:
+            return False
+        _ffi.check(rc, "sf_fpfh_moments")
+        return True
+
     def free(self) -> None:
         if getattr(self, "h", None) and self.engine.h:
             self.engine.lib.sf_spfh_free(self.engine.h, self.h)
diff --git a/shot_fpfh_amd/sharding.py b/shot_fpfh_amd/sharding.py
--- a/shot_fpfh_amd/sharding.py
+++ b/shot_fpfh_amd/sharding.py
@@ -1,5 +1,6 @@
 from __future__ import annotations
 
+import os
 from dataclasses import dataclass
 from typing import Optional
 
@@ -111,6 +112,7 @@
         self.spfh: Optional[Spfh] = None
         self._spfh_wide = -1
         self.last_pairs = 0
+        self.last_k7_moments = False
 
     def _spfh_table(self, max_count: int) -> Spfh:
         byte_capable = self.n_bins**3 <= 128 or getattr(self, "_spfh_bytes", False)
@@ -215,8 +217,21 @@
         finally:
             nb.free()
 
+    def _step_k7_moments(self, nb: Neighbors, spfh: Spfh) -> bool:
+        if os.environ.get("SF_FPFH_NO_K7_MOMENTS") or getattr(spfh, "elem_bytes", 0) != 1 or nb.max_count > 192:
+            return False
+        if not spfh.fpfh_carries_moments(nb):
+            return False
+        spfh.compute(nb)
+        if not spfh.fpfh_moments(nb, self.fpfh_out, self.moments):
+            return False
+        nb.lrf_raw_from_moments(self.moments, 0, self.lrf_out)
+        nb.shot_from_raw_lrf(self.lrf_out, self.normalize, self.min_nb, self.shot_out)
+        return True
+
     def step(self) -> None:
         cloud, (b, e) = self.cloud, self.plan.block()
+        self.last_k7_moments = False
         if self.plan.world > 1 and self.exchange == "neighbor":
             return self._step_neighbor()
         if self.plan.world > 1:
@@ -253,6 +268,9 @@
                         if self.moments is not None:
                             self.moments.free()
                         self.moments = self.engine.empty((nb.m, 6))
+                    if self.plan.world == 1 and blk is nb and not two_streams and self._step_k7_moments(nb, spfh):
+                        self.last_k7_moments = True
+                        return
                     spfh.compute(nb, moments_out=self.moments)
                 side_eig = shared and not two_streams
                 forked = False
```
